# wooginawunan/multi-modal-uncertainty

Hardware: AMD Instinct MI355X
Metric: image+text samples/sec/node, MMBT Food-101 bs=256 seq=512; ECE/NLL parity (higher is better)
Workload: dtype bf16

## Files before the change

include/mmu.h:

```cpp
#ifndef MMU_H
#define MMU_H
#include <stdint.h>

#ifdef __cplusplus
extern "C" {
#endif

typedef void* mmu_stream_t;

enum { MMU_BF16 = 0, MMU_F32 = 1 };

#define MMU_ABI_VERSION 4
int mmu_version(void);
const char* mmu_last_error(void);

int mmu_set_seed_offset(const uint64_t* dev_counter);

enum {
  MMU_EPI_STORE = 0,
  MMU_EPI_BIAS_GELU = 1,
  MMU_EPI_BIAS_DROP_RES = 2,
  MMU_EPI_DGELU = 3,
  MMU_EPI_ADD_RES = 4,
  MMU_EPI_BIAS_DROP_QGELU = 5,
  MMU_EPI_STORE_STATS = 6,
  MMU_EPI_STORE_BNB = 7,
  MMU_EPI_ADD_RES_BNB = 8,
};
typedef struct mmu_epilogue {
  int32_t kind;
  int32_t accumulate;
  const float* bias;
  int64_t bias_bstride;
  const void* residual;
  int64_t ldr, res_bstride;
  void* aux;
  int64_t ldx, aux_bstride;
  float* colsum;
  int64_t colsum_bstride;
  float drop_p;
  uint64_t seed;
  float* workspace;
  int64_t workspace_floats;
  const float* res_ln_mean;
  const float* res_ln_rstd;
  const float* res_ln_w;
  const float* res_ln_b;
  int64_t res_ln_bstride;
  const void* bn_x;
  const uint8_t* bn_mask;
  const float* bn_mean;
  const uint8_t* res_mask;
} mmu_epilogue;

int mmu_gemm(const void* A, int64_t lda, int a_kmajor,
             const void* B, int64_t ldb, int b_kmajor,
             void* C, int64_t ldc, int c_dtype,
             int64_t M, int64_t N, int64_t K,
             int64_t batch, int64_t strideA, int64_t strideB, int64_t strideC,
             const mmu_epilogue* epi, mmu_stream_t stream);

int mmu_colsum_reduce(const float* partial, int64_t parts, int64_t N, float* out,
                      int accumulate, mmu_stream_t stream);
int mmu_colsum_reduce_multi(int n, const float* const* partial, const int64_t* parts, float* const* out, int64_t N,
                            int accumulate, mmu_stream_t stream);
int mmu_colsum_bf16(const void* X, int64_t M, int64_t N, int64_t ldx, float* partial,
                    float* out, int accumulate, mmu_stream_t stream);

int mmu_transpose_bf16_batched(const int64_t* jobs, int n_jobs, int64_t max_rows, int64_t max_cols,
                               mmu_stream_t stream);

int mmu_attention_fwd(const void* QKV, int64_t ld_qkv, const float* keymask,
                      void* O, int64_t ld_o, float* LSE,
                      int64_t batch, int64_t L, int64_t heads,
                      float drop_p, uint64_t seed, uint64_t* dropmask, mmu_stream_t stream);
int mmu_attention_bwd(const void* QKV, int64_t ld_qkv, const float* keymask,
                      const void* O, int64_t ld_o, const void* dO, int64_t ld_do,
                      const float* LSE, float* delta, void* dQKV, int64_t ld_dqkv,
                      int64_t batch, int64_t L, int64_t heads,
                      float drop_p, uint64_t seed, const uint64_t* dropmask, float* dbias_parts,
                      mmu_stream_t stream);

int mmu_layernorm_fwd(const void* X, const float* w, const float* b, void* Y,
                      float* mean, float* rstd, int64_t rows, int64_t H, float eps,
                      int64_t group_rows, int64_t param_stride, mmu_stream_t stream);
int mmu_layernorm_bwd(const void* dY, const void* X, const float* mean, const float* rstd,
                      const float* w, void* dX, void* dXdrop, float drop_p, uint64_t seed,
                      float* part_dw, float* part_db, float* part_dbias,
                      int64_t rows, int64_t H, int64_t rows_per_part, mmu_stream_t stream);

int mmu_layernorm_fwd_f32(const float* X, const float* w, const float* b, void* Y, float* Y32,
                          float* mean, float* rstd, int64_t rows, int64_t H, float eps,
                          int64_t group_rows, int64_t param_stride, mmu_stream_t stream);
int mmu_layernorm_bwd_f32(const void* dY, const float* X, const float* mean, const float* rstd,
                          const float* w, void* dX, void* dXdrop, float drop_p, uint64_t seed,
                          float* part_dw, float* part_db, float* part_dbias,
                          int64_t rows, int64_t H, int64_t rows_per_part, mmu_stream_t stream);

int mmu_layernorm_bwd_res(const void* dY, const void* X, const float* mean, const float* rstd,
                          const float* w, const void* dRes, void* dX,
                          float* part_dw, float* part_db, float* part_dbias,
                          int64_t rows, int64_t H, int64_t rows_per_part, mmu_stream_t stream);

int mmu_seqattn_fwd(const void* QKV, int64_t ld_qkv, void* O, int64_t ld_o, float* LSE2,
                    int64_t S, int64_t N, int64_t heads, int64_t head_dim, mmu_stream_t stream);
int mmu_seqattn_bwd(const void* QKV, int64_t ld_qkv, const void* O, int64_t ld_o,
                    const void* dO, int64_t ld_do, const float* LSE2, float* delta,
                    void* dQKV, int64_t ld_dqkv, int64_t S, int64_t N, int64_t heads,
                    int64_t head_dim, mmu_stream_t stream);

int mmu_embed_fwd(const int64_t* ids, const int64_t* seg, const int64_t* txt_mask,
                  const float* proj, const float* word, const float* pos, const float* type,
                  const float* ln_w, const float* ln_b, float eps,
                  int64_t cls_id, int64_t sep_id,
                  const int64_t* idx, int64_t V, int64_t B, int64_t T, int64_t n_img, int64_t Lout,
                  int64_t H, float drop_txt, float drop_img, uint64_t seed,
                  void* X, float* X32, float* keymask, float* mean, float* rstd, mmu_stream_t stream);
int64_t mmu_embed_bwd_ws_floats(int64_t B, int64_t T, int64_t n_img);
int mmu_embed_bwd(const void* dX, const int64_t* ids, const int64_t* seg,
                  const float* proj, const float* word, const float* pos, const float* type,
                  const float* ln_w, const float* mean, const float* rstd,
                  int64_t cls_id, int64_t sep_id, int64_t B, int64_t T, int64_t n_img, int64_t H,
                  float drop_txt, float drop_img, uint64_t seed, float* d_word, float* d_pos, float* d_type, float* d_ln_w, float* d_ln_b,
                  float* d_proj, float* ws, mmu_stream_t stream);

int mmu_image_normalize(const uint8_t* in, int64_t n, const float* mean, const float* stdv, void* out,
                        int out_dtype, mmu_stream_t stream);

int mmu_maxpool_fwd(const void* x, int64_t B, int64_t H, int64_t W, int64_t C, void* y, uint8_t* argmax,
                    mmu_stream_t stream);
int mmu_maxpool_bwd(const void* dy, const uint8_t* argmax, int64_t B, int64_t H, int64_t W, int64_t C, void* dx,
                    mmu_stream_t stream);

int mmu_row_pool_fwd(const void* fmap, int64_t B, int64_t Hh, int64_t Ww, int64_t C, int64_t n,
                     float* out, mmu_stream_t stream);
int mmu_row_pool_bwd(const float* dout, int64_t B, int64_t Hh, int64_t Ww, int64_t C, int64_t n,
                     void* dfmap, mmu_stream_t stream);

int mmu_conv3x3_wgrad(const void* dY, const void* X, float* dW, int64_t n_img, int64_t H, int64_t W,
                      int64_t Cin, int64_t Cout, int accumulate, float* ws, int64_t ws_floats,
                      mmu_stream_t stream);

int mmu_conv3x3_implicit(const void* X, const void* Wk, void* Y, int64_t n_img, int64_t H, int64_t W,
                         int64_t C, int64_t N, float* ws, int64_t ws_floats, mmu_stream_t stream);

int mmu_conv_implicit(const void* X, const void* Wk, void* Y, int64_t n_img, int64_t H, int64_t W, int64_t C,
                      int64_t N, int64_t ksize, int64_t stride, float* ws, int64_t ws_floats,
                      mmu_stream_t stream);
int mmu_conv_implicit_stats(const void* X, const void* Wk, void* Y, int64_t n_img, int64_t H, int64_t W, int64_t C,
                            int64_t N, int64_t ksize, int64_t stride, float* stats, float* ws, int64_t ws_floats,
                            mmu_stream_t stream);
int mmu_conv3x3_implicit_bnb(const void* X, const void* Wk, void* Y, int64_t n_img, int64_t H, int64_t W, int64_t C,
                             int64_t N, const void* bn_x, const uint8_t* bn_mask, const float* bn_mean,
                             float* stats, float* ws, int64_t ws_floats, mmu_stream_t stream);
int mmu_conv_wgrad(const void* dY, const void* X, float* dW, int64_t n_img, int64_t H, int64_t W, int64_t Cin,
                   int64_t Cout, int64_t ksize, int64_t stride, int accumulate, float* ws, int64_t ws_floats,
                   mmu_stream_t stream);

int mmu_stem_conv_fwd(const void* X, const void* Wk, void* Y, int64_t n_img, int64_t H, int64_t W,
                      mmu_stream_t stream);
int64_t mmu_stem_conv_wgrad_ws_floats(int64_t n_img, int64_t H, int64_t W);
int mmu_stem_conv_wgrad(const void* dY, const void* X, float* dW, int64_t n_img, int64_t H, int64_t W,
                        int accumulate, float* ws, int64_t ws_floats, mmu_stream_t stream);

int64_t mmu_batchnorm_ws_bytes(int64_t C);
int mmu_batchnorm_fwd(const void* X, const void* skip, void* Y, int64_t rows, int64_t C,
                      const float* weight, const float* bias, float* running_mean, float* running_var,
                      int64_t* num_batches_tracked, int training, float momentum, float eps, int relu,
                      float* save_mean, float* save_invstd, void* relu_mask, const void* skip_res, void* y_res,
                      void* ws, int64_t ws_bytes, mmu_stream_t stream);
int mmu_batchnorm_fwd_parts(const void* X, const void* skip, void* Y, int64_t rows, int64_t C, const float* parts,
                            int64_t nparts, const float* weight, const float* bias, float* running_mean,
                            float* running_var, int64_t* num_batches_tracked, float momentum, float eps, int relu,
                            float* save_mean, float* save_invstd, void* relu_mask, const void* skip_res, void* y_res,
                            void* ws, int64_t ws_bytes, mmu_stream_t stream);
int mmu_batchnorm_bwd(const void* dY, const void* Y, const void* relu_mask, const void* X, int64_t rows,
                      int64_t C, const float* weight, const float* save_mean, const float* save_invstd, int relu,
                      void* dX, void* dSkip, float* dweight, float* dbias, void* ws, int64_t ws_bytes,
                      mmu_stream_t stream);

int mmu_batchnorm_bwd_parts(const void* dY, const void* Y, const void* relu_mask, const void* X, int64_t rows,
                            int64_t C, const float* parts, int64_t nparts, const float* weight,
                            const float* save_mean, const float* save_invstd, int relu, void* dX, void* dSkip,
                            float* dweight, float* dbias, void* ws, int64_t ws_bytes, mmu_stream_t stream);

int mmu_batchnorm_stats(const void* X, int64_t rows, int64_t C, double* sums, void* ws, int64_t ws_bytes,
                        mmu_stream_t stream);
int mmu_batchnorm_fwd_sums(const void* X, const void* skip, void* Y, int64_t rows, int64_t C, const double* sums,
                           const float* weight, const float* bias, float* running_mean, float* running_var,
                           int64_t* num_batches_tracked, float momentum, float eps, int relu, float* save_mean,
                           float* save_invstd, void* relu_mask, const void* skip_res, void* y_res, void* ws,
                           int64_t ws_bytes, mmu_stream_t stream);
int mmu_batchnorm_bwd_reduce(const void* dY, const void* Y, const void* relu_mask, const void* X, int64_t rows,
                             int64_t C, const float* save_mean, const float* save_invstd, int relu, double* sums,
                             float* dweight, float* dbias, void* ws, int64_t ws_bytes, mmu_stream_t stream);
int mmu_batchnorm_bwd_sums(const void* dY, const void* Y, const void* relu_mask, const void* X, int64_t rows,
                           int64_t C, const double* sums, const float* weight, const float* save_mean,
                           const float* save_invstd, int relu, void* dX, void* dSkip, void* ws, int64_t ws_bytes,
                           mmu_stream_t stream);

int mmu_bertadam_step(float* params, const float* grads, float* m, float* v, void* bf16_copy,
                      const int64_t* table, int32_t* steps, int64_t n_tensors, int64_t n_chunks,
                      float lr_decay, float lr_nodecay, float wd, float warmup, float t_total,
                      float b1, float b2, float eps, float max_grad_norm, float grad_scale,
                      float* ws, int64_t ws_floats, mmu_stream_t stream);

int mmu_uncertainty(const float* logits, const int64_t* y, int64_t S, int64_t R, int64_t C,
                    float* p_bar, float* nll, float* conf, float* correct, mmu_stream_t stream);
int mmu_ece_bins(const float* conf, const float* correct, int64_t S, int64_t n_bins,
                 float* out, mmu_stream_t stream);

int mmu_timing_enable(int on);
int mmu_timing_pause(int paused);
int mmu_timing_read(double* total_ms, int64_t* launches, double* flops);

#ifdef __cplusplus
}
#endif
#endif
```

multi-modal-uncertainty_amd/csrc/attention.hip:

```cpp
#include "mmu_common.h"
#include "mmu_internal.h"
#include <cstdlib>
#include <type_traits>
#include <utility>

namespace mmu {

constexpr float LOG2E = 1.4426950408889634f;
constexpr float LN2 = 0.6931471805599453f;
constexpr float NEG_INF = -__builtin_huge_valf();

static __device__ __forceinline__ uint32_t lowbias32(uint32_t x) {
  x ^= x >> 16; x *= 0x7feb352du; x ^= x >> 15; x *= 0x846ca68bu; x ^= x >> 16;
  return x;
}
static __device__ __forceinline__ uint32_t seed_for(uint64_t seed, int bh) {
  return lowbias32((uint32_t)seed ^ lowbias32((uint32_t)(seed >> 32) + 0x9E3779B9u * (uint32_t)(bh + 1)));
}
static __device__ __forceinline__ uint32_t drop_pair(uint32_t sbh, uint32_t q, uint32_t key, uint32_t Lp) {
  return lowbias32(((q * Lp + key) >> 1) ^ sbh);
}

static __device__ __forceinline__ float max3f(float a, float b, float c) {
  return __builtin_fmaxf(__builtin_fmaxf(a, b), c);
// ... 558 lines not shown
#pragma unroll
  for (int ks = 0; ks < 4; ++ks) {
    uint4 u = qv ? *(const uint4*)(base + (int64_t)q * p.ld_qkv + 16 * ks + 8 * h) : make_uint4(0, 0, 0, 0);
    qf[ks] = scale_frag(u, 0.125f);
    uint4 v = qv ? *(const uint4*)(dob + 16 * ks + 8 * h) : make_uint4(0, 0, 0, 0);
    df[ks] = *(bf16x8*)&v;
  }
  float dsum = 0.f;
  {
    const bf16* ob = p.o + ((int64_t)b * L + q) * p.ld_o + hd * 64;
#pragma unroll
    for (int ks = 0; ks < 4; ++ks) {
      uint4 u = qv ? *(const uint4*)(ob + 16 * ks + 8 * h) : make_uint4(0, 0, 0, 0);
      const bf16x8 ov = *(bf16x8*)&u;
#pragma unroll
      for (int e = 0; e < 8; ++e) dsum = fmaf(bf2f(ov[e]), bf2f(df[ks][e]), dsum);
    }
    dsum += __shfl_xor(dsum, 32, 64);
    if (qv && h == 0) p.delta[(int64_t)bh * L + q] = -dsum / zs;
  }
  const float nlse2 = qv ? -p.lse[(int64_t)bh * L + q] * LOG2E : -__builtin_huge_valf();
  const float ndz = -dsum / zs;
  const uint32_t ndz_bits = __float_as_uint(ndz);
  f32x16 dq[2];
#pragma unroll
  for (int i = 0; i < 16; ++i) { dq[0][i] = 0.f; dq[1][i] = 0.f; }

  uint32_t kv_off[4];
#pragma unroll
  for (int pc = 0; pc < 4; ++pc) {
    const int piece = 4 * (w & 1) + pc;
    const int row = 8 * piece + (l >> 3), c = (l & 7) ^ fsw(row);
    kv_off[pc] = (uint32_t)((row * p.ld_qkv + (w < 2 ? HD : 2 * HD) + hd * 64 + 8 * c) * 2);
  }
  const uint32_t m_off = (uint32_t)(16 * l), kw_off = (uint32_t)(((q0w + (l >> 1)) * nkv * 8) + 4 * (l & 1));
  auto issue = [&](int j) {
    char* st = smem + (j % DQ_NS) * DQ_STAGE;
    const int k0 = j * 64;
    char* dst = st + (w < 2 ? 0 : DQ_TILE);
    const __amdgpu_buffer_rsrc_t rt = urs_at(kv_base, kv_bytes, k0 * p.ld_qkv * 2);
#pragma unroll
    for (int pc = 0; pc < 4; ++pc) dma16(rt, dst + (4 * (w & 1) + pc) * 1024, kv_off[pc]);
    if (w == 0 && l < 16) dma16(urs_at(m_base, L * 4, k0 * 4), st + 2 * DQ_TILE, m_off);
    dma4(urs_at(k_base, k_bytes, j * 8), st + 2 * DQ_TILE + 256 + w * 256, kw_off);
  };
  auto wait_for = [&](int ahead) {
    if (w == 0) {
      if (ahead >= 1) asm volatile("s_waitcnt vmcnt(6)" ::: "memory");
      else asm volatile("s_waitcnt vmcnt(0)" ::: "memory");
    } else {
      if (ahead >= 1) asm volatile("s_waitcnt vmcnt(5)" ::: "memory");
      else asm volatile("s_waitcnt vmcnt(0)" ::: "memory");
    }
  };
  asm volatile("s_waitcnt vmcnt(0)" ::: "memory");
  for (int j = 0; j < DQ_NS - 1 && j < nkv; ++j) issue(j);
  auto tile_step = [&](int j, auto sg_tag) {
    constexpr int SG = decltype(sg_tag)::value;
    const int ahead = nkv - 1 - j < DQ_NS - 2 ? nkv - 1 - j : DQ_NS - 2;
    wait_for(ahead);
    raw_barrier();
    if (j + DQ_NS - 1 < nkv) issue(j + DQ_NS - 1);
    const char* st = smem + SG * DQ_STAGE;
    const char* Ks = st;
    const char* Vs = st + DQ_TILE;
    const float* mk = (const float*)(st + 2 * DQ_TILE);
    const uint32_t* kwords = (const uint32_t*)(st + 2 * DQ_TILE + 256 + w * 256);
    if (wave_live) {
      const uint64_t kw = drop ? ((uint64_t)kwords[2 * (l & 31) + 1] << 32 | kwords[2 * (l & 31)]) : ~0ull;
      const uint64_t kwh = kw >> (4 * h);
#pragma unroll
      for (int st2 = 0; st2 < 2; ++st2) {
        if (st2 == 1 && 64 * j + 32 >= L) break;
        const uint32_t kw32 = (uint32_t)(kwh >> (32 * st2));
        f32x16 sc, dp;
#pragma unroll
        for (int g = 0; g < 4; ++g) {
          const f32x4 mv = *(const f32x4*)(mk + 32 * st2 + 8 * g + 4 * h);
#pragma unroll
          for (int e = 0; e < 4; ++e) {
            sc[4 * g + e] = mv[e];
            dp[4 * g + e] = ndz;
          }
        }
#pragma unroll
        for (int ks = 0; ks < 4; ++ks) {
          sc = __builtin_amdgcn_mfma_f32_32x32x16_bf16(row_frag(Ks, 32 * st2, ks, l), qf[ks], sc, 0, 0, 0);
          dp = __builtin_amdgcn_mfma_f32_32x32x16_bf16(row_frag(Vs, 32 * st2, ks, l), df[ks], dp, 0, 0, 0);
        }
        auto one = [&](auto r_tag) {
          constexpr int r = decltype(r_tag)::value;
          const float pr = __builtin_amdgcn_exp2f(fmaf(sc[r], LOG2E, nlse2));
          const uint32_t m = keepmask<(r & 3) + 8 * (r >> 2)>(kw32);
          sc[r] = pr * __uint_as_float(bfi(m, __float_as_uint(dp[r]), ndz_bits));
        };
        static_for(one, std::make_integer_sequence<int, 16>{});
#pragma unroll
        for (int s2 = 0; s2 < 2; ++s2) {
          bf16x8 sf = acc_frag(sc, s2);
#pragma unroll
          for (int dt = 0; dt < 2; ++dt)
            dq[dt] = __builtin_amdgcn_mfma_f32_32x32x16_bf16(tr_frag(Ks, 32 * st2 + 16 * s2, 32 * dt, l), sf, dq[dt],
                                                             0, 0, 0);
        }
      }
    }
    };
  for (int j0 = 0; j0 < nkv; j0 += DQ_NS) {
    tile_step(j0, std::integral_constant<int, 0>{});
    if (j0 + 1 < nkv) tile_step(j0 + 1, std::integral_constant<int, 1>{});
    if (j0 + 2 < nkv) tile_step(j0 + 2, std::integral_constant<int, 2>{});
  }
  if (p.colsum) {
    constexpr int RS = 68;
    static_assert(4 * 32 * RS * 4 <= DQ_NS * DQ_STAGE, "dQ column-sum rows exceed the ring's LDS");
    float* rows = (float*)smem;
    raw_barrier();
    float* mine = rows + w * 32 * RS + (l & 31) * RS;
    const float sc = qv ? 0.125f * zs : 0.f;
#pragma unroll
    for (int dt = 0; dt < 2; ++dt)
#pragma unroll
      for (int g = 0; g < 4; ++g)
        *(float4*)(mine + 32 * dt + 8 * g + 4 * h) =
            make_float4(dq[dt][4 * g] * sc, dq[dt][4 * g + 1] * sc, dq[dt][4 * g + 2] * sc, dq[dt][4 * g + 3] * sc);
    raw_barrier();
    if (t < 64) {
      float v = 0.f;
      for (int r = 0; r < 128; ++r) v += rows[r * RS + t];
      p.colsum[((int64_t)bx * p.batch + b) * HD + hd * 64 + t] = v;
    }
  }
  if (!qv) return;
  bf16* ob = p.out + ((int64_t)b * L + q) * p.ld_out + hd * 64;
#pragma unroll
  for (int dt = 0; dt < 2; ++dt)
#pragma unroll
    for (int g = 0; g < 4; ++g) {
      const float s = 0.125f * zs;
      bf16x4 v = {f2bf(dq[dt][4 * g] * s), f2bf(dq[dt][4 * g + 1] * s), f2bf(dq[dt][4 * g + 2] * s),
                  f2bf(dq[dt][4 * g + 3] * s)};
      *(bf16x4*)(ob + 32 * dt + 8 * g + 4 * h) = v;
    }
}

void attention_bwd_launch(const AttnParams& p, hipStream_t s) {
  hipLaunchKernelGGL(attn_dq_dma_kernel, dim3((p.L + 127) / 128, p.batch * p.heads), dim3(256), 0, s, p);
  if (drop_thr(p.drop_p))
    hipLaunchKernelGGL(attn_dkdv_dma_kernel<true>, dim3((p.L + 63) / 64, p.batch * p.heads), dim3(128), 0, s, p);
  else
    hipLaunchKernelGGL(attn_dkdv_dma_kernel<false>, dim3((p.L + 63) / 64, p.batch * p.heads), dim3(128), 0, s, p);
}

}
```

multi-modal-uncertainty_amd/csrc/capi.hip:

```cpp
#include <stdarg.h>
#include <stdio.h>
#include <map>
#include <tuple>
#include <mutex>
#include <string>
#include <vector>
#include "mmu_internal.h"
#include <cstdlib>
#include <cmath>

using namespace mmu;

static thread_local std::string g_err;

namespace mmu {
const uint64_t* g_seed_off = nullptr;
}

int mmu_set_seed_offset(const uint64_t* dev_counter) {
  g_seed_off = dev_counter;
  return 0;
}

static int fail(const char* fmt, ...) {
  char buf[512];
  va_list ap;
  va_start(ap, fmt);
  vsnprintf(buf, sizeof buf, fmt, ap);
  va_end(ap);
  g_err = buf;
  return 1;
}

static int check_launch(const char* what) {
  hipError_t e = hipGetLastError();
  if (e != hipSuccess) return fail("%s: launch failed: %s", what, hipGetErrorString(e));
  return 0;
}

namespace {
struct Timing {
  std::mutex mu;
  bool on = false;
  bool paused = false;
  std::vector<std::pair<hipEvent_t, hipEvent_t>> pool, used;
  std::vector<double> flops;
} g_t;

std::pair<hipEvent_t, hipEvent_t> take_events() {
  std::lock_guard<std::mutex> lk(g_t.mu);
  std::pair<hipEvent_t, hipEvent_t> ev;
  if (!g_t.pool.empty()) {
    ev = g_t.pool.back();
    g_t.pool.pop_back();
  } else {
    (void)hipEventCreate(&ev.first);
    (void)hipEventCreate(&ev.second);
  }
  return ev;
}
constexpr int64_t TAIL_WS_FLOATS = 8ll << 20;
float* tail_workspace(int64_t floats, hipStream_t s, int slot = 0) {
  static std::mutex mu;
  static std::map<std::tuple<int, hipStream_t, int>, float*> bufs;
  if (floats > TAIL_WS_FLOATS) return nullptr;
  int dev = 0;
  if (hipGetDevice(&dev) != hipSuccess) return nullptr;
  std::lock_guard<std::mutex> lk(mu);
  auto it = bufs.find({dev, s, slot});
  if (it != bufs.end()) return it->second;
  hipStreamCaptureStatus st = hipStreamCaptureStatusNone;
  if (hipStreamIsCapturing(s, &st) != hipSuccess || st != hipStreamCaptureStatusNone) return nullptr;
  void* b = nullptr;
  if (hipMalloc(&b, sizeof(float) * TAIL_WS_FLOATS) != hipSuccess) {
    (void)hipGetLastError();
    return nullptr;
  }
  bufs[{dev, s, slot}] = (float*)b;
  return (float*)b;
}
}

extern "C" {

int mmu_version(void) { return MMU_ABI_VERSION; }
const char* mmu_last_error(void) { return g_err.c_str(); }

int mmu_timing_enable(int on) {
  std::lock_guard<std::mutex> lk(g_t.mu);
  g_t.on = on != 0;
  for (auto& e : g_t.used) g_t.pool.push_back(e);
  g_t.used.clear();
  g_t.flops.clear();
  return 0;
}

int mmu_timing_pause(int paused) {
  std::lock_guard<std::mutex> lk(g_t.mu);
  g_t.paused = paused != 0;
  return 0;
}

int mmu_timing_read(double* total_ms, int64_t* launches, double* flops) {
  std::lock_guard<std::mutex> lk(g_t.mu);
  double tot = 0.0, fl = 0.0;
  for (size_t i = 0; i < g_t.used.size(); ++i) {
    (void)hipEventSynchronize(g_t.used[i].second);
    float ms = 0.f;
    if (hipEventElapsedTime(&ms, g_t.used[i].first, g_t.used[i].second) != hipSuccess) return fail("timing: elapsed");
    tot += ms;
    fl += g_t.flops[i];
  }
  *total_ms = tot;
  *launches = (int64_t)g_t.used.size();
  *flops = fl;
  return 0;
}

int mmu_gemm(const void* A, int64_t lda, int a_kmajor, const void* B, int64_t ldb, int b_kmajor, void* C,
             int64_t ldc, int c_dtype, int64_t M, int64_t N, int64_t K, int64_t batch, int64_t strideA,
             int64_t strideB, int64_t strideC, const mmu_epilogue* epi, mmu_stream_t stream) {
  if (!A || !B || !C) return fail("mmu_gemm: null operand");
  if (M <= 0 || N <= 0 || K <= 0 || batch <= 0) return fail("mmu_gemm: bad shape M=%ld N=%ld K=%ld", M, N, K);
  if (N % 128) return fail("mmu_gemm: N=%ld must be a multiple of 128", N);
  if ((a_kmajor || b_kmajor) && K % 64) return fail("mmu_gemm: K=%ld must be a multiple of 64 for a K-major operand", K);
  if (!a_kmajor && M % 128) return fail("mmu_gemm: M=%ld must be a multiple of 128 when A is M-major", M);
  if ((lda % 8) || (ldb % 8) || (ldc % 4)) return fail("mmu_gemm: leading dims must be 16-B aligned");
  if (c_dtype != MMU_BF16 && c_dtype != MMU_F32) return fail("mmu_gemm: bad c_dtype");
  GemmParams p{};
  p.A = (const bf16*)A; p.B = (const bf16*)B; p.C = C;
  p.lda = lda; p.ldb = ldb; p.ldc = ldc; p.M = M; p.N = N; p.K = K;
  p.sA = strideA; p.sB = strideB; p.sC = strideC;
  const int64_t a_span = 2 * (a_kmajor ? (M + 256) * lda : (K + 64) * lda);
  const int64_t b_span = 2 * (b_kmajor ? (N + 256) * ldb : (K + 64) * ldb);
  const bool big = M >= 256 && N >= 256 && a_span < (1ll << 32) - 4096 && b_span < (1ll << 32) - 4096;
  const int tile = big ? 256 : 128;
  p.tiles_m = (int)((M + tile - 1) / tile);
  p.tiles_n = (int)((N + tile - 1) / tile);
  int kind = MMU_EPI_STORE;
  if (epi) kind = epi->kind;
  p.group_m = p.tiles_n <= 3 ? 1 : ((b_kmajor && kind != MMU_EPI_DGELU) ? 8 : 2);
  if (epi) {
    kind = epi->kind;
    p.accumulate = epi->accumulate;
    p.bias = epi->bias; p.bias_bstride = epi->bias_bstride;
    p.residual = epi->residual; p.ldr = epi->ldr; p.res_bstride = epi->res_bstride;
    p.aux = epi->aux; p.ldx = epi->ldx; p.aux_bstride = epi->aux_bstride;
    p.colsum = epi->colsum; p.colsum_bstride = epi->colsum_bstride;
    p.drop_p = epi->drop_p; p.seed = epi->seed; p.seed_off = g_seed_off;
    p.res_ln_mean = epi->res_ln_mean; p.res_ln_rstd = epi->res_ln_rstd;
    p.res_ln_w = epi->res_ln_w; p.res_ln_b = epi->res_ln_b; p.res_ln_bstride = epi->res_ln_bstride;
    p.bn_x = (const bf16*)epi->bn_x; p.bn_mask = epi->bn_mask; p.bn_mean = epi->bn_mean;
    p.res_mask = epi->res_mask;
  }
  p.kind = kind;
  if (kind < 0 || kind > MMU_EPI_ADD_RES_BNB) return fail("mmu_gemm: bad epilogue kind %d", kind);
  if ((kind == MMU_EPI_STORE_BNB || kind == MMU_EPI_ADD_RES_BNB) &&
      (!p.colsum || !p.bn_x || !p.bn_mean || batch != 1 || !a_kmajor || b_kmajor || p.accumulate || p.bias ||
       ldc != N || c_dtype != MMU_BF16))
    return fail("mmu_gemm: *_BNB needs the table (colsum), bn_x, bn_mean, batch 1, K-major A, N-major B, "
                "bf16 C with ldc == N, no bias / accumulate");
  if (kind == MMU_EPI_STORE_STATS && (!p.colsum || batch != 1 || !a_kmajor || !b_kmajor || p.accumulate))
    return fail("mmu_gemm: STORE_STATS needs the stats table (colsum), batch 1, K-major A and B, no accumulate");
  if (kind != MMU_EPI_STORE && kind != MMU_EPI_BIAS_DROP_RES && c_dtype != MMU_BF16)
    return fail("mmu_gemm: fused epilogues other than BIAS_DROP_RES write bf16");
  if (kind == MMU_EPI_BIAS_DROP_RES && c_dtype == MMU_F32 && (ldc % 4 || (epi && epi->ldr % 4)))
    return fail("mmu_gemm: f32 hidden-stream epilogue needs 16-B aligned rows");
  {
    const int nln = !!p.res_ln_mean + !!p.res_ln_rstd + !!p.res_ln_w + !!p.res_ln_b;
    if (nln && (nln != 4 || kind != MMU_EPI_BIAS_DROP_RES || c_dtype != MMU_F32))
      return fail("mmu_gemm: res_ln_* (all four) only with BIAS_DROP_RES into an f32 C");
  }
  if (kind == MMU_EPI_DGELU && !p.aux) return fail("mmu_gemm: DGELU epilogue needs aux");
  if ((kind == MMU_EPI_BIAS_DROP_RES || kind == MMU_EPI_ADD_RES || kind == MMU_EPI_ADD_RES_BNB) && !p.residual)
    return fail("mmu_gemm: epilogue needs residual");
  if (p.res_mask && ((kind != MMU_EPI_ADD_RES && kind != MMU_EPI_ADD_RES_BNB) || epi->ldr != N || batch != 1))
    return fail("mmu_gemm: res_mask only with ADD_RES / ADD_RES_BNB, batch 1, ldr == N");
  if (p.accumulate && c_dtype != MMU_F32) return fail("mmu_gemm: accumulate needs f32 C");
  if (p.drop_p < 0.f || p.drop_p >= 1.f) return fail("mmu_gemm: drop_p out of range");
  p.splitk = 1;
  p.kchunk = K;
  if (kind == MMU_EPI_STORE && c_dtype == MMU_F32 && !p.bias && !p.colsum && epi && epi->workspace && K >= 1024) {
    const int64_t tiles = (int64_t)p.tiles_m * p.tiles_n * batch;
    const int64_t max_split = 64, min_k = K >= 32768 ? 1024 : 256;
    int64_t want = (640 + tiles - 1) / tiles;
    if (want > K / min_k) want = K / min_k;
    if (want > max_split) want = max_split;
    const int64_t cap = epi->workspace_floats / (batch * M * N);
    if (want > cap) want = cap;
    if (want >= 2) {
      int64_t chunk = (K + want - 1) / want;
      chunk = (chunk + 63) / 64 * 64;
      p.kchunk = chunk;
      p.splitk = (int)((K + chunk - 1) / chunk);
      p.ws = epi->workspace;
    }
  }
  const char* wide_env = getenv("MMU_GEMM_WIDE");
  const char* wide_min_env = getenv("MMU_GEMM_WIDE_MIN_TILES");
  const int wide_mode = wide_env ? atoi(wide_env) : 1;
  const int64_t wide_min = wide_min_env ? (int64_t)atoll(wide_min_env) : (int64_t)1024;
  const bool tail_kind = kind == MMU_EPI_STORE || kind == MMU_EPI_BIAS_GELU || kind == MMU_EPI_BIAS_DROP_RES ||
                         kind == MMU_EPI_DGELU || kind == MMU_EPI_ADD_RES;
  const bool wide_kind = tail_kind && kind != MMU_EPI_DGELU;
  const bool wide = (wide_mode == 2 ? tail_kind : wide_mode == 1 && wide_kind && N >= 2304) && big && a_kmajor &&
                    b_kmajor && N % 384 == 0 && p.splitk == 1 &&
                    2 * (M + 256) * lda < (1ll << 32) - 4096 && 2 * (N + 384) * ldb < (1ll << 32) - 4096 &&
                    (M + 255) / 256 * (N / 384) * batch >= wide_min;
  if (wide) {
    p.tiles_m = (int)((M + 255) / 256);
    p.tiles_n = (int)(N / 384);
    p.group_m = p.tiles_n <= 2 ? 1 : (kind != MMU_EPI_DGELU ? 8 : 2);
  }
  const char* tail_env = getenv("MMU_GEMM_TAIL");
  const int tail_mode = tail_env ? atoi(tail_env) : 1;
  int64_t tail_rows = 0, m_main = M, tail_chunk = K;
  int tail_split = 1;
  float* tail_ws = nullptr;
  if ((tail_mode == 2 || (tail_mode == 1 && wide)) && big && batch == 1 && p.splitk == 1 && tail_kind &&
      a_kmajor && K >= 512) {
    const int64_t tiles = (int64_t)p.tiles_m * p.tiles_n, left = tiles % 256;
    if (tiles > 256 && left > 0 && left % p.tiles_n == 0 && left * 8 <= 256) {
      m_main = (int64_t)(p.tiles_m - left / p.tiles_n) * 256;
      tail_rows = M - m_main;
      const int64_t st = (tail_rows + 127) / 128 * (N / 128);
      int64_t sk = 256 / st;
      if (sk > K / 256) sk = K / 256;
      if (sk < 1) sk = 1;
      tail_chunk = ((K + sk - 1) / sk + 63) / 64 * 64;
      tail_split = (int)((K + tail_chunk - 1) / tail_chunk);
      tail_ws = tail_split >= 2 ? tail_workspace((int64_t)tail_split * tail_rows * N, (hipStream_t)stream) : nullptr;
      if (!tail_ws) {
        tail_rows = 0;
        m_main = M;
      }
    }
  }
  hipStream_t s = (hipStream_t)stream;
  bool timed;
  std::pair<hipEvent_t, hipEvent_t> ev;
  {
    std::lock_guard<std::mutex> lk(g_t.mu);
    timed = g_t.on && !g_t.paused;
  }
  if (timed) {
    ev = take_events();
    (void)hipEventRecord(ev.first, s);
  }
  const char* csp_env = getenv("MMU_GEMM_CS_PART");
  const bool cs_rows_ok = p.colsum && batch == 1 && p.splitk == 1 && kind != MMU_EPI_STORE_STATS &&
                          kind != MMU_EPI_STORE_BNB && kind != MMU_EPI_ADD_RES_BNB && (!csp_env || atoi(csp_env) != 0);
  const int cs_rows_main = (big && !wide) ? 128 : 64;
  const int64_t cs_parts_main = (m_main + cs_rows_main - 1) / cs_rows_main;
  const int64_t cs_parts = cs_parts_main + (tail_rows + 63) / 64;
  float* cs_part = cs_rows_ok ? tail_workspace(cs_parts * N, s, 1) : nullptr;
  if (cs_part) {
    p.cs_part = cs_part;
    p.cs_m0 = 0;
    p.cs_rows = cs_rows_main;
  }
  {
    GemmParams pm = p;
    if (tail_rows) pm.tiles_m = (int)(m_main / 256);
    if (!(wide && gemm_wide_launch(pm, c_dtype == MMU_F32, (int)batch, s)))
      gemm_launch(pm, a_kmajor != 0, b_kmajor != 0, c_dtype == MMU_F32, big, (int)batch, s);
  }
  if (tail_rows) {
    GemmParams pt = p;
    pt.A = p.A + m_main * lda;
    pt.M = tail_rows;
    pt.kind = MMU_EPI_STORE;
    pt.accumulate = 0;
    pt.splitk = tail_split;
    pt.kchunk = tail_chunk;
    pt.ws = tail_ws;
    pt.tiles_m = (int)((tail_rows + 127) / 128);
    pt.tiles_n = (int)(N / 128);
    pt.group_m = 1;
    pt.cs_part = nullptr;
    gemm_launch(pt, true, b_kmajor != 0, true, false, 1, s);
    GemmParams pe = p;
    if (cs_part) {
      pe.cs_part = cs_part + cs_parts_main * N;
      pe.cs_m0 = m_main;
      pe.cs_rows = 64;
    }
    splitk_epilogue_launch(pe, c_dtype == MMU_F32, tail_ws, m_main, tail_rows, tail_split, s);
  }
  if (cs_part) colsum_reduce_launch(cs_part, cs_parts, N, p.colsum, 1, s);
  if (p.splitk > 1) splitk_reduce_launch(p, (int)batch, s);
  if (timed) {
    (void)hipEventRecord(ev.second, s);
    std::lock_guard<std::mutex> lk(g_t.mu);
    g_t.used.push_back(ev);
    g_t.flops.push_back(2.0 * (double)M * (double)N * (double)K * (double)batch);
  }
  return check_launch("mmu_gemm");
}

int mmu_transpose_bf16_batched(const int64_t* jobs, int n_jobs, int64_t max_rows, int64_t max_cols,
                               mmu_stream_t stream) {
  if (!jobs || n_jobs <= 0 || n_jobs > 65535 || max_rows <= 0 || max_cols <= 0)
    return fail("mmu_transpose_bf16_batched: bad args");
  transpose_bf16_batched_launch(jobs, n_jobs, max_rows, max_cols, (hipStream_t)stream);
  return check_launch("mmu_transpose_bf16_batched");
}

int mmu_colsum_reduce(const float* partial, int64_t parts, int64_t N, float* out, int accumulate,
                      mmu_stream_t stream) {
  if (!partial || !out || parts <= 0 || N <= 0) return fail("mmu_colsum_reduce: bad args");
  colsum_reduce_launch(partial, parts, N, out, accumulate, (hipStream_t)stream);
  return check_launch("mmu_colsum_reduce");
}

int mmu_colsum_reduce_multi(int n, const float* const* partial, const int64_t* parts, float* const* out, int64_t N,
                            int accumulate, mmu_stream_t stream) {
  if (n <= 0 || n > COLSUM_MULTI || !partial || !parts || !out || N <= 0)
    return fail("mmu_colsum_reduce_multi: bad args (1 <= n <= %d)", COLSUM_MULTI);
  ColsumJobs jobs{};
  for (int z = 0; z < n; ++z) {
    if (!partial[z] || !out[z] || parts[z] <= 0) return fail("mmu_colsum_reduce_multi: bad job %d", z);
    jobs.part[z] = partial[z];
    jobs.parts[z] = parts[z];
    jobs.out[z] = out[z];
  }
  colsum_reduce_multi_launch(jobs, n, N, accumulate, (hipStream_t)stream);
  return check_launch("mmu_colsum_reduce_multi");
}

int mmu_colsum_bf16(const void* X, int64_t M, int64_t N, int64_t ldx, float* partial, float* out, int accumulate,
                    mmu_stream_t stream) {
  if (!X || !out || M <= 0 || N <= 0 || N % 8 || ldx % 8) return fail("mmu_colsum_bf16: bad args");
  colsum_bf16_launch((const bf16*)X, M, N, ldx, partial, out, accumulate, (hipStream_t)stream);
  return check_launch("mmu_colsum_bf16");
}

static int attn_common(int64_t ld_qkv, int64_t batch, int64_t L, int64_t heads, float drop_p) {
  if (batch <= 0 || L <= 0 || heads <= 0) return fail("attention: bad shape");
  if (ld_qkv < 3 * heads * 64 || ld_qkv % 8) return fail("attention: ld_qkv too small / unaligned");
  if (drop_p < 0.f || drop_p >= 1.f) return fail("attention: drop_p out of range");
  if ((int64_t)batch * heads > 65535 * 64) return fail("attention: batch*heads too large");
  if (L > 576) return fail("attention: L=%ld > 576 (the kernels stage ceil(L/64) <= 9 key tiles)", L);
  return 0;
}

int mmu_attention_fwd(const void* QKV, int64_t ld_qkv, const float* keymask, void* O, int64_t ld_o, float* LSE,
                      int64_t batch, int64_t L, int64_t heads, float drop_p, uint64_t seed, uint64_t* dropmask,
                      mmu_stream_t stream) {
  if (!QKV || !keymask || !O || !LSE) return fail("mmu_attention_fwd: null pointer");
  if (attn_common(ld_qkv, batch, L, heads, drop_p)) return 1;
  if (ld_o < heads * 64 || ld_o % 8) return fail("mmu_attention_fwd: bad ld_o");
  if (batch * heads > 65535) return fail("mmu_attention_fwd: batch*heads > 65535");
  AttnParams p{};
  p.qkv = (const bf16*)QKV; p.ld_qkv = ld_qkv; p.keymask = keymask; p.out = (bf16*)O; p.ld_out = ld_o;
  p.lse = LSE; p.batch = (int)batch; p.L = (int)L; p.heads = (int)heads; p.drop_p = drop_p; p.seed = seed;
  p.seed_off = g_seed_off;
  p.dropmask = dropmask;
  attention_fwd_launch(p, (hipStream_t)stream);
  return check_launch("mmu_attention_fwd");
}

int mmu_attention_bwd(const void* QKV, int64_t ld_qkv, const float* keymask, const void* O, int64_t ld_o,
                      const void* dO, int64_t ld_do, const float* LSE, float* delta, void* dQKV, int64_t ld_dqkv,
                      int64_t batch, int64_t L, int64_t heads, float drop_p, uint64_t seed,
                      const uint64_t* dropmask, float* dbias_parts, mmu_stream_t stream) {
  if (!QKV || !keymask || !O || !dO || !LSE || !delta || !dQKV) return fail("mmu_attention_bwd: null pointer");
  if ((uint32_t)(drop_p * 65536.0f + 0.5f) != 0 && !dropmask)
    return fail("mmu_attention_bwd: dropout needs the forward's dropmask");
  if (attn_common(ld_qkv, batch, L, heads, drop_p)) return 1;
  if (ld_dqkv < 3 * heads * 64 || ld_do < heads * 64 || ld_o < heads * 64 || ld_do % 8 || ld_o % 8 || ld_dqkv % 4)
    return fail("mmu_attention_bwd: bad ld");
  if (batch * heads > 65535) return fail("mmu_attention_bwd: batch*heads > 65535");
  AttnParams p{};
  p.qkv = (const bf16*)QKV; p.ld_qkv = ld_qkv; p.keymask = keymask; p.o = (const bf16*)O; p.ld_o = ld_o;
  p.dout = (const bf16*)dO; p.ld_do = ld_do; p.lse = (float*)LSE; p.delta = delta; p.out = (bf16*)dQKV;
  p.ld_out = ld_dqkv; p.batch = (int)batch; p.L = (int)L; p.heads = (int)heads; p.drop_p = drop_p; p.seed = seed;
  p.seed_off = g_seed_off;
  p.dropmask = (uint64_t*)dropmask;
  p.colsum = dbias_parts;
  attention_bwd_launch(p, (hipStream_t)stream);
  return check_launch("mmu_attention_bwd");
}

int mmu_layernorm_fwd(const void* X, const float* w, const float* b, void* Y, float* mean, float* rstd, int64_t rows,
                      int64_t H, float eps, int64_t group_rows, int64_t param_stride, mmu_stream_t stream) {
  if (!X || !w || !b || !Y) return fail("mmu_layernorm_fwd: null pointer");
  if ((mean == nullptr) != (rstd == nullptr)) return fail("mmu_layernorm_fwd: mean/rstd must both be given or NULL");
  if (rows <= 0 || H <= 0 || H % 256 || H > 1024) return fail("mmu_layernorm_fwd: H=%ld must be 256/512/768/1024", H);
  if (group_rows <= 0) group_rows = rows;
  if (param_stride < 0) return fail("mmu_layernorm_fwd: bad param_stride");
  layernorm_fwd_launch((const bf16*)X, w, b, (bf16*)Y, mean, rstd, rows, H, eps, group_rows, param_stride,
                       (hipStream_t)stream);
  return check_launch("mmu_layernorm_fwd");
}

int mmu_layernorm_bwd(const void* dY, const void* X, const float* mean, const float* rstd, const float* w, void* dX,
                      void* dXdrop, float drop_p, uint64_t seed, float* part_dw, float* part_db, float* part_dbias,
                      int64_t rows, int64_t H, int64_t rows_per_part, mmu_stream_t stream) {
  if (!dY || !X || !mean || !rstd || !w || !dX) return fail("mmu_layernorm_bwd: null pointer");
  if (rows <= 0 || H <= 0 || H % 256 || H > 1024 || rows_per_part <= 0) return fail("mmu_layernorm_bwd: bad shape");
  if (drop_p < 0.f || drop_p >= 1.f) return fail("mmu_layernorm_bwd: drop_p out of range");
  layernorm_bwd_launch((const bf16*)dY, X, false, mean, rstd, w, (bf16*)dX, (bf16*)dXdrop, nullptr, drop_p, seed,
                       g_seed_off, part_dw, part_db, part_dbias, rows, H, rows_per_part, (hipStream_t)stream);
  return check_launch("mmu_layernorm_bwd");
}

int mmu_layernorm_fwd_f32(const float* X, const float* w, const float* b, void* Y, float* Y32, float* mean,
                          float* rstd, int64_t rows, int64_t H, float eps, int64_t group_rows, int64_t param_stride,
                          mmu_stream_t stream) {
  if (!X || !w || !b || !Y) return fail("mmu_layernorm_fwd_f32: null pointer");
  if ((mean == nullptr) != (rstd == nullptr)) return fail("mmu_layernorm_fwd_f32: mean/rstd must both be given or NULL");
  if (rows <= 0 || H <= 0 || H % 256 || H > 1024) return fail("mmu_layernorm_fwd_f32: H=%ld must be 256/512/768/1024", H);
  if (group_rows <= 0) group_rows = rows;
  if (param_stride < 0) return fail("mmu_layernorm_fwd_f32: bad param_stride");
  layernorm_fwd32_launch(X, w, b, (bf16*)Y, Y32, mean, rstd, rows, H, eps, group_rows, param_stride,
                         (hipStream_t)stream);
  return check_launch("mmu_layernorm_fwd_f32");
}

int mmu_layernorm_bwd_f32(const void* dY, const float* X, const float* mean, const float* rstd, const float* w,
                          void* dX, void* dXdrop, float drop_p, uint64_t seed, float* part_dw, float* part_db,
                          float* part_dbias, int64_t rows, int64_t H, int64_t rows_per_part, mmu_stream_t stream) {
  if (!dY || !X || !mean || !rstd || !w || !dX) return fail("mmu_layernorm_bwd_f32: null pointer");
  if (rows <= 0 || H <= 0 || H % 256 || H > 1024 || rows_per_part <= 0) return fail("mmu_layernorm_bwd_f32: bad shape");
  if (drop_p < 0.f || drop_p >= 1.f) return fail("mmu_layernorm_bwd_f32: drop_p out of range");
  layernorm_bwd_launch((const bf16*)dY, X, true, mean, rstd, w, (bf16*)dX, (bf16*)dXdrop, nullptr, drop_p, seed,
                       g_seed_off, part_dw, part_db, part_dbias, rows, H, rows_per_part, (hipStream_t)stream);
  return check_launch("mmu_layernorm_bwd_f32");
}

int mmu_layernorm_bwd_res(const void* dY, const void* X, const float* mean, const float* rstd, const float* w,
                          const void* dRes, void* dX, float* part_dw, float* part_db, float* part_dbias, int64_t rows,
                          int64_t H, int64_t rows_per_part, mmu_stream_t stream) {
  if (!dY || !X || !mean || !rstd || !w || !dX || !dRes) return fail("mmu_layernorm_bwd_res: null pointer");
  if (rows <= 0 || H <= 0 || H % 256 || H > 1024 || rows_per_part <= 0) return fail("mmu_layernorm_bwd_res: bad shape");
  layernorm_bwd_launch((const bf16*)dY, X, false, mean, rstd, w, (bf16*)dX, nullptr, (const bf16*)dRes, 0.f, 0,
                       nullptr, part_dw, part_db, part_dbias, rows, H, rows_per_part, (hipStream_t)stream);
  return check_launch("mmu_layernorm_bwd_res");
}

static int seqattn_check(const char* what, int64_t ld_qkv, int64_t S, int64_t N, int64_t heads, int64_t D) {
  if (S <= 0 || N <= 0 || heads <= 0) return fail("%s: bad shape", what);
  if (D != 64 && D != 128 && D != 256) return fail("%s: head_dim %ld not in {64, 128, 256}", what, D);
  if (ld_qkv < 3 * heads * D || ld_qkv % 8) return fail("%s: ld_qkv too small / unaligned", what);
  if (N * heads > 65535) return fail("%s: N*heads > 65535", what);
  return 0;
}

int mmu_seqattn_fwd(const void* QKV, int64_t ld_qkv, void* O, int64_t ld_o, float* LSE2, int64_t S, int64_t N,
                    int64_t heads, int64_t head_dim, mmu_stream_t stream) {
  if (!QKV || !O || !LSE2) return fail("mmu_seqattn_fwd: null pointer");
  if (seqattn_check("mmu_seqattn_fwd", ld_qkv, S, N, heads, head_dim)) return 1;
  if (ld_o < heads * head_dim || ld_o % 4) return fail("mmu_seqattn_fwd: bad ld_o");
  SeqAttnParams p{};
  p.qkv = (const bf16*)QKV; p.ld_qkv = ld_qkv;
  p.out = (bf16*)O; p.ld_out = ld_o;
  p.lse2 = LSE2;
  p.S = (int)S; p.N = (int)N; p.heads = (int)heads; p.D = (int)head_dim; p.E = (int)(heads * head_dim);
  p.scale = 1.0f / sqrtf((float)head_dim);
  seqattn_fwd_launch(p, (hipStream_t)stream);
  return check_launch("mmu_seqattn_fwd");
}

int mmu_seqattn_bwd(const void* QKV, int64_t ld_qkv, const void* O, int64_t ld_o, const void* dO, int64_t ld_do,
                    const float* LSE2, float* delta, void* dQKV, int64_t ld_dqkv, int64_t S, int64_t N, int64_t heads,
                    int64_t head_dim, mmu_stream_t stream) {
  if (!QKV || !O || !dO || !LSE2 || !delta || !dQKV) return fail("mmu_seqattn_bwd: null pointer");
  if (seqattn_check("mmu_seqattn_bwd", ld_qkv, S, N, heads, head_dim)) return 1;
  if (ld_dqkv < 3 * heads * head_dim || ld_dqkv % 4 || ld_o % 4 || ld_do % 8) return fail("mmu_seqattn_bwd: bad ld");
  SeqAttnParams p{};
  p.qkv = (const bf16*)QKV; p.ld_qkv = ld_qkv;
  p.o = (const bf16*)O; p.ld_o = ld_o;
  p.dout = (const bf16*)dO; p.ld_do = ld_do;
  p.out = (bf16*)dQKV; p.ld_out = ld_dqkv;
  p.lse2 = (float*)LSE2; p.delta = delta;
  p.S = (int)S; p.N = (int)N; p.heads = (int)heads; p.D = (int)head_dim; p.E = (int)(heads * head_dim);
  p.scale = 1.0f / sqrtf((float)head_dim);
  seqattn_bwd_launch(p, (hipStream_t)stream);
  return check_launch("mmu_seqattn_bwd");
}


int mmu_embed_fwd(const int64_t* ids, const int64_t* seg, const int64_t* txt_mask, const float* proj, const float* word,
                  const float* pos, const float* type, const float* ln_w, const float* ln_b, float eps, int64_t cls_id,
                  int64_t sep_id, const int64_t* idx, int64_t V, int64_t B, int64_t T, int64_t n_img, int64_t Lout,
                  int64_t H, float drop_txt, float drop_img, uint64_t seed, void* X, float* X32, float* keymask,
                  float* mean, float* rstd, mmu_stream_t stream) {
  if (H != 768) return fail("mmu_embed_fwd: H must be 768");
  if (!word || !pos || !type || !ln_w || !ln_b || !X || !keymask || !proj) return fail("mmu_embed_fwd: null pointer");
  if (T > 0 && (!ids || !seg)) return fail("mmu_embed_fwd: text ids/segments missing");
  if (V <= 0 || B <= 0 || Lout <= 0 || n_img <= 0) return fail("mmu_embed_fwd: bad shape");
  if (!idx && Lout != n_img + 2 + T) return fail("mmu_embed_fwd: identity variant needs Lout == n_img+2+T");
  EmbedParams p{};
  p.ids = ids; p.seg = seg; p.txt_mask = txt_mask; p.idx = idx; p.proj = proj; p.word = word; p.pos = pos;
  p.type = type; p.ln_w = ln_w; p.ln_b = ln_b; p.eps = eps; p.cls_id = cls_id; p.sep_id = sep_id; p.V = V; p.B = B;
  p.T = T; p.n_img = n_img; p.Lout = Lout; p.H = H; p.X = (bf16*)X; p.X32 = X32;
  if (drop_txt < 0.f || drop_txt >= 1.f || drop_img < 0.f || drop_img >= 1.f) return fail("mmu_embed_fwd: bad dropout");
  p.drop_txt = drop_txt; p.drop_img = drop_img; p.seed = seed; p.seed_off = g_seed_off; p.keymask = keymask; p.mean = mean; p.rstd = rstd;
  embed_fwd_launch(p, (hipStream_t)stream);
  return check_launch("mmu_embed_fwd");
}

int64_t mmu_embed_bwd_ws_floats(int64_t B, int64_t T, int64_t n_img) {
  return 4 * embed_bwd_blocks(B, n_img + 2 + T) * 768;
}

int mmu_embed_bwd(const void* dX, const int64_t* ids, const int64_t* seg, const float* proj, const float* word,
                  const float* pos, const float* type, const float* ln_w, const float* mean, const float* rstd,
                  int64_t cls_id, int64_t sep_id, int64_t B, int64_t T, int64_t n_img, int64_t H, float drop_txt,
                  float drop_img, uint64_t seed, float* d_word,
                  float* d_pos, float* d_type, float* d_ln_w, float* d_ln_b, float* d_proj, float* ws,
                  mmu_stream_t stream) {
  if (H != 768) return fail("mmu_embed_bwd: H must be 768");
  if (!dX || !ids || !seg || !proj || !word || !pos || !type || !ln_w || !mean || !rstd || !d_word || !d_pos ||
      !d_type || !d_ln_w || !d_ln_b || !d_proj || !ws)
    return fail("mmu_embed_bwd: null pointer");
  EmbedBwdParams q{};
  q.dX = (const bf16*)dX; q.ids = ids; q.seg = seg; q.proj = proj; q.word = word; q.pos = pos; q.type = type;
  q.ln_w = ln_w; q.mean = mean; q.rstd = rstd; q.cls_id = cls_id; q.sep_id = sep_id; q.B = B; q.T = T;
  q.n_img = n_img; q.H = H; q.drop_txt = drop_txt; q.drop_img = drop_img; q.seed = seed; q.seed_off = g_seed_off; q.d_word = d_word; q.d_pos = d_pos; q.d_type = d_type; q.d_ln_w = d_ln_w;
  q.d_ln_b = d_ln_b; q.d_proj = d_proj; q.ws = ws;
  embed_bwd_launch(q, (hipStream_t)stream);
  return check_launch("mmu_embed_bwd");
}

int mmu_image_normalize(const uint8_t* in, int64_t n, const float* mean, const float* stdv, void* out,
                        int out_dtype, mmu_stream_t stream) {
  if (!in || !out || !mean || !stdv || n < 0) return fail("mmu_image_normalize: bad args");
  if (out_dtype != MMU_BF16 && out_dtype != MMU_F32) return fail("mmu_image_normalize: bad out_dtype");
  for (int c = 0; c < 3; ++c)
    if (!(stdv[c] > 0.f)) return fail("mmu_image_normalize: std must be > 0");
  if (n == 0) return 0;
  image_normalize_launch(in, n, mean, stdv, out, out_dtype == MMU_BF16, (hipStream_t)stream);
  return check_launch("mmu_image_normalize");
}

int mmu_maxpool_fwd(const void* x, int64_t B, int64_t H, int64_t W, int64_t C, void* y, uint8_t* argmax,
                    mmu_stream_t stream) {
  if (!x || !y || !argmax || B <= 0 || H <= 0 || W <= 0 || C <= 0 || C % 8 || H > 65536 || W > 65536)
    return fail("mmu_maxpool_fwd: bad args");
  maxpool3s2_fwd_launch((const bf16*)x, B, (int)H, (int)W, (int)C, (int)((H - 1) / 2 + 1), (int)((W - 1) / 2 + 1),
                        (bf16*)y, argmax, (hipStream_t)stream);
  return check_launch("mmu_maxpool_fwd");
}

int mmu_maxpool_bwd(const void* dy, const uint8_t* argmax, int64_t B, int64_t H, int64_t W, int64_t C, void* dx,
                    mmu_stream_t stream) {
  if (!dy || !dx || !argmax || B <= 0 || H <= 0 || W <= 0 || C <= 0 || C % 8 || H > 65536 || W > 65536)
    return fail("mmu_maxpool_bwd: bad args");
  maxpool3s2_bwd_launch((const bf16*)dy, argmax, B, (int)H, (int)W, (int)C, (int)((H - 1) / 2 + 1),
                        (int)((W - 1) / 2 + 1), (bf16*)dx, (hipStream_t)stream);
  return check_launch("mmu_maxpool_bwd");
}

int mmu_row_pool_fwd(const void* fmap, int64_t B, int64_t Hh, int64_t Ww, int64_t C, int64_t n, float* out,
                     mmu_stream_t stream) {
  if (!fmap || !out || C % 8 || n <= 0 || n > Hh) return fail("mmu_row_pool_fwd: bad args");
  row_pool_fwd_launch((const bf16*)fmap, B, Hh, Ww, C, n, out, (hipStream_t)stream);
  return check_launch("mmu_row_pool_fwd");
}

int mmu_row_pool_bwd(const float* dout, int64_t B, int64_t Hh, int64_t Ww, int64_t C, int64_t n, void* dfmap,
                     mmu_stream_t stream) {
  if (!dout || !dfmap || C % 8 || n <= 0 || n > Hh) return fail("mmu_row_pool_bwd: bad args");
  row_pool_bwd_launch(dout, B, Hh, Ww, C, n, (bf16*)dfmap, (hipStream_t)stream);
  return check_launch("mmu_row_pool_bwd");
}

static int conv_geometry(GemmParams& p, int64_t n_img, int64_t H, int64_t W, int64_t C, int64_t ks, int64_t st,
                         int64_t& Mo, const char* who) {
  if (n_img <= 0 || H <= 0 || W <= 0 || C <= 0 || (ks != 1 && ks != 3) || st < 1 || st > 4)
    return fail("%s: bad geometry (n=%ld H=%ld W=%ld C=%ld ksize=%ld stride=%ld)", who, n_img, H, W, C, ks, st);
  const int64_t pad = ks / 2, Ho = (H + 2 * pad - ks) / st + 1, Wo = (W + 2 * pad - ks) / st + 1;
  const int64_t in_bytes = 2 * n_img * H * W * C;
  if (in_bytes >= 0x7FFF0000ll) return fail("%s: input map too large for 32-bit buffer offsets", who);
  p.conv_h = (int)H; p.conv_w = (int)W; p.conv_c = (int)C;
  p.conv_ho = (int)Ho; p.conv_wo = (int)Wo; p.conv_ks = (int)ks; p.conv_s = (int)st; p.conv_pad = (int)pad;
  p.conv_in_bytes = in_bytes;
  Mo = n_img * Ho * Wo;
  return 0;
}
// ... 350 lines not shown
```

multi-modal-uncertainty_amd/csrc/gemm.hip:

```cpp
#include "mmu_common.h"
#include "mmu_internal.h"
#include <cstdlib>

namespace mmu {

constexpr int BKT = 64;

#ifdef MMU_GEMM_STAMPS
__device__ uint64_t g_gemm_stamps[1 << 16][4];
#define GEMM_STAMP(i)                                                                       \
  do {                                                                                      \
    if (threadIdx.x == 0) {                                                                 \
      const int lin_ = (int)(blockIdx.x + gridDim.x * (blockIdx.y + gridDim.y * blockIdx.z)); \
      if (lin_ < (1 << 16)) g_gemm_stamps[lin_][i] = __builtin_amdgcn_s_memtime();          \
    }                                                                                       \
  } while (0)
#else
#define GEMM_STAMP(i) \
  do {                \
  } while (0)
#endif

static __device__ __forceinline__ int sw_mn(int r) { return (r & 7) ^ (((r >> 3) & 1) << 2); }

static __device__ __forceinline__ void tile_of(int pid, int tiles_m, int tiles_n, int group_m, int& tm, int& tn) {
  const int per_group = group_m * tiles_n;
  const int g = pid / per_group, first = g * group_m;
  const int gm = tiles_m - first < group_m ? tiles_m - first : group_m;
  const int r = pid - g * per_group;
  tm = first + r % gm;
  tn = r / gm;
}
static __device__ __forceinline__ void block_tile(const GemmParams& p, int64_t& z, int& slice, int& tm, int& tn) {
  const int ntiles = p.tiles_m * p.tiles_n;
  const int per_z = ntiles * (int)gridDim.y;
  const int lin = (int)(blockIdx.x + gridDim.x * (blockIdx.y + gridDim.y * blockIdx.z));
  const int pid = xcd_remap(lin, per_z * (int)gridDim.z);
  z = pid / per_z;
  const int r = pid - (int)z * per_z;
  slice = r / ntiles;
  tile_of(r - slice * ntiles, p.tiles_m, p.tiles_n, p.group_m, tm, tn);
}

template <bool KMAJ, int ROWB>
static __device__ __forceinline__ bf16x8 s_frag(const char* s, int row0, int ks, int l) {
  if (KMAJ) {
    const int row = row0 + (l & 15), c = 4 * ks + (l >> 4);
    return *(const bf16x8*)(s + row * 128 + ((c ^ (row & 7)) << 4));
  } else {
    const int g = l >> 4, i = l & 15, q = i >> 2, p = i & 3;
    const int b = row0 >> 4;
    const int k0 = 32 * ks + 8 * g + q, k1 = k0 + 4;
    const char* a0 = s + k0 * ROWB + ((b ^ sw_mn(k0)) << 5) + 8 * p;
    const char* a1 = s + k1 * ROWB + ((b ^ sw_mn(k1)) << 5) + 8 * p;
    bf16x4 lo = __builtin_amdgcn_ds_read_tr16_b64_v4bf16((MMU_LDS(bf16x4)*)a0);
    bf16x4 hi = __builtin_amdgcn_ds_read_tr16_b64_v4bf16((MMU_LDS(bf16x4)*)a1);
    return __builtin_shufflevector(lo, hi, 0, 1, 2, 3, 4, 5, 6, 7);
  }
}


template <int EPI, bool OUT_F32>
static __device__ __forceinline__ void epi_oct(const GemmParams& p, void* cdst, bf16* xdst, uint64_t qd,
                                               float (&v)[8], const float (&in)[8], float scale, uint32_t thr,
                                               uint64_t seed) {
  if (EPI == MMU_EPI_BIAS_GELU) {
    float d[8];
#pragma unroll
    for (int r = 0; r < 8; ++r) gelu_pair(v[r], v[r], d[r]);
    if (xdst) {
      bf16x8 o;
#pragma unroll
      for (int r = 0; r < 8; ++r) o[r] = f2bf(d[r]);
      *(bf16x8*)xdst = o;
    }
  } else if (EPI == MMU_EPI_BIAS_DROP_RES) {
    if (thr) {
      const uint32_t keep = mmu_keep4(seed, qd, thr) | (mmu_keep4(seed, qd + 1, thr) << 4);
#pragma unroll
      for (int r = 0; r < 8; ++r) v[r] = ((keep >> r) & 1) ? v[r] * scale : 0.f;
    }
#pragma unroll
    for (int r = 0; r < 8; ++r) v[r] += in[r];
  } else if (EPI == MMU_EPI_BIAS_DROP_QGELU) {
    uint32_t keep = 0xFFu;
    if (thr) keep = mmu_keep4(seed, qd, thr) | (mmu_keep4(seed, qd + 1, thr) << 4);
    float d[8];
#pragma unroll
    for (int r = 0; r < 8; ++r) {
      const float kz = ((keep >> r) & 1) ? scale : 0.f;
      const float u = v[r] * kz;
      const float sg = __builtin_amdgcn_rcpf(1.0f + __builtin_amdgcn_exp2f(u * -2.4554669595930157f));
      v[r] = u * sg;
      d[r] = kz * fmaf(1.702f * u * sg, 1.0f - sg, sg);
    }
    if (xdst) {
      bf16x8 o;
#pragma unroll
      for (int r = 0; r < 8; ++r) o[r] = f2bf(d[r]);
      *(bf16x8*)xdst = o;
    }
  } else if (EPI == MMU_EPI_DGELU) {
#pragma unroll
    for (int r = 0; r < 8; ++r) v[r] *= in[r];
  } else if (EPI == MMU_EPI_ADD_RES) {
#pragma unroll
    for (int r = 0; r < 8; ++r) v[r] += in[r];
  }
  if (OUT_F32) {
    float4* C = (float4*)cdst;
    float4 lo = make_float4(v[0], v[1], v[2], v[3]), hi = make_float4(v[4], v[5], v[6], v[7]);
    if (p.accumulate) {
      const float4 c0 = C[0], c1 = C[1];
      lo.x += c0.x; lo.y += c0.y; lo.z += c0.z; lo.w += c0.w;
      hi.x += c1.x; hi.y += c1.y; hi.z += c1.z; hi.w += c1.w;
    }
    C[0] = lo;
    C[1] = hi;
  } else {
    bf16x8 o;
#pragma unroll
    for (int r = 0; r < 8; ++r) o[r] = f2bf(v[r]);
    *(bf16x8*)cdst = o;
  }
}

template <int EPI_, bool OUT_F32, int NJ, int PJ = 4>
static __device__ __forceinline__ void epilogue_block(const GemmParams& p, int64_t z, int slice, int64_t mw,
                                                      int64_t nw, f32x4 (&acc)[4][NJ], int l, char* ws) {
  constexpr bool BNB = EPI_ == MMU_EPI_STORE_BNB || EPI_ == MMU_EPI_ADD_RES_BNB;
  constexpr int EPI = EPI_ == MMU_EPI_STORE_BNB ? MMU_EPI_STORE : EPI_ == MMU_EPI_ADD_RES_BNB ? MMU_EPI_ADD_RES : EPI_;
  if (nw >= p.N) return;
  const int q = l & 7, rr = l >> 3;
  const int64_t n = nw + 8 * q;
  const bool slab = EPI == MMU_EPI_STORE && p.splitk > 1;
  float* slab_base = slab ? p.ws + (z * p.splitk + slice) * p.M * p.N : nullptr;
  const float* bias = (!slab && p.bias && EPI != MMU_EPI_DGELU && EPI != MMU_EPI_ADD_RES)
                          ? p.bias + z * p.bias_bstride : nullptr;
  const bf16* res = p.residual ? (const bf16*)p.residual + z * p.res_bstride : nullptr;
  bf16* aux = p.aux ? (bf16*)p.aux + z * p.aux_bstride : nullptr;
  const float scale = p.drop_p > 0.f ? 1.0f / (1.0f - p.drop_p) : 1.0f;
  const uint32_t thr = (uint32_t)(p.drop_p * 65536.0f + 0.5f);
  float bv[8];
  {
    float4 b0 = make_float4(0.f, 0.f, 0.f, 0.f), b1 = b0;
    if (bias) { b0 = *(const float4*)(bias + n); b1 = *(const float4*)(bias + n + 4); }
    bv[0] = b0.x; bv[1] = b0.y; bv[2] = b0.z; bv[3] = b0.w; bv[4] = b1.x; bv[5] = b1.y; bv[6] = b1.z; bv[7] = b1.w;
  }
  constexpr bool STATS = EPI == MMU_EPI_STORE_STATS;
  const bool want_cs = !STATS && !BNB && p.colsum != nullptr && !slab;
  constexpr bool TAB = STATS || BNB;
  float mu[8];
  const int64_t b_l = BNB ? (mw + rr) * p.N + n : 0;
  if (BNB) {
    const float4 m0 = *(const float4*)(p.bn_mean + n), m1 = *(const float4*)(p.bn_mean + n + 4);
    mu[0] = m0.x; mu[1] = m0.y; mu[2] = m0.z; mu[3] = m0.w; mu[4] = m1.x; mu[5] = m1.y; mu[6] = m1.z; mu[7] = m1.w;
  }
  float cs[8];
#pragma unroll
  for (int r = 0; r < 8; ++r) cs[r] = 0.f;
  constexpr bool LOADS = EPI == MMU_EPI_BIAS_DROP_RES || EPI == MMU_EPI_DGELU || EPI == MMU_EPI_ADD_RES;
  constexpr bool RES32 = OUT_F32 && EPI == MMU_EPI_BIAS_DROP_RES;
  const bf16* src = EPI == MMU_EPI_DGELU ? (const bf16*)aux : res;
  const float* src32 = RES32 && p.residual ? (const float*)p.residual + z * p.res_bstride : nullptr;
  const int64_t lds_ = EPI == MMU_EPI_DGELU ? p.ldx : p.ldr;
  const int64_t m_l = mw + rr;
  const int64_t in_l = m_l * lds_ + n;
  const int64_t c_l = z * p.sC + m_l * p.ldc + n;
  constexpr bool XST = EPI == MMU_EPI_BIAS_GELU || EPI == MMU_EPI_BIAS_DROP_QGELU;
  constexpr bool DRP = EPI == MMU_EPI_BIAS_DROP_RES || EPI == MMU_EPI_BIAS_DROP_QGELU;
  const int64_t x_l = XST ? m_l * p.ldx + n : 0;
  const int64_t s_l = EPI == MMU_EPI_STORE ? m_l * p.N + n : 0;
  const int64_t q_l = DRP ? (z * p.M + m_l) * p.N + n : 0;
  const uint64_t seed = DRP && thr ? mmu_eff_seed(p.seed, p.seed_off) : 0;
  const bool res_ln = RES32 && p.res_ln_w != nullptr && !slab;
  float lw[8], lb[8];
  if (RES32) {
    float4 w0 = make_float4(1.f, 1.f, 1.f, 1.f), w1 = w0, b0 = make_float4(0.f, 0.f, 0.f, 0.f), b1 = b0;
    if (res_ln) {
      const float* lw_ = p.res_ln_w + z * p.res_ln_bstride;
      const float* lb_ = p.res_ln_b + z * p.res_ln_bstride;
      w0 = *(const float4*)(lw_ + n); w1 = *(const float4*)(lw_ + n + 4);
      b0 = *(const float4*)(lb_ + n); b1 = *(const float4*)(lb_ + n + 4);
    }
    lw[0] = w0.x; lw[1] = w0.y; lw[2] = w0.z; lw[3] = w0.w; lw[4] = w1.x; lw[5] = w1.y; lw[6] = w1.z; lw[7] = w1.w;
    lb[0] = b0.x; lb[1] = b0.y; lb[2] = b0.z; lb[3] = b0.w; lb[4] = b1.x; lb[5] = b1.y; lb[6] = b1.z; lb[7] = b1.w;
  }
  static_assert(!TAB || PJ == 4, "STORE_STATS / *_BNB: one epilogue pass = one 64-row table block");
#pragma unroll
  for (int pass = 0; pass < NJ / PJ; ++pass) {
    float st1[8], st2[8];
    if (TAB) {
#pragma unroll
      for (int e = 0; e < 8; ++e) st1[e] = st2[e] = 0.f;
    }
    bf16x8 in[RES32 ? 1 : 2 * PJ];
    uint32_t rmk[EPI == MMU_EPI_ADD_RES ? 2 * PJ : 1];
    float4 in32[RES32 ? 2 * PJ : 1][2];
    float rmu[RES32 ? 2 * PJ : 1], rrs[RES32 ? 2 * PJ : 1];
#pragma unroll
    for (int it = 0; it < 2 * PJ; ++it) {
      const int d = 16 * PJ * pass + 8 * it;
      const int64_t m = m_l + d;
      if (RES32) {
        rmu[it] = 0.f;
        rrs[it] = 1.f;
        if (!slab && m < p.M) {
          const float* s32 = src32 + in_l + d * lds_;
          in32[it][0] = *(const float4*)s32;
          in32[it][1] = *(const float4*)(s32 + 4);
          if (res_ln) {
            rmu[it] = p.res_ln_mean[z * p.M + m];
            rrs[it] = p.res_ln_rstd[z * p.M + m];
          }
        } else {
          in32[it][0] = in32[it][1] = make_float4(0.f, 0.f, 0.f, 0.f);
        }
      } else if (LOADS && !slab && m < p.M) {
        in[it] = *(const bf16x8*)(src + in_l + d * lds_);
        if (EPI == MMU_EPI_ADD_RES) rmk[it] = p.res_mask ? (uint32_t)p.res_mask[(in_l + d * lds_) >> 3] : 0xFFu;
      } else {
        in[it] = bf16x8{};
        if (EPI == MMU_EPI_ADD_RES) rmk[it] = 0;
      }
    }
#pragma unroll
    for (int jj = 0; jj < PJ; ++jj) {
      const int r = 16 * jj + (l & 15);
#pragma unroll
      for (int i = 0; i < 4; ++i) {
        const int ch = 4 * i + (l >> 4);
        *(f32x4*)(ws + r * 256 + ((ch ^ (r & 15)) << 4)) = acc[i][PJ * pass + jj];
      }
    }
    bf16x8 bx[BNB ? 2 * PJ : 1];
    uint32_t bm[BNB ? 2 * PJ : 1];
    if (BNB) {
#pragma unroll
      for (int it = 0; it < 2 * PJ; ++it) {
        const int d = 16 * PJ * pass + 8 * it;
        if (!slab && m_l + d < p.M) {
          const int64_t o = b_l + (int64_t)d * p.N;
          bx[it] = *(const bf16x8*)(p.bn_x + o);
          bm[it] = p.bn_mask ? (uint32_t)p.bn_mask[o >> 3] : 0xFFu;
        } else {
          bx[it] = bf16x8{};
          bm[it] = 0;
        }
      }
    }
#pragma unroll
    for (int it = 0; it < 2 * PJ; ++it) {
      const int r = rr + 8 * it;
      const int d = 16 * PJ * pass + 8 * it;
      const int64_t m = m_l + d;
      const float4 lo = *(const float4*)(ws + r * 256 + (((2 * q) ^ (r & 15)) << 4));
      const float4 hi = *(const float4*)(ws + r * 256 + (((2 * q + 1) ^ (r & 15)) << 4));
      if (m >= p.M) continue;
      if (slab) {
        float4* sd = (float4*)(slab_base + s_l + d * p.N);
        sd[0] = lo;
        sd[1] = hi;
        continue;
      }
      float v[8] = {lo.x + bv[0], lo.y + bv[1], lo.z + bv[2], lo.w + bv[3],
                    hi.x + bv[4], hi.y + bv[5], hi.z + bv[6], hi.w + bv[7]};
      float inf[8];
      if (RES32) {
        inf[0] = in32[it][0].x; inf[1] = in32[it][0].y; inf[2] = in32[it][0].z; inf[3] = in32[it][0].w;
        inf[4] = in32[it][1].x; inf[5] = in32[it][1].y; inf[6] = in32[it][1].z; inf[7] = in32[it][1].w;
        if (res_ln) {
#pragma unroll
          for (int e = 0; e < 8; ++e) inf[e] = fmaf((inf[e] - rmu[it]) * rrs[it], lw[e], lb[e]);
        }
      } else {
#pragma unroll
        for (int r = 0; r < 8; ++r) inf[r] = LOADS ? bf2f(in[RES32 ? 0 : it][r]) : 0.f;
        if (EPI == MMU_EPI_ADD_RES) {
#pragma unroll
          for (int r = 0; r < 8; ++r) inf[r] = ((rmk[EPI == MMU_EPI_ADD_RES ? it : 0] >> r) & 1) ? inf[r] : 0.f;
        }
      }
      void* cdst = OUT_F32 ? (void*)((float*)p.C + c_l + d * p.ldc) : (void*)((bf16*)p.C + c_l + d * p.ldc);
      epi_oct<EPI, OUT_F32>(p, cdst, (XST && aux) ? aux + x_l + d * p.ldx : nullptr,
                            DRP ? (uint64_t)(q_l + d * p.N) >> 2 : 0, v, inf, scale, thr, seed);
      if (want_cs) {
#pragma unroll
        for (int e = 0; e < 8; ++e) cs[e] += v[e];
      }
      if (STATS) {
#pragma unroll
        for (int e = 0; e < 8; ++e) {
          const float y = bf2f(f2bf(v[e]));
          st1[e] += y;
          st2[e] = fmaf(y, y, st2[e]);
        }
      }
      if (BNB) {
#pragma unroll
        for (int e = 0; e < 8; ++e) {
          const float g = ((bm[BNB ? it : 0] >> e) & 1) ? bf2f(f2bf(v[e])) : 0.f;
          st1[e] += g;
          st2[e] = fmaf(g, bf2f(bx[BNB ? it : 0][e]) - mu[e], st2[e]);
        }
      }
    }
    if (TAB) {
#pragma unroll
      for (int e = 0; e < 8; ++e) {
#pragma unroll
        for (int o = 8; o < 64; o <<= 1) {
          st1[e] += __shfl_xor(st1[e], o, 64);
          st2[e] += __shfl_xor(st2[e], o, 64);
        }
      }
      const int64_t prow = (mw + 64 * pass) >> 6;
      if (rr == 0 && mw + 64 * pass < p.M) {
        float4* d = (float4*)(p.colsum + 2 * (prow * p.N + n));
#pragma unroll
        for (int e = 0; e < 4; ++e) d[e] = make_float4(st1[2 * e], st2[2 * e], st1[2 * e + 1], st2[2 * e + 1]);
      }
    }
  }
  if (want_cs) {
#pragma unroll
    for (int e = 0; e < 8; ++e) {
      float s = cs[e];
      s += __shfl_xor(s, 8, 64);
      s += __shfl_xor(s, 16, 64);
      s += __shfl_xor(s, 32, 64);
      cs[e] = s;
    }
    if (rr == 0) {
      if (p.cs_part) {
        if (mw >= p.M) return;
        float4* d = (float4*)(p.cs_part + ((mw - p.cs_m0) / p.cs_rows) * p.N + n);
        d[0] = make_float4(cs[0], cs[1], cs[2], cs[3]);
        d[1] = make_float4(cs[4], cs[5], cs[6], cs[7]);
      } else {
        float* out = p.colsum + z * p.colsum_bstride + n;
#pragma unroll
        for (int e = 0; e < 8; ++e) atomicAdd(out + e, cs[e]);
      }
    }
  }
}

constexpr int SBM = 128, SBN = 128;
constexpr int S_STAGE = (SBM * BKT + SBN * BKT) * 2;

template <bool KMAJ>
static __device__ __forceinline__ void g_load(uint4 (&r)[4], const bf16* __restrict__ P, int64_t ld, int64_t r0,
                                              int64_t rlim, int64_t k0, int64_t klim, int t) {
#pragma unroll
  for (int i = 0; i < 4; ++i) {
    if (KMAJ) {
      const int row = (t >> 3) + 32 * i, c = t & 7;
      const int64_t gr = r0 + row;
      r[i] = gr < rlim ? *(const uint4*)(P + gr * ld + k0 + 8 * c) : make_uint4(0, 0, 0, 0);
    } else {
      const int kr = (t >> 4) + 16 * i, c = t & 15;
      const int64_t gk = k0 + kr;
      r[i] = (gk < klim && r0 + 8 * c < rlim) ? *(const uint4*)(P + gk * ld + r0 + 8 * c) : make_uint4(0, 0, 0, 0);
    }
  }
}

template <bool KMAJ>
static __device__ __forceinline__ void s_store(char* s, const uint4 (&r)[4], int t) {
#pragma unroll
  for (int i = 0; i < 4; ++i) {
    int off;
    if (KMAJ) {
      const int row = (t >> 3) + 32 * i, c = t & 7;
      off = row * 128 + ((c ^ (row & 7)) << 4);
    } else {
      const int kr = (t >> 4) + 16 * i, c = t & 15;
      off = kr * 256 + (((c >> 1) ^ sw_mn(kr)) << 5) + ((c & 1) << 4);
    }
    *(uint4*)(s + off) = r[i];
  }
}

template <bool AK, bool BKM, int EPI, bool OUT_F32>
__global__ __launch_bounds__(256) void gemm_small_kernel(GemmParams p) {
  __shared__ __attribute__((aligned(16))) char smem[2 * S_STAGE];
  const int t = threadIdx.x, l = t & 63, w = t >> 6, wm = w >> 1, wn = w & 1;
  int tm, tn, slice;
  int64_t z;
  block_tile(p, z, slice, tm, tn);
  const bf16* __restrict__ A = p.A + z * p.sA;
  const bf16* __restrict__ B = p.B + z * p.sB;
  const int64_t m0 = (int64_t)tm * SBM, n0 = (int64_t)tn * SBN;
  f32x4 acc[4][4];
#pragma unroll
  for (int i = 0; i < 4; ++i)
#pragma unroll
    for (int j = 0; j < 4; ++j) acc[i][j] = f32x4{0.f, 0.f, 0.f, 0.f};
  uint4 ra[4], rb[4];
  const int64_t kb = (int64_t)slice * p.kchunk;
  const int64_t ke = kb + p.kchunk < p.K ? kb + p.kchunk : p.K;
  const int nk = (int)((ke - kb + BKT - 1) / BKT);
  g_load<AK>(ra, A, p.lda, m0, p.M, kb, ke, t);
  g_load<BKM>(rb, B, p.ldb, n0, p.N, kb, ke, t);
  s_store<AK>(smem, ra, t);
  s_store<BKM>(smem + SBM * BKT * 2, rb, t);
  __syncthreads();
  for (int kt = 0; kt < nk; ++kt) {
    const char* sa = smem + (kt & 1) * S_STAGE;
    const char* sb = sa + SBM * BKT * 2;
    const bool more = kt + 1 < nk;
    if (more) {
      g_load<AK>(ra, A, p.lda, m0, p.M, kb + (int64_t)(kt + 1) * BKT, ke, t);
      g_load<BKM>(rb, B, p.ldb, n0, p.N, kb + (int64_t)(kt + 1) * BKT, ke, t);
    }
#pragma unroll
    for (int ks = 0; ks < 2; ++ks) {
      bf16x8 fb[4], fa[4];
#pragma unroll
      for (int i = 0; i < 4; ++i) fb[i] = s_frag<BKM, 256>(sb, 64 * wn + 16 * i, ks, l);
#pragma unroll
      for (int j = 0; j < 4; ++j) fa[j] = s_frag<AK, 256>(sa, 64 * wm + 16 * j, ks, l);
#pragma unroll
      for (int i = 0; i < 4; ++i)
#pragma unroll
        for (int j = 0; j < 4; ++j)
          acc[i][j] = __builtin_amdgcn_mfma_f32_16x16x32_bf16(fb[i], fa[j], acc[i][j], 0, 0, 0);
    }
    if (more) {
      char* dst = smem + ((kt + 1) & 1) * S_STAGE;
      s_store<AK>(dst, ra, t);
      s_store<BKM>(dst + SBM * BKT * 2, rb, t);
    }
    __syncthreads();
  }
  epilogue_block<EPI, OUT_F32, 4>(p, z, slice, m0 + 64 * wm, n0 + 64 * wn, acc, l, smem + w * 16384);
}

// ... 773 lines not shown
```

multi-modal-uncertainty_amd/csrc/layernorm.hip:

```cpp
#include <cstdlib>
#include "mmu_common.h"
#include "mmu_internal.h"

namespace mmu {

constexpr int LN_FWD_ROWS = 16;

template <int NV>
__global__ __launch_bounds__(256) void ln_fwd_kernel(const bf16* __restrict__ X, const float* __restrict__ w,
                                                     const float* __restrict__ b, bf16* __restrict__ Y,
                                                     float* __restrict__ mean, float* __restrict__ rstd,
                                                     int64_t rows, float eps, int64_t group_rows, int64_t pstride) {
  constexpr int H = 256 * NV;
  const int l = threadIdx.x & 63, wv = threadIdx.x >> 6;
  auto load = [&](int64_t row, bf16x4 (&x)[NV]) {
#pragma unroll
    for (int i = 0; i < NV; ++i) x[i] = *(const bf16x4*)(X + row * H + 256 * i + 4 * l);
  };
  auto process = [&](int64_t row, const bf16x4 (&x)[NV]) {
    float v[NV][4];
    float s = 0.f;
#pragma unroll
    for (int i = 0; i < NV; ++i)
#pragma unroll
// ... 24 lines not shown
    const bool two = row + 4 < rend;
    load(row, xa);
    if (two) load(row + 4, xb);
    process(row, xa);
    if (two) process(row + 4, xb);
  }
}

constexpr int LN2_PAIRS = 8;
template <int NV>
__global__ __launch_bounds__(256) void ln_fwd2_kernel(const bf16* __restrict__ X, const float* __restrict__ w,
                                                      const float* __restrict__ b, bf16* __restrict__ Y,
                                                      float* __restrict__ mean, float* __restrict__ rstd,
                                                      int64_t rows, float eps, int64_t group_rows, int64_t pstride) {
  constexpr int H = 256 * NV, CPR = 32 * NV;
  const int l = threadIdx.x & 63, wv = threadIdx.x >> 6;
  int cc[NV];
  bool hb[NV];
#pragma unroll
  for (int i = 0; i < NV; ++i) {
    const int q = 64 * i + l;
    hb[i] = q >= CPR;
    cc[i] = 8 * (hb[i] ? q - CPR : q);
  }
  const int64_t p0 = (int64_t)blockIdx.x * LN2_PAIRS;
  const int64_t np = (rows + 1) / 2;
  const int64_t pend = p0 + LN2_PAIRS < np ? p0 + LN2_PAIRS : np;
  for (int64_t pr = p0 + wv; pr < pend; pr += 8) {
    bf16x8 xa[NV], xb[NV];
    const bool two = pr + 4 < pend;
    auto load = [&](int64_t pp, bf16x8 (&x)[NV]) {
#pragma unroll
      for (int i = 0; i < NV; ++i) {
        const int64_t row = 2 * pp + (hb[i] ? 1 : 0);
        x[i] = row < rows ? *(const bf16x8*)(X + row * H + cc[i]) : bf16x8{};
      }
    };
    auto process = [&](int64_t pp, const bf16x8 (&x)[NV]) {
      float v[NV][8];
      float sa = 0.f, sb = 0.f;
#pragma unroll
      for (int i = 0; i < NV; ++i) {
        float s = 0.f;
#pragma unroll
        for (int e = 0; e < 8; ++e) { v[i][e] = bf2f(x[i][e]); s += v[i][e]; }
        if (hb[i]) sb += s; else sa += s;
      }
      const float mua = wave_sum(sa) / H, mub = wave_sum(sb) / H;
      float qa = 0.f, qb = 0.f;
#pragma unroll
      for (int i = 0; i < NV; ++i) {
        const float mu = hb[i] ? mub : mua;
        float q = 0.f;
#pragma unroll
        for (int e = 0; e < 8; ++e) { const float d = v[i][e] - mu; q += d * d; }
        if (hb[i]) qb += q; else qa += q;
      }
      const float rsa = rsqrtf(wave_sum(qa) / H + eps), rsb = rsqrtf(wave_sum(qb) / H + eps);
      const int64_t ra = 2 * pp;
      const float* wr = w + (ra / group_rows) * pstride;
      const float* br = b + (ra / group_rows) * pstride;
#pragma unroll
      for (int i = 0; i < NV; ++i) {
        const int64_t row = ra + (hb[i] ? 1 : 0);
        if (row >= rows) continue;
        const float mu = hb[i] ? mub : mua, rs = hb[i] ? rsb : rsa;
        const float4 w0 = *(const float4*)(wr + cc[i]), w1 = *(const float4*)(wr + cc[i] + 4);
        const float4 b0 = *(const float4*)(br + cc[i]), b1 = *(const float4*)(br + cc[i] + 4);
        const float ww[8] = {w0.x, w0.y, w0.z, w0.w, w1.x, w1.y, w1.z, w1.w};
        const float bb[8] = {b0.x, b0.y, b0.z, b0.w, b1.x, b1.y, b1.z, b1.w};
        bf16x8 y;
#pragma unroll
        for (int e = 0; e < 8; ++e) y[e] = f2bf((v[i][e] - mu) * rs * ww[e] + bb[e]);
        *(bf16x8*)(Y + row * H + cc[i]) = y;
      }
      if (mean && l == 0) {
        mean[ra] = mua;
        rstd[ra] = rsa;
        if (ra + 1 < rows) { mean[ra + 1] = mub; rstd[ra + 1] = rsb; }
      }
    };
    load(pr, xa);
    if (two) load(pr + 4, xb);
    process(pr, xa);
    if (two) process(pr + 4, xb);
  }
}

template <int NV>
__global__ __launch_bounds__(256) void ln_fwd32_kernel(const float* __restrict__ X, const float* __restrict__ w,
                                                       const float* __restrict__ b, bf16* __restrict__ Y,
                                                       float* __restrict__ Y32, float* __restrict__ mean,
                                                       float* __restrict__ rstd, int64_t rows, float eps,
                                                       int64_t group_rows, int64_t pstride) {
  constexpr int H = 256 * NV;
  const int l = threadIdx.x & 63, wv = threadIdx.x >> 6;
  auto load = [&](int64_t row, float4 (&x)[NV]) {
#pragma unroll
    for (int i = 0; i < NV; ++i) x[i] = *(const float4*)(X + row * H + 256 * i + 4 * l);
  };
  auto process = [&](int64_t row, const float4 (&x)[NV]) {
    float s = 0.f;
#pragma unroll
    for (int i = 0; i < NV; ++i) s += (x[i].x + x[i].y) + (x[i].z + x[i].w);
    const float mu = wave_sum(s) / H;
    float q = 0.f;
#pragma unroll
    for (int i = 0; i < NV; ++i) {
      const float d0 = x[i].x - mu, d1 = x[i].y - mu, d2 = x[i].z - mu, d3 = x[i].w - mu;
      q += (d0 * d0 + d1 * d1) + (d2 * d2 + d3 * d3);
    }
    const float rs = rsqrtf(wave_sum(q) / H + eps);
    const float* wr = w + (row / group_rows) * pstride;
    const float* br = b + (row / group_rows) * pstride;
#pragma unroll
    for (int i = 0; i < NV; ++i) {
      const int c = 256 * i + 4 * l;
      const float4 ww = *(const float4*)(wr + c), bb = *(const float4*)(br + c);
      const float4 y = make_float4((x[i].x - mu) * rs * ww.x + bb.x, (x[i].y - mu) * rs * ww.y + bb.y,
                                   (x[i].z - mu) * rs * ww.z + bb.z, (x[i].w - mu) * rs * ww.w + bb.w);
      *(bf16x4*)(Y + row * H + c) = bf16x4{f2bf(y.x), f2bf(y.y), f2bf(y.z), f2bf(y.w)};
      if (Y32) *(float4*)(Y32 + row * H + c) = y;
    }
    if (l == 0 && mean) { mean[row] = mu; rstd[row] = rs; }
  };
  const int64_t r0 = (int64_t)blockIdx.x * LN_FWD_ROWS;
  const int64_t rend = r0 + LN_FWD_ROWS < rows ? r0 + LN_FWD_ROWS : rows;
  for (int64_t row = r0 + wv; row < rend; row += 8) {
    float4 xa[NV], xb[NV];
    const bool two = row + 4 < rend;
    load(row, xa);
    if (two) load(row + 4, xb);
    process(row, xa);
    if (two) process(row + 4, xb);
  }
}

static __device__ __forceinline__ void ld4f(const bf16* p, float (&o)[4]) {
  const bf16x4 v = *(const bf16x4*)p;
  o[0] = bf2f(v[0]); o[1] = bf2f(v[1]); o[2] = bf2f(v[2]); o[3] = bf2f(v[3]);
}
static __device__ __forceinline__ void ld4f(const float* p, float (&o)[4]) {
  const float4 v = *(const float4*)p;
  o[0] = v.x; o[1] = v.y; o[2] = v.z; o[3] = v.w;
}

template <int NV, typename XT>
__global__ __launch_bounds__(256) void ln_bwd_kernel(const bf16* __restrict__ dY, const XT* __restrict__ X,
                                                     const float* __restrict__ mean, const float* __restrict__ rstd,
                                                     const float* __restrict__ w, bf16* __restrict__ dX,
                                                     bf16* __restrict__ dXd, const bf16* __restrict__ dR,
                                                     float drop_p, uint64_t seed, const uint64_t* seed_off,
                                                     float* __restrict__ pdw, float* __restrict__ pdb,
                                                     float* __restrict__ pdbias, int64_t rows, int rpp) {
  constexpr int H = 256 * NV, nv = NV;
  __shared__ float red[4][H];
  const int l = threadIdx.x & 63, wv = threadIdx.x >> 6;
  const float scale = drop_p > 0.f ? 1.0f / (1.0f - drop_p) : 1.0f;
  const uint32_t thr = (uint32_t)(drop_p * 65536.0f + 0.5f);
  float aw[NV][4], ab[NV][4], ac[NV][4], ww[NV][4];
#pragma unroll
  for (int i = 0; i < NV; ++i)
#pragma unroll
    for (int e = 0; e < 4; ++e) {
      aw[i][e] = ab[i][e] = ac[i][e] = 0.f;
      ww[i][e] = w[256 * i + 4 * l + e];
    }
  struct Row {
    bf16x4 a[NV];
    float x[NV][4];
    float mu, rs;
  };
  auto load = [&](int64_t row, Row& R) {
    R.mu = mean[row];
    R.rs = rstd[row];
#pragma unroll
    for (int i = 0; i < NV; ++i)
      if (i < nv) {
        R.a[i] = *(const bf16x4*)(dY + row * H + 256 * i + 4 * l);
        ld4f(X + row * H + 256 * i + 4 * l, R.x[i]);
      }
  };
  auto process = [&](int64_t row, const Row& R) {
    float g[NV][4], xh[NV][4], dy[NV][4];
    float s1 = 0.f, s2 = 0.f;
#pragma unroll
    for (int i = 0; i < NV; ++i)
      if (i < nv) {
#pragma unroll
        for (int e = 0; e < 4; ++e) {
          dy[i][e] = bf2f(R.a[i][e]);
          xh[i][e] = (R.x[i][e] - R.mu) * R.rs;
          g[i][e] = dy[i][e] * ww[i][e];
          s1 += g[i][e];
          s2 += g[i][e] * xh[i][e];
        }
      }
    s1 = wave_sum(s1) / H;
    s2 = wave_sum(s2) / H;
#pragma unroll
    for (int i = 0; i < NV; ++i)
      if (i < nv) {
        const int c = 256 * i + 4 * l;
        float dx[4];
        bf16x4 rr{};
        if (dR) rr = *(const bf16x4*)(dR + row * H + c);
#pragma unroll
        for (int e = 0; e < 4; ++e) {
          dx[e] = R.rs * (g[i][e] - s1 - xh[i][e] * s2);
          if (dR) dx[e] += bf2f(rr[e]);
          aw[i][e] += dy[i][e] * xh[i][e];
          ab[i][e] += dy[i][e];
        }
        *(bf16x4*)(dX + row * H + c) = bf16x4{f2bf(dx[0]), f2bf(dx[1]), f2bf(dx[2]), f2bf(dx[3])};
        if (dXd) {
          uint32_t keep = thr ? mmu_keep4(mmu_eff_seed(seed, seed_off), (uint64_t)(row * H + c) >> 2, thr) : 0xFu;
#pragma unroll
          for (int e = 0; e < 4; ++e) dx[e] = ((keep >> e) & 1) ? dx[e] * scale : 0.f;
          *(bf16x4*)(dXd + row * H + c) = bf16x4{f2bf(dx[0]), f2bf(dx[1]), f2bf(dx[2]), f2bf(dx[3])};
        }
#pragma unroll
        for (int e = 0; e < 4; ++e) ac[i][e] += dx[e];
      }
  };
  const int64_t r0 = (int64_t)blockIdx.x * rpp;
  const int64_t rend = r0 + rpp < rows ? r0 + rpp : rows;
  for (int64_t row = r0 + wv; row < rend; row += 8) {
    Row A, Bq;
    const bool two = row + 4 < rend;
    load(row, A);
    if (two) load(row + 4, Bq);
    process(row, A);
    if (two) process(row + 4, Bq);
  }
  float* outs[3] = {pdw, pdb, pdbias};
#pragma unroll
  for (int k = 0; k < 3; ++k) {
#pragma unroll
    for (int i = 0; i < NV; ++i)
      if (i < nv)
#pragma unroll
        for (int e = 0; e < 4; ++e) red[wv][256 * i + 4 * l + e] = k == 0 ? aw[i][e] : (k == 1 ? ab[i][e] : ac[i][e]);
    __syncthreads();
    if (outs[k])
      for (int c = threadIdx.x; c < H; c += 256)
        outs[k][(int64_t)blockIdx.x * H + c] = red[0][c] + red[1][c] + red[2][c] + red[3][c];
    __syncthreads();
  }
}

void layernorm_fwd_launch(const bf16* X, const float* w, const float* b, bf16* Y, float* mean, float* rstd,
                          int64_t rows, int64_t H, float eps, int64_t group_rows, int64_t pstride, hipStream_t s) {
  if ((group_rows % 2 == 0 || group_rows >= rows || pstride == 0) && H % 256 == 0 && H <= 1024) {
    const dim3 g2((unsigned)(((rows + 1) / 2 + LN2_PAIRS - 1) / LN2_PAIRS));
#define LNF2(NV) hipLaunchKernelGGL(ln_fwd2_kernel<NV>, g2, dim3(256), 0, s, X, w, b, Y, mean, rstd, rows, eps, \
                                    group_rows, pstride)
    switch (H / 256) {
      case 1: LNF2(1); break;
      case 2: LNF2(2); break;
      case 3: LNF2(3); break;
      default: LNF2(4); break;
    }
#undef LNF2
    return;
  }
  const dim3 g((unsigned)((rows + LN_FWD_ROWS - 1) / LN_FWD_ROWS));
#define LNF(NV) hipLaunchKernelGGL(ln_fwd_kernel<NV>, g, dim3(256), 0, s, X, w, b, Y, mean, rstd, rows, eps, \
                                   group_rows, pstride)
  switch (H / 256) {
    case 1: LNF(1); break;
    case 2: LNF(2); break;
    case 3: LNF(3); break;
    default: LNF(4); break;
  }
#undef LNF
}

void layernorm_fwd32_launch(const float* X, const float* w, const float* b, bf16* Y, float* Y32, float* mean,
                            float* rstd, int64_t rows, int64_t H, float eps, int64_t group_rows, int64_t pstride,
                            hipStream_t s) {
  const dim3 g((unsigned)((rows + LN_FWD_ROWS - 1) / LN_FWD_ROWS));
#define LNF32(NV) hipLaunchKernelGGL(ln_fwd32_kernel<NV>, g, dim3(256), 0, s, X, w, b, Y, Y32, mean, rstd, rows, eps, \
                                     group_rows, pstride)
  switch (H / 256) {
    case 1: LNF32(1); break;
    case 2: LNF32(2); break;
    case 3: LNF32(3); break;
    default: LNF32(4); break;
  }
#undef LNF32
}

template <typename XT>
static void ln_bwd_launch_t(const bf16* dY, const XT* X, const float* mean, const float* rstd, const float* w,
                            bf16* dX, bf16* dXdrop, const bf16* dR, float drop_p, uint64_t seed,
                            const uint64_t* seed_off, float* pdw, float* pdb, float* pdbias, int64_t rows, int64_t H,
                            int64_t rpp, hipStream_t s) {
  const dim3 g((unsigned)((rows + rpp - 1) / rpp));
#define LNB(NV) hipLaunchKernelGGL((ln_bwd_kernel<NV, XT>), g, dim3(256), 0, s, dY, X, mean, rstd, w, dX, dXdrop, dR, \
                                   drop_p, seed, seed_off, pdw, pdb, pdbias, rows, (int)rpp)
  switch (H / 256) {
    case 1: LNB(1); break;
    case 2: LNB(2); break;
    case 3: LNB(3); break;
    default: LNB(4); break;
  }
#undef LNB
}

void layernorm_bwd_launch(const bf16* dY, const void* X, bool x_f32, const float* mean, const float* rstd,
                          const float* w, bf16* dX, bf16* dXdrop, const bf16* dR, float drop_p, uint64_t seed,
                          const uint64_t* seed_off, float* pdw, float* pdb, float* pdbias, int64_t rows, int64_t H,
                          int64_t rpp, hipStream_t s) {
  if (x_f32)
    ln_bwd_launch_t(dY, (const float*)X, mean, rstd, w, dX, dXdrop, dR, drop_p, seed, seed_off, pdw, pdb, pdbias, rows,
                    H, rpp, s);
  else
    ln_bwd_launch_t(dY, (const bf16*)X, mean, rstd, w, dX, dXdrop, dR, drop_p, seed, seed_off, pdw, pdb, pdbias, rows,
                    H, rpp, s);
}

}
```

multi-modal-uncertainty_amd/csrc/mmu_internal.h:

```cpp
#pragma once
#include <hip/hip_runtime.h>
#include <stdint.h>
#include "../../include/mmu.h"

typedef __bf16 bf16;

namespace mmu {

extern const uint64_t* g_seed_off;

struct GemmParams {
  const bf16* A;
  const bf16* B;
  void* C;
  int64_t lda, ldb, ldc, M, N, K, sA, sB, sC;
  int tiles_m, tiles_n;
  int group_m;
  int kind, accumulate;
  const float* bias;
  int64_t bias_bstride;
  const void* residual;
  int64_t ldr, res_bstride;
  void* aux;
  int64_t ldx, aux_bstride;
  float* colsum;
  int64_t colsum_bstride;
  float drop_p;
  uint64_t seed;
  const uint64_t* seed_off;
  const float *res_ln_mean, *res_ln_rstd, *res_ln_w, *res_ln_b;
  int64_t res_ln_bstride;
  int splitk;
  int64_t kchunk;
  float* ws;
  int conv_h, conv_w, conv_c, conv_ho, conv_wo, conv_ks, conv_s, conv_pad;
  int64_t conv_in_bytes;
  const bf16* bn_x;
  const uint8_t* bn_mask;
  const float* bn_mean;
  const uint8_t* res_mask;
  float* cs_part;
  int64_t cs_m0;
  int cs_rows;
};
void conv3x3_wgrad_launch(const GemmParams& p, hipStream_t s);
void conv3x3_implicit_launch(const GemmParams& p, bool small, hipStream_t s);
struct StemParams {
  const bf16* X;
  const bf16* Wt;
  const bf16* dY;
  bf16* Y;
  int n, H, W, Ho, Wo, tiles_r, tiles_c;
  int64_t n_tiles;
};
void stem_fill_geometry(StemParams& p);
int64_t stem_wgrad_ws_floats(int64_t n_tiles);
void stem_fwd_launch(const StemParams& p, hipStream_t s);
void stem_wgrad_launch(const StemParams& p, float* dW, int accumulate, float* ws, hipStream_t s);

void splitk_reduce_launch(const GemmParams& p, int batch, hipStream_t s);
void gemm_launch(const GemmParams& p, bool a_kmajor, bool b_kmajor, bool f32out, bool big, int batch, hipStream_t s);
bool gemm_wide_launch(const GemmParams& p, bool f32out, int batch, hipStream_t s);
bool splitk_epilogue_launch(const GemmParams& p, bool f32out, const float* slabs, int64_t m_base, int64_t rows,
                            int splitk, hipStream_t s);
void transpose_bf16_batched_launch(const int64_t* jobs, int n_jobs, int64_t max_rows, int64_t max_cols,
                                   hipStream_t s);
void colsum_reduce_launch(const float* part, int64_t parts, int64_t N, float* out, int acc, hipStream_t s);
constexpr int COLSUM_MULTI = 4;
struct ColsumJobs {
  const float* part[COLSUM_MULTI];
  int64_t parts[COLSUM_MULTI];
  float* out[COLSUM_MULTI];
};
void colsum_reduce_multi_launch(const ColsumJobs& jobs, int n, int64_t N, int acc, hipStream_t s);
void colsum_bf16_launch(const bf16* X, int64_t M, int64_t N, int64_t ld, float* part, float* out, int acc,
                        hipStream_t s);

struct AttnParams {
  const bf16* qkv;
  int64_t ld_qkv;
  const float* keymask;
  const bf16* o;
  int64_t ld_o;
  const bf16* dout;
  int64_t ld_do;
  float* lse;
  float* delta;
  bf16* out;
  int64_t ld_out;
  uint64_t* dropmask;
  float* colsum;
  int batch, L, heads;
  float drop_p;
  uint64_t seed;
  const uint64_t* seed_off;
};
void attention_fwd_launch(const AttnParams& p, hipStream_t s);
void attention_bwd_launch(const AttnParams& p, hipStream_t s);

void layernorm_fwd_launch(const bf16* X, const float* w, const float* b, bf16* Y, float* mean, float* rstd,
                          int64_t rows, int64_t H, float eps, int64_t group_rows, int64_t pstride, hipStream_t s);
void layernorm_fwd32_launch(const float* X, const float* w, const float* b, bf16* Y, float* Y32, float* mean,
                            float* rstd, int64_t rows, int64_t H, float eps, int64_t group_rows, int64_t pstride,
                            hipStream_t s);
void layernorm_bwd_launch(const bf16* dY, const void* X, bool x_f32, const float* mean, const float* rstd,
                          const float* w, bf16* dX, bf16* dXdrop, const bf16* dR, float drop_p, uint64_t seed,
                          const uint64_t* seed_off, float* pdw, float* pdb, float* pdbias, int64_t rows, int64_t H,
                          int64_t rows_per_part, hipStream_t s);

struct SeqAttnParams {
  const bf16* qkv;
  int64_t ld_qkv;
  const bf16* o;
  int64_t ld_o;
  const bf16* dout;
  int64_t ld_do;
  bf16* out;
  int64_t ld_out;
  float* lse2;
  float* delta;
  int S, N, heads, E, D;
  float scale;
};
void seqattn_fwd_launch(const SeqAttnParams& p, hipStream_t s);
void seqattn_bwd_launch(const SeqAttnParams& p, hipStream_t s);

struct EmbedParams {
  const int64_t *ids, *seg, *txt_mask, *idx;
  const float *proj, *word, *pos, *type, *ln_w, *ln_b;
  float eps, drop_txt, drop_img;
  uint64_t seed;
  const uint64_t* seed_off;
  int64_t cls_id, sep_id, V, B, T, n_img, Lout, H;
  bf16* X;
  float* X32;
  float *keymask, *mean, *rstd;
};
void embed_fwd_launch(const EmbedParams& p, hipStream_t s);
struct EmbedBwdParams {
  const bf16* dX;
  const int64_t *ids, *seg;
  const float *proj, *word, *pos, *type, *ln_w, *mean, *rstd;
  int64_t cls_id, sep_id, B, T, n_img, H;
  float drop_txt, drop_img;
  uint64_t seed;
  const uint64_t* seed_off;
  float *d_word, *d_pos, *d_type, *d_ln_w, *d_ln_b, *d_proj, *ws;
};
void embed_bwd_launch(const EmbedBwdParams& p, hipStream_t s);
int64_t embed_bwd_blocks(int64_t B, int64_t S);
void image_normalize_launch(const uint8_t* in, int64_t n, const float* mean, const float* stdv, void* out,
                            bool out_bf16, hipStream_t s);
void maxpool3s2_fwd_launch(const bf16* x, int64_t B, int H, int W, int C, int OH, int OW, bf16* y, uint8_t* am,
                           hipStream_t s);
void maxpool3s2_bwd_launch(const bf16* dy, const uint8_t* am, int64_t B, int H, int W, int C, int OH, int OW,
                           bf16* dx, hipStream_t s);
void row_pool_fwd_launch(const bf16* fmap, int64_t B, int64_t Hh, int64_t Ww, int64_t C, int64_t n, float* out,
                         hipStream_t s);
void row_pool_bwd_launch(const float* dout, int64_t B, int64_t Hh, int64_t Ww, int64_t C, int64_t n, bf16* dfmap,
                         hipStream_t s);

struct AdamParams {
  float *params, *m, *v;
  const float* grads;
  bf16* bf16_copy;
  const int64_t* table;
  int32_t* steps;
  int64_t n_tensors, total;
  float lr_decay, lr_nodecay, wd, warmup, t_total, b1, b2, eps, max_grad_norm, grad_scale;
  float* ws;
  int64_t ws_floats;
};
int bertadam_launch(const AdamParams& p, hipStream_t s, const char** err);

struct BnFwdParams {
  const bf16 *X, *skip;
  bf16* Y;
  int64_t rows;
  int C;
  const float *w, *b;
  float *rmean, *rvar;
  int training, relu;
  float momentum, eps;
  float *smean, *sinvstd;
  int64_t* nbt;
  void* ws;
  uint8_t* mask;
  const int8_t* skip_res;
  int8_t* y_res;
  double* lsum;
  const double* gsum;
  const float* parts;
  int64_t nparts;
};
void batchnorm_fwd_launch(const BnFwdParams& q, hipStream_t s);
struct BnBwdParams {
  const bf16 *dY, *Y, *X;
  int64_t rows;
  int C;
  const float *w, *smean, *sinvstd;
  int relu;
  bf16 *dX, *dS;
  float *dw, *db;
  void* ws;
  const uint8_t* mask;
  double* lsum;
  const double* gsum;
  const float* parts;
  int64_t nparts;
};
void batchnorm_bwd_launch(const BnBwdParams& q, hipStream_t s);
int64_t batchnorm_ws_bytes(int64_t C);

void uncertainty_launch(const float* logits, const int64_t* y, int64_t S, int64_t R, int64_t C, float* p_bar,
                        float* nll, float* conf, float* correct, hipStream_t s);
void ece_bins_launch(const float* conf, const float* correct, int64_t S, int64_t n_bins, float* out, hipStream_t s);

}
```

multi-modal-uncertainty_amd/src/_native.py:

```python
import ctypes
import os

_HERE = os.path.dirname(os.path.abspath(__file__))
LIB_PATH = os.environ.get("MMU_LIB_PATH") or os.path.join(_HERE, "libmmu_hip.so")

c_i64, c_i32, c_f32, c_u64, c_vp = ctypes.c_int64, ctypes.c_int32, ctypes.c_float, ctypes.c_uint64, ctypes.c_void_p
c_f32p, c_i64p, c_dp = ctypes.POINTER(ctypes.c_float), ctypes.POINTER(ctypes.c_int64), ctypes.POINTER(ctypes.c_double)

MMU_BF16, MMU_F32 = 0, 1
(EPI_STORE, EPI_BIAS_GELU, EPI_BIAS_DROP_RES, EPI_DGELU, EPI_ADD_RES, EPI_BIAS_DROP_QGELU, EPI_STORE_STATS,
 EPI_STORE_BNB, EPI_ADD_RES_BNB) = range(9)


class Epilogue(ctypes.Structure):
    _fields_ = [("kind", c_i32), ("accumulate", c_i32), ("bias", c_vp), ("bias_bstride", c_i64),
                ("residual", c_vp), ("ldr", c_i64), ("res_bstride", c_i64), ("aux", c_vp), ("ldx", c_i64),
                ("aux_bstride", c_i64), ("colsum", c_vp), ("colsum_bstride", c_i64), ("drop_p", c_f32),
                ("seed", c_u64), ("workspace", c_vp), ("workspace_floats", c_i64), ("res_ln_mean", c_vp),
                ("res_ln_rstd", c_vp), ("res_ln_w", c_vp), ("res_ln_b", c_vp), ("res_ln_bstride", c_i64),
                ("bn_x", c_vp), ("bn_mask", c_vp), ("bn_mean", c_vp), ("res_mask", c_vp)]


SIGNATURES = {
    "mmu_version": (c_i32, []),
    "mmu_embed_bwd_ws_floats": (c_i64, [c_i64, c_i64, c_i64]),
    "mmu_last_error": (ctypes.c_char_p, []),
    "mmu_set_seed_offset": (c_i32, [c_vp]),
    "mmu_gemm": (c_i32, [c_vp, c_i64, c_i32, c_vp, c_i64, c_i32, c_vp, c_i64, c_i32, c_i64, c_i64, c_i64,
                         c_i64, c_i64, c_i64, c_i64, ctypes.POINTER(Epilogue), c_vp]),
    "mmu_colsum_reduce": (c_i32, [c_vp, c_i64, c_i64, c_vp, c_i32, c_vp]),
    "mmu_colsum_reduce_multi": (c_i32, [c_i32, c_vp, c_vp, c_vp, c_i64, c_i32, c_vp]),
    "mmu_colsum_bf16": (c_i32, [c_vp, c_i64, c_i64, c_i64, c_vp, c_vp, c_i32, c_vp]),
    "mmu_transpose_bf16_batched": (c_i32, [c_vp, c_i32, c_i64, c_i64, c_vp]),
    "mmu_attention_fwd": (c_i32, [c_vp, c_i64, c_vp, c_vp, c_i64, c_vp, c_i64, c_i64, c_i64, c_f32, c_u64, c_vp,
                                  c_vp]),
    "mmu_attention_bwd": (c_i32, [c_vp, c_i64, c_vp, c_vp, c_i64, c_vp, c_i64, c_vp, c_vp, c_vp, c_i64,
                                  c_i64, c_i64, c_i64, c_f32, c_u64, c_vp, c_vp, c_vp]),
    "mmu_layernorm_fwd": (c_i32, [c_vp, c_vp, c_vp, c_vp, c_vp, c_vp, c_i64, c_i64, c_f32, c_i64, c_i64, c_vp]),
    "mmu_layernorm_bwd": (c_i32, [c_vp, c_vp, c_vp, c_vp, c_vp, c_vp, c_vp, c_f32, c_u64, c_vp, c_vp, c_vp,
                                  c_i64, c_i64, c_i64, c_vp]),
    "mmu_layernorm_fwd_f32": (c_i32, [c_vp, c_vp, c_vp, c_vp, c_vp, c_vp, c_vp, c_i64, c_i64, c_f32, c_i64, c_i64,
                                      c_vp]),
    "mmu_layernorm_bwd_f32": (c_i32, [c_vp, c_vp, c_vp, c_vp, c_vp, c_vp, c_vp, c_f32, c_u64, c_vp, c_vp, c_vp,
                                      c_i64, c_i64, c_i64, c_vp]),
    "mmu_layernorm_bwd_res": (c_i32, [c_vp, c_vp, c_vp, c_vp, c_vp, c_vp, c_vp, c_vp, c_vp, c_vp, c_i64, c_i64,
                                      c_i64, c_vp]),
    "mmu_seqattn_fwd": (c_i32, [c_vp, c_i64, c_vp, c_i64, c_vp, c_i64, c_i64, c_i64, c_i64, c_vp]),
    "mmu_seqattn_bwd": (c_i32, [c_vp, c_i64, c_vp, c_i64, c_vp, c_i64, c_vp, c_vp, c_vp, c_i64, c_i64, c_i64, c_i64,
                                c_i64, c_vp]),
    "mmu_embed_fwd": (c_i32, [c_vp, c_vp, c_vp, c_vp, c_vp, c_vp, c_vp, c_vp, c_vp, c_f32, c_i64, c_i64, c_vp,
                              c_i64, c_i64, c_i64, c_i64, c_i64, c_i64, c_f32, c_f32, c_u64, c_vp, c_vp, c_vp, c_vp,
                              c_vp, c_vp]),
    "mmu_embed_bwd": (c_i32, [c_vp, c_vp, c_vp, c_vp, c_vp, c_vp, c_vp, c_vp, c_vp, c_vp, c_i64, c_i64, c_i64,
                              c_i64, c_i64, c_i64, c_f32, c_f32, c_u64, c_vp, c_vp, c_vp, c_vp, c_vp, c_vp, c_vp,
                              c_vp]),
    "mmu_image_normalize": (c_i32, [c_vp, c_i64, c_f32p, c_f32p, c_vp, c_i32, c_vp]),
    "mmu_maxpool_fwd": (c_i32, [c_vp, c_i64, c_i64, c_i64, c_i64, c_vp, c_vp, c_vp]),
    "mmu_maxpool_bwd": (c_i32, [c_vp, c_vp, c_i64, c_i64, c_i64, c_i64, c_vp, c_vp]),
    "mmu_row_pool_fwd": (c_i32, [c_vp, c_i64, c_i64, c_i64, c_i64, c_i64, c_vp, c_vp]),
    "mmu_row_pool_bwd": (c_i32, [c_vp, c_i64, c_i64, c_i64, c_i64, c_i64, c_vp, c_vp]),
    "mmu_conv3x3_implicit": (c_i32, [c_vp, c_vp, c_vp, c_i64, c_i64, c_i64, c_i64, c_i64, c_vp, c_i64, c_vp]),
    "mmu_conv3x3_implicit_bnb": (c_i32, [c_vp, c_vp, c_vp, c_i64, c_i64, c_i64, c_i64, c_i64, c_vp, c_vp, c_vp,
                                         c_vp, c_vp, c_i64, c_vp]),
    "mmu_conv3x3_wgrad": (c_i32, [c_vp, c_vp, c_vp, c_i64, c_i64, c_i64, c_i64, c_i64, c_i32, c_vp, c_i64, c_vp]),
    "mmu_conv_implicit": (c_i32, [c_vp, c_vp, c_vp, c_i64, c_i64, c_i64, c_i64, c_i64, c_i64, c_i64, c_vp, c_i64,
                                  c_vp]),
    "mmu_conv_implicit_stats": (c_i32, [c_vp, c_vp, c_vp, c_i64, c_i64, c_i64, c_i64, c_i64, c_i64, c_i64, c_vp, c_vp,
                                        c_i64, c_vp]),
    "mmu_conv_wgrad": (c_i32, [c_vp, c_vp, c_vp, c_i64, c_i64, c_i64, c_i64, c_i64, c_i64, c_i64, c_i32, c_vp, c_i64,
                               c_vp]),
    "mmu_stem_conv_fwd": (c_i32, [c_vp, c_vp, c_vp, c_i64, c_i64, c_i64, c_vp]),
    "mmu_stem_conv_wgrad_ws_floats": (c_i64, [c_i64, c_i64, c_i64]),
    "mmu_stem_conv_wgrad": (c_i32, [c_vp, c_vp, c_vp, c_i64, c_i64, c_i64, c_i32, c_vp, c_i64, c_vp]),
    "mmu_batchnorm_ws_bytes": (c_i64, [c_i64]),
    "mmu_batchnorm_fwd": (c_i32, [c_vp, c_vp, c_vp, c_i64, c_i64, c_vp, c_vp, c_vp, c_vp, c_vp, c_i32, c_f32,
                                  c_f32, c_i32, c_vp, c_vp, c_vp, c_vp, c_vp, c_vp, c_i64, c_vp]),
    "mmu_batchnorm_bwd": (c_i32, [c_vp, c_vp, c_vp, c_vp, c_i64, c_i64, c_vp, c_vp, c_vp, c_i32, c_vp, c_vp,
                                  c_vp, c_vp, c_vp, c_i64, c_vp]),
    "mmu_batchnorm_bwd_parts": (c_i32, [c_vp, c_vp, c_vp, c_vp, c_i64, c_i64, c_vp, c_i64, c_vp, c_vp, c_vp, c_i32,
                                        c_vp, c_vp, c_vp, c_vp, c_vp, c_i64, c_vp]),
    "mmu_batchnorm_stats": (c_i32, [c_vp, c_i64, c_i64, c_vp, c_vp, c_i64, c_vp]),
    "mmu_batchnorm_fwd_sums": (c_i32, [c_vp, c_vp, c_vp, c_i64, c_i64, c_vp, c_vp, c_vp, c_vp, c_vp, c_vp, c_f32,
                                       c_f32, c_i32, c_vp, c_vp, c_vp, c_vp, c_vp, c_vp, c_i64, c_vp]),
    "mmu_batchnorm_fwd_parts": (c_i32, [c_vp, c_vp, c_vp, c_i64, c_i64, c_vp, c_i64, c_vp, c_vp, c_vp, c_vp, c_vp,
                                        c_f32, c_f32, c_i32, c_vp, c_vp, c_vp, c_vp, c_vp, c_vp, c_i64, c_vp]),
    "mmu_batchnorm_bwd_reduce": (c_i32, [c_vp, c_vp, c_vp, c_vp, c_i64, c_i64, c_vp, c_vp, c_i32, c_vp, c_vp, c_vp,
                                         c_vp, c_i64, c_vp]),
    "mmu_batchnorm_bwd_sums": (c_i32, [c_vp, c_vp, c_vp, c_vp, c_i64, c_i64, c_vp, c_vp, c_vp, c_vp, c_i32, c_vp,
                                       c_vp, c_vp, c_i64, c_vp]),
    "mmu_bertadam_step": (c_i32, [c_vp, c_vp, c_vp, c_vp, c_vp, c_vp, c_vp, c_i64, c_i64, c_f32, c_f32, c_f32,
                                  c_f32, c_f32, c_f32, c_f32, c_f32, c_f32, c_f32, c_vp, c_i64, c_vp]),
    "mmu_uncertainty": (c_i32, [c_vp, c_vp, c_i64, c_i64, c_i64, c_vp, c_vp, c_vp, c_vp, c_vp]),
    "mmu_ece_bins": (c_i32, [c_vp, c_vp, c_i64, c_i64, c_vp, c_vp]),
    "mmu_timing_enable": (c_i32, [c_i32]),
    "mmu_timing_pause": (c_i32, [c_i32]),
    "mmu_timing_read": (c_i32, [c_dp, c_i64p, c_dp]),
}

_lib = None


class NativeError(RuntimeError):
    pass


ABI_VERSION = 4


def load():
    global _lib
    if _lib is None:
        if not os.path.exists(LIB_PATH):
            raise NativeError(f"libmmu_hip.so not built at {LIB_PATH}: run `python -c 'import __graft_entry__ as g; "
                              f"g.build()'` (hipcc --offload-arch=gfx950)")
        import torch
        if torch.cuda.is_available():
            torch.cuda.init()
        lib = ctypes.CDLL(LIB_PATH)
        for name, (res, args) in SIGNATURES.items():
            fn = getattr(lib, name)
            fn.restype, fn.argtypes = res, args
        if lib.mmu_version() != ABI_VERSION:
            raise NativeError(f"libmmu_hip.so ABI {lib.mmu_version()} != {ABI_VERSION} (include/mmu.h "
                              "MMU_ABI_VERSION): rebuild the library")
        _lib = lib
    return _lib


def call(name, *args):
    rc = getattr(load(), name)(*args)
    if rc != 0:
        raise NativeError(f"{name}: {load().mmu_last_error().decode()}")
    return rc


def last_error():
    return load().mmu_last_error().decode()
```

multi-modal-uncertainty_amd/src/encoder.py:

```python

import os

import torch

from . import kernels as K

HID, FFN, HEADS = 768, 3072, 12
bf16 = torch.bfloat16


class LayerWeights:

    def __init__(self, store, prefix, layer_module):
        self.store, self.prefix, self.module = store, prefix, layer_module
        q = [f"{prefix}attention.self.{n}.weight" for n in ("query", "key", "value")]
        qb = [f"{prefix}attention.self.{n}.bias" for n in ("query", "key", "value")]
        self._names = dict(
            wqkv=q, bqkv=qb,
            wo=[f"{prefix}attention.output.dense.weight"], bo=[f"{prefix}attention.output.dense.bias"],
            ln1w=[f"{prefix}attention.output.LayerNorm.weight"], ln1b=[f"{prefix}attention.output.LayerNorm.bias"],
            w1=[f"{prefix}intermediate.dense.weight"], b1=[f"{prefix}intermediate.dense.bias"],
            w2=[f"{prefix}output.dense.weight"], b2=[f"{prefix}output.dense.bias"],
            ln2w=[f"{prefix}output.LayerNorm.weight"], ln2b=[f"{prefix}output.LayerNorm.bias"])
        self._shapes = dict(wqkv=(3 * HID, HID), bqkv=(3 * HID,), wo=(HID, HID), bo=(HID,), ln1w=(HID,), ln1b=(HID,),
                            w1=(FFN, HID), b1=(FFN,), w2=(HID, FFN), b2=(HID,), ln2w=(HID,), ln2b=(HID,))
        self.refresh()

    def refresh(self):
        s = self.store
        for k, names in self._names.items():
            setattr(self, k, s.fused(names, self._shapes[k]))
            setattr(self, "g_" + k, s.fused_grad(names, self._shapes[k]))
        for k in ("wqkv", "wo", "w1", "w2"):
            setattr(self, k + "16", s.fused_compute(self._names[k], self._shapes[k]))
        for k in ("wqkv", "wo", "w1", "w2"):
            setattr(self, k + "t16", s.transposed_compute(self._names[k], self._shapes[k]))
        self.anchor = s.params[self._names["wqkv"][0]]

    def trainable(self):
        return self.anchor.requires_grad


def layer_forward(lw, X, R, keymask, B, L, p_attn, p_hid, seeds, save, res_ln=None, out32=False):
    M = B * L
    dev = X.device
    f32 = torch.float32
    qkv = torch.empty(M, 3 * HID, dtype=bf16, device=dev)
    K.gemm(X, HID, True, lw.wqkv16, HID, True, qkv, 3 * HID, M, 3 * HID, HID, epi=K.epilogue(K.EPI_STORE, bias=lw.bqkv))
    O = torch.empty(M, HID, dtype=bf16, device=dev)
    lse = torch.empty(B * HEADS, L, dtype=torch.float32, device=dev)
    dmask = K.dropmask_empty(B, L, HEADS, dev) if (save and p_attn > 0) else None
    K.attention_fwd(qkv, keymask, O, lse, B, L, HEADS, p_attn, seeds[0], dmask)
    S1 = torch.empty(M, HID, dtype=f32, device=dev)
    K.gemm(O, HID, True, lw.wo16, HID, True, S1, HID, M, HID, HID,
           epi=K.epilogue(K.EPI_BIAS_DROP_RES, bias=lw.bo, residual=R, drop_p=p_hid, seed=seeds[1], res_ln=res_ln))
    A = torch.empty(M, HID, dtype=bf16, device=dev)
    mean1 = torch.empty(M, dtype=f32, device=dev)
    rstd1 = torch.empty(M, dtype=f32, device=dev)
    K.layernorm_fwd_f32(S1, lw.ln1w, lw.ln1b, A, None, mean1, rstd1)
    Z = torch.empty(M, FFN, dtype=bf16, device=dev) if save else None
    Hh = torch.empty(M, FFN, dtype=bf16, device=dev)
    K.gemm(A, HID, True, lw.w116, HID, True, Hh, FFN, M, FFN, HID, epi=K.epilogue(K.EPI_BIAS_GELU, bias=lw.b1, aux=Z))
    S2 = torch.empty(M, HID, dtype=f32, device=dev)
    K.gemm(Hh, FFN, True, lw.w216, FFN, True, S2, HID, M, HID, FFN,
           epi=K.epilogue(K.EPI_BIAS_DROP_RES, bias=lw.b2, residual=S1, drop_p=p_hid, seed=seeds[2],
                          res_ln=(mean1, rstd1, lw.ln1w, lw.ln1b)))
    Y = torch.empty(M, HID, dtype=bf16, device=dev)
    Y32 = torch.empty(M, HID, dtype=f32, device=dev) if out32 is True else None
    mean2 = torch.empty(M, dtype=f32, device=dev)
    rstd2 = torch.empty(M, dtype=f32, device=dev)
    K.layernorm_fwd_f32(S2, lw.ln2w, lw.ln2b, Y, Y32, mean2, rstd2)
    if out32 == "cls":
        S2c = S2.view(B, L, HID)[:, 0].contiguous()
        Y32 = torch.empty(B, HID, dtype=f32, device=dev)
        K.layernorm_fwd_f32(S2c, lw.ln2w, lw.ln2b, torch.empty(B, HID, dtype=bf16, device=dev), Y32)
    saved = (X, qkv, O, lse, dmask, S1, mean1, rstd1, A, Z, Hh, S2, mean2, rstd2) if save else None
    return Y, S2, mean2, rstd2, saved, Y32


def encoder_stack(lws, X, X32, keymask, B, L, p_attn, p_hid, seeds_of, need_grad, hook=None, all_layers=False,
                  cls_only=False):
    R, rln, outs = X32, None, []
    n = len(lws)
    for i, lw in enumerate(lws):
        out32 = all_layers or i == n - 1
        if out32 and cls_only and not all_layers:
            out32 = "cls"
        if need_grad:
            X, R, mu, rs, Y32 = BertLayerFunction.apply(X, R, lw.anchor, lw, keymask, B, L, p_attn, p_hid,
                                                        seeds_of(i), hook, rln, out32, i == 0)
        else:
            X, R, mu, rs, _, Y32 = layer_forward(lw, X, R, keymask, B, L, p_attn, p_hid, seeds_of(i), False, rln,
                                                 out32)
        rln = (mu, rs, lw.ln2w, lw.ln2b)
        if out32:
            outs.append(Y32)
    return outs if all_layers else outs[-1]


DEFER_WGRAD = True
DEFER_MAX_BYTES = None

_deferred = {}
_deferred_bytes = {}


def _defer_budget(dev):
    if DEFER_MAX_BYTES is not None:
        return DEFER_MAX_BYTES
    return torch.cuda.get_device_properties(dev).total_memory // 4


INTERLEAVE = os.environ.get("MMU_WGRAD_INTERLEAVE", "2") != "0"
INTERLEAVE_ALL = os.environ.get("MMU_WGRAD_INTERLEAVE", "2") == "2"
_pending = {}


def _issue(dev, items):
    side = K.side_stream(dev)
    with torch.cuda.stream(side):
        e0 = _mark()
        for fn, tensors in items:
            for t in tensors:
                t.record_stream(side)
            fn()
        if e0 is not None:
            _block_extra.append((e0, _mark()))


def _flush_deferred(dev, interleave=False):
    items = _deferred.pop(dev, None)
    _deferred_bytes.pop(dev, None)
    if not items:
        return
    main = torch.cuda.current_stream(dev)
    side = K.side_stream(dev)
    side.wait_stream(main)
    if interleave:
        _pending.setdefault(dev, []).extend(items)
    else:
        _issue(dev, items)
    K.join_at_backward_end(main, side)


def pump_deferred(dev, n=1):
    items = _pending.get(dev)
    if items:
        if INTERLEAVE_ALL:
            K.side_stream(dev).wait_stream(torch.cuda.current_stream(dev))
            n = len(items)
        _pending[dev] = items[n:]
        _issue(dev, items[:n])


K.set_side_pump(pump_deferred)


def _defer(dev, fn, tensors):
    items = _deferred.get(dev)
    if items is None:
        items = _deferred[dev] = []

        def at_end():
            if dev in _deferred:
                _flush_deferred(dev)
            if _pending.get(dev):
                _issue(dev, _pending.pop(dev))
            torch.cuda.current_stream(dev).wait_stream(K.side_stream(dev))

        torch.autograd.Variable._execution_engine.queue_callback(at_end)
    items.append((fn, tensors))
    held = _deferred_bytes.get(dev, 0) + sum(t.numel() * t.element_size() for t in tensors)
    _deferred_bytes[dev] = held
    if held > _defer_budget(dev):
        _flush_deferred(dev)


class _Side:

    def __init__(self, dev, on):
        self.dev = dev
        self.defer = on and DEFER_WGRAD and dev.type == "cuda"

    def run(self, fn, *tensors):
        if self.defer:
            return _defer(self.dev, fn, tensors)
        return fn()


def layer_backward(lw, saved, dY, keymask, B, L, p_attn, p_hid, seeds, wgrad):
    X, qkv, O, lse, dmask, S1, mean1, rstd1, A, Z, Hh, S2, mean2, rstd2 = saved
    M = B * L
    dev = dY.device
    P = K.ln_parts(M)
    side = _Side(dev, wgrad)
    pw = pb = pbias = pw1 = pb1 = pbias1 = None
    if wgrad:
        pw, pb, pbias, pw1, pb1, pbias1 = (torch.empty(P, HID, dtype=torch.float32, device=dev) for _ in range(6))
    acc = K.epilogue(K.EPI_STORE, accumulate=True)
    dS2 = torch.empty(M, HID, dtype=bf16, device=dev)
    dY2 = torch.empty(M, HID, dtype=bf16, device=dev)
    K.layernorm_bwd(dY, S2, mean2, rstd2, lw.ln2w, dS2, dY2, p_hid, seeds[2], pw, pb, pbias)
    if wgrad:
        def w2():
            K.colsum_reduce_multi([(pw, lw.g_ln2w), (pb, lw.g_ln2b), (pbias, lw.g_b2)], accumulate=True)
            K.gemm(dY2, HID, False, Hh, FFN, False, lw.g_w2, FFN, HID, FFN, M, epi=acc)
        side.run(w2, pw, pb, pbias, dY2, Hh)
    dZ = torch.empty(M, FFN, dtype=bf16, device=dev)
    K.gemm(dY2, HID, True, lw.w2t16, HID, True, dZ, FFN, M, FFN, HID,
           epi=K.epilogue(K.EPI_DGELU, aux=Z, colsum=lw.g_b1 if wgrad else None))
    if wgrad:
        side.run(lambda: K.gemm(dZ, FFN, False, A, HID, False, lw.g_w1, HID, FFN, HID, M, epi=acc), dZ, A)
    dA = torch.empty(M, HID, dtype=bf16, device=dev)
    K.gemm(dZ, FFN, True, lw.w1t16, FFN, True, dA, HID, M, HID, FFN, epi=K.epilogue(K.EPI_ADD_RES, residual=dS2))
    dS1 = torch.empty(M, HID, dtype=bf16, device=dev)
    dAo = torch.empty(M, HID, dtype=bf16, device=dev)
    K.layernorm_bwd(dA, S1, mean1, rstd1, lw.ln1w, dS1, dAo, p_hid, seeds[1], pw1, pb1, pbias1)
    if wgrad:
        def wo():
            K.colsum_reduce_multi([(pw1, lw.g_ln1w), (pb1, lw.g_ln1b), (pbias1, lw.g_bo)], accumulate=True)
            K.gemm(dAo, HID, False, O, HID, False, lw.g_wo, HID, HID, HID, M, epi=acc)
        side.run(wo, pw1, pb1, pbias1, dAo, O)
    dO = torch.empty(M, HID, dtype=bf16, device=dev)
    K.gemm(dAo, HID, True, lw.wot16, HID, True, dO, HID, M, HID, HID)
    dqkv = torch.empty(M, 3 * HID, dtype=bf16, device=dev)
    delta = torch.empty(B * HEADS, L, dtype=torch.float32, device=dev)
    dbp = K.attention_dbias_parts(B, L, HEADS, dev) if wgrad else None
    K.attention_bwd(qkv, keymask, O, dO, lse, delta, dqkv, B, L, HEADS, p_attn, seeds[0], dmask, dbp)
    if wgrad:
        def wqkv():
            K.attention_dbias_reduce(dbp, B, L, lw.g_bqkv, HEADS)
            K.gemm(dqkv, 3 * HID, False, X, HID, False, lw.g_wqkv, HID, 3 * HID, HID, M, epi=acc)
        side.run(wqkv, dqkv, X, dbp)
    dX = torch.empty(M, HID, dtype=bf16, device=dev)
    K.gemm(dqkv, 3 * HID, True, lw.wqkvt16, 3 * HID, True, dX, HID, M, HID, 3 * HID,
           epi=K.epilogue(K.EPI_ADD_RES, residual=dS1))
    return dX, side


_block_events = None
_block_extra = []


def block_timing(on):
    global _block_events, _block_extra
    _block_events = [] if on else None
    _block_extra = []


def block_timing_read():
    if not _block_events:
        return 0.0, 0
    torch.cuda.synchronize()
    ms = sum(a.elapsed_time(b) for a, b in _block_events) + sum(a.elapsed_time(b) for a, b in _block_extra)
    return ms, len(_block_events)


def _mark():
    if _block_events is None:
        return None
    e = torch.cuda.Event(enable_timing=True)
    e.record()
    return e


class BertLayerFunction(torch.autograd.Function):

    @staticmethod
    def forward(ctx, X, R, anchor, lw, keymask, B, L, p_attn, p_hid, seeds, on_grads_ready, res_ln=None,
                out32=True, flush=False):
        ctx.set_materialize_grads(False)
        e0 = _mark()
        Y, S2, mean2, rstd2, saved, Y32 = layer_forward(lw, X, R, keymask, B, L, p_attn, p_hid, seeds, True,
                                                        res_ln, out32)
        if e0 is not None:
            _block_events.append((e0, _mark()))
        ctx.saved_bufs = saved
        ctx.meta = (lw, keymask, B, L, p_attn, p_hid, seeds, on_grads_ready, flush)
        ctx.mark_non_differentiable(S2, mean2, rstd2)
        if Y32 is None:
            Y32 = Y.new_empty(0, dtype=torch.float32)
            ctx.mark_non_differentiable(Y32)
        return Y, S2, mean2, rstd2, Y32

    @staticmethod
    def backward(ctx, dY, _dS2, _dmean2, _drstd2, dY32):
        lw, keymask, B, L, p_attn, p_hid, seeds, hook, flush = ctx.meta
        wgrad = lw.trainable()
        if dY32 is not None and dY32.numel():
            if dY32.shape[0] == B and B * L != B:
                g = torch.zeros(B * L, HID, dtype=bf16, device=dY32.device) if dY is None else dY.clone()
                g.view(B, L, HID)[:, 0] += dY32.to(bf16)
                dY = g
            else:
                dY = dY32.to(bf16) if dY is None else dY + dY32.to(bf16)
        if dY is None:
            return (None,) * 14
        e0 = _mark()
        dX, side = layer_backward(lw, ctx.saved_bufs, dY.contiguous(), keymask, B, L, p_attn, p_hid, seeds, wgrad)
        if e0 is not None:
            _block_events.append((e0, _mark()))
        ctx.saved_bufs = None
        if wgrad and side.defer:
            if hook is not None:
                _defer(side.dev, lambda: hook(lw), ())
            if flush:
                _flush_deferred(side.dev, INTERLEAVE)
        elif wgrad and hook is not None:
            hook(lw)
        return (dX,) + (None,) * 13
```

multi-modal-uncertainty_amd/src/kernels.py:

```python
import ctypes

import torch

from . import _native as N
from ._native import (Epilogue, EPI_STORE, EPI_BIAS_GELU, EPI_BIAS_DROP_RES, EPI_DGELU, EPI_ADD_RES,
                      EPI_BIAS_DROP_QGELU, EPI_STORE_STATS, EPI_STORE_BNB, EPI_ADD_RES_BNB)


def bn_stats_table(rows, C, device):
    nparts = (rows + 63) // 64
    return torch.empty(nparts * C * 2, dtype=torch.float32, device=device), nparts


def _dev_check(*ts):
    for t in ts:
        if t is not None and not t.is_cuda:
            raise N.NativeError("mmu kernels need tensors on a HIP (cuda) device; got CPU tensor "
                                f"{tuple(t.shape)} {t.dtype}")


_raw_stream = torch._C._cuda_getCurrentRawStream


def _stream(t):
    return _raw_stream(t.get_device())


def _ptr(t):
    return None if t is None else t.data_ptr()


def _want(t, dtype, name):
    if t.dtype != dtype:
        raise N.NativeError(f"{name}: expected {dtype}, got {t.dtype}")


def epilogue(kind=EPI_STORE, bias=None, residual=None, aux=None, colsum=None, drop_p=0.0, seed=0, accumulate=False,
             ldr=0, ldx=0, bias_bstride=0, res_bstride=0, aux_bstride=0, colsum_bstride=0, res_ln=None,
             res_ln_bstride=0, bn=None, res_mask=None):
    e = Epilogue()
    e.kind, e.accumulate = kind, int(accumulate)
    e.bias, e.bias_bstride = _ptr(bias), bias_bstride
    e.residual, e.ldr, e.res_bstride = _ptr(residual), ldr or (residual.shape[-1] if residual is not None else 0), \
        res_bstride
    e.aux, e.ldx, e.aux_bstride = _ptr(aux), ldx or (aux.shape[-1] if aux is not None else 0), aux_bstride
    e.colsum, e.colsum_bstride = _ptr(colsum), colsum_bstride
    e.drop_p, e.seed = float(drop_p), int(seed) & 0xFFFFFFFFFFFFFFFF
    e.workspace, e.workspace_floats = None, 0
    if res_ln is not None:
        for t in res_ln:
            _want(t, torch.float32, "epilogue res_ln")
            if not t.is_contiguous():
                raise N.NativeError("epilogue res_ln tensors must be contiguous")
        e.res_ln_mean, e.res_ln_rstd, e.res_ln_w, e.res_ln_b = (_ptr(t) for t in res_ln)
        e.res_ln_bstride = res_ln_bstride
    if bn is not None:
        _bnb_check(*bn, "epilogue bn")
        e.bn_x, e.bn_mask, e.bn_mean = (_ptr(t) for t in bn)
    if res_mask is not None:
        if res_mask.dtype != torch.uint8 or not res_mask.is_contiguous() or residual is None \
                or res_mask.numel() * 8 != residual.numel():
            raise N.NativeError("epilogue res_mask: contiguous uint8 with numel = residual.numel() / 8")
        e.res_mask = _ptr(res_mask)
    return e


def _bnb_check(x, mask, mean, what):
    if (x.dtype != torch.bfloat16 or mean.dtype != torch.float32 or not mean.is_contiguous()
            or mean.numel() != x.shape[1] or not x.is_contiguous(memory_format=torch.channels_last)):
        raise N.NativeError(f"{what}: (x channels-last bf16, relu_mask, mean f32 [C]) of a training BatchNorm")
    _bn_mask_check(mask, x, what)


SPLITK_WS_FLOATS = 16 << 20
_ws = {}
_side = {}


def _splitk_workspace(dev):
    key = (dev, _raw_stream(dev.index if dev.index is not None else torch.cuda.current_device()))
    t = _ws.get(key)
    if t is None:
        t = _ws[key] = torch.empty(SPLITK_WS_FLOATS, dtype=torch.float32, device=dev)
    return t


SIDE_CU_FRAC = None


def _cu_masked_stream(dev, frac):
    import ctypes
    n_cu = torch.cuda.get_device_properties(dev).multi_processor_count
    groups = n_cu // 8
    keep = max(1, min(groups, round(frac * groups)))
    bits = [0] * ((n_cu + 31) // 32)
    for g in range(groups):
        if (g + 1) * keep // groups != g * keep // groups:
            for c in range(8 * g, 8 * g + 8):
                bits[c // 32] |= 1 << (c % 32)
    hip = ctypes.CDLL("libamdhip64.so.7")
    h = ctypes.c_void_p()
    arr = (ctypes.c_uint32 * len(bits))(*bits)
    with torch.cuda.device(dev):
        err = hip.hipExtStreamCreateWithCUMask(ctypes.byref(h), ctypes.c_uint32(len(bits)), arr)
    if err != 0:
        raise N.NativeError(f"hipExtStreamCreateWithCUMask failed ({err})")
    return torch.cuda.ExternalStream(h.value, device=dev)


def side_stream(dev):
    dev = torch.device(dev)
    s = _side.get(dev)
    if s is None:
        s = _side[dev] = (_cu_masked_stream(dev, SIDE_CU_FRAC) if SIDE_CU_FRAC
                          else torch.cuda.Stream(device=dev))
    return s


_side_pump = None


def set_side_pump(fn):
    global _side_pump
    _side_pump = fn


def side_pump(dev, n=1):
    if _side_pump is not None:
        _side_pump(dev, n)


def side_stream_if_any(dev):
    return _side.get(torch.device(dev))


_pending_join = set()


def join_at_backward_end(main, side):
    key = (main.cuda_stream, side.cuda_stream)
    if key in _pending_join:
        return
    _pending_join.add(key)

    def join():
        _pending_join.discard(key)
        main.wait_stream(side)

    torch.autograd.Variable._execution_engine.queue_callback(join)


def gemm(A, lda, a_kmajor, B, ldb, b_kmajor, C, ldc, M, N_, K, epi=None, batch=1, sA=0, sB=0, sC=0):
    _dev_check(A, B, C)
    _want(A, torch.bfloat16, "gemm A")
    _want(B, torch.bfloat16, "gemm B")
    cdt = N.MMU_F32 if C.dtype == torch.float32 else N.MMU_BF16
    if C.dtype not in (torch.float32, torch.bfloat16):
        raise N.NativeError("gemm C must be f32 or bf16")
    if epi is None:
        epi = epilogue(EPI_STORE)
    if not epi.workspace:
        epi = type(epi).from_buffer_copy(epi)
        ws = _splitk_workspace(C.device)
        epi.workspace, epi.workspace_floats = ws.data_ptr(), ws.numel()
    N.call("mmu_gemm", _ptr(A), lda, int(a_kmajor), _ptr(B), ldb, int(b_kmajor), _ptr(C), ldc, cdt, M, N_, K,
           batch, sA, sB, sC, ctypes.byref(epi) if epi is not None else None, _stream(C))
    if _alg["on"]:
        _count_alg(M, N_, K, batch, 4 if cdt == N.MMU_F32 else 2, epi)
    return C


def colsum_reduce_multi(jobs, accumulate=False):
    n = len(jobs)
    N_ = jobs[0][0].shape[1]
    for part, out in jobs:
        _dev_check(part, out)
        if part.dtype != torch.float32 or out.dtype != torch.float32 or part.shape[1] != N_ or out.numel() != N_ \
                or not part.is_contiguous() or not out.is_contiguous():
            raise N.NativeError("colsum_reduce_multi: f32 contiguous [parts, N] partials / [N] outputs of one N")
    parts_p = (ctypes.c_void_p * n)(*[p.data_ptr() for p, _ in jobs])
    rows = (ctypes.c_int64 * n)(*[p.shape[0] for p, _ in jobs])
    outs = (ctypes.c_void_p * n)(*[o.data_ptr() for _, o in jobs])
    N.call("mmu_colsum_reduce_multi", n, ctypes.cast(parts_p, ctypes.c_void_p), ctypes.cast(rows, ctypes.c_void_p),
           ctypes.cast(outs, ctypes.c_void_p), N_, int(accumulate), _stream(jobs[0][1]))


def colsum_reduce(partial, out, accumulate=False):
    _dev_check(partial, out)
    N.call("mmu_colsum_reduce", _ptr(partial), partial.shape[0], partial.shape[1], _ptr(out), int(accumulate),
           _stream(out))


def transpose_bf16_batched(jobs, n_jobs, max_rows, max_cols, stream_of):
    _dev_check(jobs, stream_of)
    if jobs.dtype != torch.int64 or not jobs.is_contiguous() or jobs.numel() < 6 * n_jobs:
        raise N.NativeError("transpose_bf16_batched: jobs must be a contiguous int64 [n_jobs, 6] device table")
    N.call("mmu_transpose_bf16_batched", _ptr(jobs), int(n_jobs), int(max_rows), int(max_cols), _stream(stream_of))


def colsum_bf16(X, out, accumulate=False):
    _dev_check(X, out)
    M, N_ = X.shape
    part = torch.empty(((M + 63) // 64) * N_, dtype=torch.float32, device=X.device)
    N.call("mmu_colsum_bf16", _ptr(X), M, N_, X.stride(0), _ptr(part), _ptr(out), int(accumulate), _stream(X))


def dropmask_empty(batch, L, heads=12, device=None):
    return torch.empty(batch * heads, L, (L + 63) // 64, dtype=torch.int64, device=device)


def dropmask_dense(mask, L):
    bits = torch.arange(64, device=mask.device, dtype=torch.int64)
    d = (mask.unsqueeze(-1) >> bits) & 1
    return d.flatten(-2)[..., :L].float()


def attention_fwd(qkv, keymask, O, lse, batch, L, heads=12, drop_p=0.0, seed=0, dropmask=None):
    _dev_check(qkv, keymask, O, lse)
    _want(qkv, torch.bfloat16, "attention qkv")
    if dropmask is not None:
        _dev_check(dropmask)
        if dropmask.numel() < batch * heads * L * ((L + 63) // 64) or not dropmask.is_contiguous():
            raise ValueError("attention_fwd: dropmask too small / not contiguous")
    N.call("mmu_attention_fwd", _ptr(qkv), qkv.stride(0), _ptr(keymask), _ptr(O), O.stride(0), _ptr(lse), batch, L,
           heads, float(drop_p), int(seed), _ptr(dropmask) if dropmask is not None else None, _stream(qkv))


def attention_dbias_parts(batch, L, heads=12, device=None):
    nqb, nkb = (L + 127) // 128, (L + 63) // 64
    return torch.empty((nqb + 2 * nkb) * batch, heads * 64, dtype=torch.float32, device=device)


def attention_dbias_reduce(parts, batch, L, g_bqkv, heads=12):
    nqb, nkb = (L + 127) // 128, (L + 63) // 64
    H = heads * 64
    r0, r1 = nqb * batch, (nqb + nkb) * batch
    colsum_reduce_multi([(parts[:r0], g_bqkv[:H]), (parts[r0:r1], g_bqkv[H:2 * H]), (parts[r1:], g_bqkv[2 * H:])],
                        accumulate=True)


def attention_bwd(qkv, keymask, O, dO, lse, delta, dqkv, batch, L, heads=12, drop_p=0.0, seed=0, dropmask=None,
                  dbias_parts=None):
    _dev_check(qkv, keymask, O, dO, lse, delta, dqkv)
    if dropmask is not None:
        _dev_check(dropmask)
        if dropmask.numel() < batch * heads * L * ((L + 63) // 64) or not dropmask.is_contiguous():
            raise ValueError("attention_bwd: dropmask too small / not contiguous")
    N.call("mmu_attention_bwd", _ptr(qkv), qkv.stride(0), _ptr(keymask), _ptr(O), O.stride(0), _ptr(dO), dO.stride(0),
           _ptr(lse), _ptr(delta), _ptr(dqkv), dqkv.stride(0), batch, L, heads, float(drop_p), int(seed),
           _ptr(dropmask) if dropmask is not None else None, _ptr(dbias_parts), _stream(qkv))


LN_ROWS_PER_PART = 64


def ln_parts(rows):
    return (rows + LN_ROWS_PER_PART - 1) // LN_ROWS_PER_PART


def _ln_rows(who, X, x_dtype, same=(), vecs=(), parts=()):
    if X.dim() != 2 or not X.is_contiguous():
        raise N.NativeError(f"{who}: X must be a contiguous 2-D [rows, H] tensor, got {tuple(X.shape)}")
    _want(X, x_dtype, f"{who} X")
    rows, H = X.shape
    for name, t in same:
        if t is None:
            continue
        _want(t, torch.bfloat16, f"{who} {name}")
        if t.shape != X.shape or not t.is_contiguous():
            raise N.NativeError(f"{who}: {name} must be contiguous [{rows}, {H}] like X, got {tuple(t.shape)}")
    for name, t in vecs:
        if t is None:
            continue
        _want(t, torch.float32, f"{who} {name}")
        if t.numel() < rows or not t.is_contiguous():
            raise N.NativeError(f"{who}: {name} must hold >= {rows} contiguous elements, got {t.numel()}")
    need = ln_parts(rows) * H
    for name, t in parts:
        if t is None:
            continue
        _want(t, torch.float32, f"{who} {name}")
        if t.numel() < need or not t.is_contiguous():
            raise N.NativeError(f"{who}: {name} must hold >= ln_parts(rows) x H = {need} contiguous elements, "
                                f"got {t.numel()}")
    return rows, H


def _ln_params(who, rows, H, group_rows, param_stride, **params):
    group_rows, param_stride = int(group_rows), int(param_stride)
    groups = 1
    if group_rows > 0:
        if rows % group_rows:
            raise N.NativeError(f"{who}: rows = {rows} is no multiple of group_rows = {group_rows}")
        groups = rows // group_rows
    if param_stride < 0:
        raise N.NativeError(f"{who}: bad param_stride {param_stride}")
    need = (groups - 1) * param_stride + H
    for name, t in params.items():
        _want(t, torch.float32, f"{who} {name}")
        if t.numel() < need or not t.is_contiguous():
            raise N.NativeError(f"{who}: {name} must hold (groups - 1) * param_stride + H = {need} contiguous "
                                f"elements, got {t.numel()}")


def layernorm_fwd(X, w, b, Y, mean, rstd, eps=1e-12, group_rows=0, param_stride=0):
    rows, H = _ln_rows("layernorm_fwd", X, torch.bfloat16, same=(("Y", Y),), vecs=(("mean", mean), ("rstd", rstd)))
    _ln_params("layernorm_fwd", rows, H, group_rows, param_stride, w=w, b=b)
    _dev_check(X, w, b, Y, mean, rstd)
    N.call("mmu_layernorm_fwd", _ptr(X), _ptr(w), _ptr(b), _ptr(Y), _ptr(mean), _ptr(rstd), rows, H, float(eps),
           int(group_rows), int(param_stride), _stream(X))


def layernorm_fwd_f32(X, w, b, Y, Y32=None, mean=None, rstd=None, eps=1e-12, group_rows=0, param_stride=0):
    rows, H = _ln_rows("layernorm_fwd_f32", X, torch.float32, same=(("Y", Y),),
                       vecs=(("mean", mean), ("rstd", rstd)))
    if Y32 is not None:
        _want(Y32, torch.float32, "layernorm_fwd_f32 Y32")
        if Y32.shape != X.shape or not Y32.is_contiguous():
            raise N.NativeError(f"layernorm_fwd_f32: Y32 must be contiguous [{rows}, {H}] like X, got "
                                f"{tuple(Y32.shape)}")
    _ln_params("layernorm_fwd_f32", rows, H, group_rows, param_stride, w=w, b=b)
    _dev_check(X, w, b, Y, Y32, mean, rstd)
    N.call("mmu_layernorm_fwd_f32", _ptr(X), _ptr(w), _ptr(b), _ptr(Y), _ptr(Y32), _ptr(mean), _ptr(rstd), rows, H,
           float(eps), int(group_rows), int(param_stride), _stream(X))


def layernorm_bwd(dY, X, mean, rstd, w, dX, dXdrop=None, drop_p=0.0, seed=0, part_dw=None, part_db=None,
                  part_dbias=None):
    x32 = X.dtype == torch.float32
    rows, H = _ln_rows("layernorm_bwd", X, torch.float32 if x32 else torch.bfloat16,
                       same=(("dY", dY), ("dX", dX), ("dXdrop", dXdrop)), vecs=(("mean", mean), ("rstd", rstd)),
                       parts=(("part_dw", part_dw), ("part_db", part_db), ("part_dbias", part_dbias)))
    _ln_params("layernorm_bwd", rows, H, 0, 0, w=w)
    _dev_check(dY, X, mean, rstd, w, dX, dXdrop, part_dw, part_db, part_dbias)
    N.call("mmu_layernorm_bwd_f32" if x32 else "mmu_layernorm_bwd", _ptr(dY), _ptr(X), _ptr(mean), _ptr(rstd),
           _ptr(w), _ptr(dX), _ptr(dXdrop), float(drop_p), int(seed), _ptr(part_dw), _ptr(part_db), _ptr(part_dbias),
           rows, H, LN_ROWS_PER_PART, _stream(X))


def layernorm_bwd_res(dY, X, mean, rstd, w, dRes, dX, part_dw=None, part_db=None, part_dbias=None):
    rows, H = _ln_rows("layernorm_bwd_res", X, torch.bfloat16, same=(("dY", dY), ("dRes", dRes), ("dX", dX)),
                       vecs=(("mean", mean), ("rstd", rstd)),
                       parts=(("part_dw", part_dw), ("part_db", part_db), ("part_dbias", part_dbias)))
    _ln_params("layernorm_bwd_res", rows, H, 0, 0, w=w)
    _dev_check(dY, X, mean, rstd, w, dRes, dX, part_dw, part_db, part_dbias)
    N.call("mmu_layernorm_bwd_res", _ptr(dY), _ptr(X), _ptr(mean), _ptr(rstd), _ptr(w), _ptr(dRes), _ptr(dX),
           _ptr(part_dw), _ptr(part_db), _ptr(part_dbias), rows, H, LN_ROWS_PER_PART, _stream(X))


def seqattn_fwd(qkv, O, lse2, S, N_, heads):
    _dev_check(qkv, O, lse2)
    _want(qkv, torch.bfloat16, "seqattn qkv")
    D = qkv.shape[1] // (3 * heads)
    if lse2.numel() < S * N_ * heads:
        raise ValueError("seqattn_fwd: lse2 too small")
    N.call("mmu_seqattn_fwd", _ptr(qkv), qkv.stride(0), _ptr(O), O.stride(0), _ptr(lse2), S, N_, heads, D,
           _stream(qkv))


def seqattn_bwd(qkv, O, dO, lse2, delta, dqkv, S, N_, heads):
    _dev_check(qkv, O, dO, lse2, delta, dqkv)
    D = qkv.shape[1] // (3 * heads)
    if delta.numel() < S * N_ * heads:
        raise ValueError("seqattn_bwd: delta too small")
    N.call("mmu_seqattn_bwd", _ptr(qkv), qkv.stride(0), _ptr(O), O.stride(0), _ptr(dO), dO.stride(0), _ptr(lse2),
           _ptr(delta), _ptr(dqkv), dqkv.stride(0), S, N_, heads, D, _stream(qkv))


def _embed_common(who, ids, seg, proj, word, pos, typ, ln_w, cls_id, sep_id, B, T, n_img):
    B, T, n_img = int(B), int(T), int(n_img)
    for name, t in (("ids", ids), ("seg", seg)):
        _want(t, torch.int64, f"{who} {name}")
        if tuple(t.shape) != (B, T) or not t.is_contiguous():
            raise N.NativeError(f"{who}: {name} must be contiguous int64 [B, T] = [{B}, {T}], got {tuple(t.shape)}")
    _want(proj, torch.float32, f"{who} proj")
    if tuple(proj.shape) != (B, n_img, 768) or not proj.is_contiguous():
        raise N.NativeError(f"{who}: proj must be contiguous f32 [B, n_img, 768] = [{B}, {n_img}, 768], got "
                            f"{tuple(proj.shape)}")
    for name, t in (("word", word), ("pos", pos), ("typ", typ)):
        _want(t, torch.float32, f"{who} {name}")
        if t.dim() != 2 or t.shape[1] != 768 or not t.is_contiguous():
            raise N.NativeError(f"{who}: {name} must be a contiguous f32 [n, 768] table, got {tuple(t.shape)}")
    _want(ln_w, torch.float32, f"{who} ln_w")
    if ln_w.numel() != 768 or not ln_w.is_contiguous():
        raise N.NativeError(f"{who}: ln_w must hold 768 contiguous elements, got {ln_w.numel()}")
    if max(n_img + 2, T) > pos.shape[0]:
        raise N.NativeError(f"{who}: max(n_img + 2, T) = {max(n_img + 2, T)} exceeds the {pos.shape[0]} position rows")
    if not (0 <= int(cls_id) < word.shape[0] and 0 <= int(sep_id) < word.shape[0]):
        raise N.NativeError(f"{who}: cls_id / sep_id = {cls_id} / {sep_id} outside the {word.shape[0]} word rows")
    if typ.shape[0] < 2:
        raise N.NativeError(f"{who}: typ must hold >= 2 token-type rows, got {typ.shape[0]}")


def embed_fwd(ids, seg, txt_mask, proj, word, pos, typ, ln_w, ln_b, eps, cls_id, sep_id, idx, V, B, T, n_img, Lout,
              X, keymask, mean=None, rstd=None, drop_txt=0.0, drop_img=0.0, seed=0, X32=None):
    who = "embed_fwd"
    _embed_common(who, ids, seg, proj, word, pos, typ, ln_w, cls_id, sep_id, B, T, n_img)
    rows = int(V) * int(B) * int(Lout)
    if txt_mask is not None:
        _want(txt_mask, torch.int64, f"{who} txt_mask")
        if tuple(txt_mask.shape) != (B, T) or not txt_mask.is_contiguous():
            raise N.NativeError(f"{who}: txt_mask must be contiguous int64 [B, T] = [{B}, {T}], got "
                                f"{tuple(txt_mask.shape)}")
    _want(ln_b, torch.float32, f"{who} ln_b")
    if ln_b.numel() != 768 or not ln_b.is_contiguous():
        raise N.NativeError(f"{who}: ln_b must hold 768 contiguous elements, got {ln_b.numel()}")
    if idx is not None:
        _want(idx, torch.int64, f"{who} idx")
        if tuple(idx.shape) != (V, Lout) or not idx.is_contiguous():
            raise N.NativeError(f"{who}: idx must be contiguous int64 [V, Lout] = [{V}, {Lout}], got "
                                f"{tuple(idx.shape)}")
    for name, t, dt in (("X", X, torch.bfloat16), ("X32", X32, torch.float32)):
        if t is None:
            continue
        _want(t, dt, f"{who} {name}")
        if tuple(t.shape) != (rows, 768) or not t.is_contiguous():
            raise N.NativeError(f"{who}: {name} must be contiguous [V * B * Lout, 768] = [{rows}, 768], got "
                                f"{tuple(t.shape)}")
    for name, t in (("keymask", keymask), ("mean", mean), ("rstd", rstd)):
        if t is None:
            continue
        _want(t, torch.float32, f"{who} {name}")
        if t.numel() < rows or not t.is_contiguous():
            raise N.NativeError(f"{who}: {name} must hold >= V * B * Lout = {rows} contiguous elements, got "
                                f"{t.numel()}")
    _dev_check(ids, seg, txt_mask, idx, proj, word, pos, typ, ln_w, ln_b, X, X32, keymask, mean, rstd)
    N.call("mmu_embed_fwd", _ptr(ids), _ptr(seg), _ptr(txt_mask), _ptr(proj), _ptr(word), _ptr(pos), _ptr(typ),
           _ptr(ln_w), _ptr(ln_b), float(eps), int(cls_id), int(sep_id), _ptr(idx), V, B, T, n_img, Lout, 768,
           float(drop_txt), float(drop_img), int(seed), _ptr(X), _ptr(X32), _ptr(keymask), _ptr(mean), _ptr(rstd),
           _stream(X))


def embed_bwd(dX, ids, seg, proj, word, pos, typ, ln_w, mean, rstd, cls_id, sep_id, B, T, n_img, d_word, d_pos,
              d_type, d_ln_w, d_ln_b, d_proj, drop_txt=0.0, drop_img=0.0, seed=0):
    who = "embed_bwd"
    _embed_common(who, ids, seg, proj, word, pos, typ, ln_w, cls_id, sep_id, B, T, n_img)
    rows = int(B) * (int(n_img) + 2 + int(T))
    _want(dX, torch.bfloat16, f"{who} dX")
    if tuple(dX.shape) != (rows, 768) or not dX.is_contiguous():
        raise N.NativeError(f"{who}: dX must be contiguous bf16 [B * (n_img + 2 + T), 768] = [{rows}, 768], got "
                            f"{tuple(dX.shape)}")
    for name, t in (("mean", mean), ("rstd", rstd)):
        _want(t, torch.float32, f"{who} {name}")
        if t.numel() < rows or not t.is_contiguous():
            raise N.NativeError(f"{who}: {name} must hold >= {rows} contiguous elements, got {t.numel()}")
    for name, t, like in (("d_word", d_word, word), ("d_pos", d_pos, pos), ("d_type", d_type, typ),
                          ("d_ln_w", d_ln_w, ln_w), ("d_ln_b", d_ln_b, ln_w), ("d_proj", d_proj, proj)):
        _want(t, torch.float32, f"{who} {name}")
        if t.shape != like.shape or not t.is_contiguous():
            raise N.NativeError(f"{who}: {name} must be contiguous f32 {tuple(like.shape)} like its parameter, got "
                                f"{tuple(t.shape)}")
    _dev_check(dX, ids, seg, proj, word, pos, typ, ln_w, mean, rstd, d_word, d_pos, d_type, d_ln_w, d_ln_b, d_proj)
    ws = torch.empty(N.load().mmu_embed_bwd_ws_floats(B, T, n_img), dtype=torch.float32, device=dX.device)
    N.call("mmu_embed_bwd", _ptr(dX), _ptr(ids), _ptr(seg), _ptr(proj), _ptr(word), _ptr(pos), _ptr(typ),
           _ptr(ln_w), _ptr(mean), _ptr(rstd), int(cls_id), int(sep_id), B, T, n_img, 768, float(drop_txt),
           float(drop_img), int(seed), _ptr(d_word),
           _ptr(d_pos), _ptr(d_type), _ptr(d_ln_w), _ptr(d_ln_b), _ptr(d_proj), _ptr(ws), _stream(dX))


def image_normalize(img_u8, mean, std, out):
    _dev_check(img_u8, out)
    _want(img_u8, torch.uint8, "image_normalize input")
    if not img_u8.is_contiguous() or img_u8.shape[-1] != 3:
        raise N.NativeError("image_normalize: input must be contiguous [B, H, W, 3] uint8")
    if out.dtype not in (torch.float32, torch.bfloat16) or out.numel() != img_u8.numel() or \
            not out.is_contiguous(memory_format=torch.channels_last):
        raise N.NativeError("image_normalize: out must be a channels-last f32/bf16 [B, 3, H, W] of the same size")
    m = (ctypes.c_float * 3)(*[float(v) for v in mean])
    s = (ctypes.c_float * 3)(*[float(v) for v in std])
    N.call("mmu_image_normalize", _ptr(img_u8), img_u8.numel(), m, s, _ptr(out),
           N.MMU_F32 if out.dtype == torch.float32 else N.MMU_BF16, _stream(out))
    return out


def maxpool_fwd(x, y, argmax):
    _dev_check(x, y, argmax)
    B, C, H, W = x.shape
    _maxpool_check(x, y, argmax, B, C, H, W, "x", "y")
    N.call("mmu_maxpool_fwd", _ptr(x), B, H, W, C, _ptr(y), _ptr(argmax), _stream(x))


def maxpool_bwd(dy, argmax, dx):
    _dev_check(dy, argmax, dx)
    B, C, H, W = dx.shape
    _maxpool_check(dx, dy, argmax, B, C, H, W, "dx", "dy")
    N.call("mmu_maxpool_bwd", _ptr(dy), _ptr(argmax), B, H, W, C, _ptr(dx), _stream(dx))

# ... 378 lines not shown
```

Baseline: 1616.

## Compute only the CLS row through the final encoder layer

Adds a last-layer path for when only the CLS output is needed. The final layer's attention computes a single query row per batch and head, using new row-0 forward and backward kernels, and the output projection, FFN and LayerNorm run on the CLS rows only. New row-stepped GEMM and LayerNorm-backward entry points keep the dropout RNG indexing identical to the full-sequence layout so results stay consistent. This removes roughly L-1 of L rows of work from the last layer's post-attention compute, at the cost of extra code paths and a dependence on matching the dropout masks exactly.

```diff
diff --git a/include/mmu.h b/include/mmu.h
--- a/include/mmu.h
+++ b/include/mmu.h
@@ -60,6 +60,14 @@
              int64_t batch, int64_t strideA, int64_t strideB, int64_t strideC,
              const mmu_epilogue* epi, mmu_stream_t stream);
 
+int mmu_gemm_rows(const void* A, int64_t lda, int a_kmajor,
+                  const void* B, int64_t ldb, int b_kmajor,
+                  void* C, int64_t ldc, int c_dtype,
+                  int64_t M, int64_t N, int64_t K,
+                  int64_t batch, int64_t strideA, int64_t strideB, int64_t strideC,
+                  const mmu_epilogue* epi, int64_t drop_row_step, int64_t drop_row_offset,
+                  mmu_stream_t stream);
+
 int mmu_colsum_reduce(const float* partial, int64_t parts, int64_t N, float* out,
                       int accumulate, mmu_stream_t stream);
 int mmu_colsum_reduce_multi(int n, const float* const* partial, const int64_t* parts, float* const* out, int64_t N,
@@ -81,6 +89,17 @@
                       float drop_p, uint64_t seed, const uint64_t* dropmask, float* dbias_parts,
                       mmu_stream_t stream);
 
+int mmu_attention_row0_fwd(const void* QKV, int64_t ld_qkv, const float* keymask,
+                           void* O, int64_t ld_o, float* LSE,
+                           int64_t batch, int64_t L, int64_t heads,
+                           float drop_p, uint64_t seed, uint64_t* dropmask, mmu_stream_t stream);
+int mmu_attention_row0_bwd(const void* QKV, int64_t ld_qkv, const float* keymask,
+                           const void* O, int64_t ld_o, const void* dO, int64_t ld_do,
+                           const float* LSE, void* dQKV, int64_t ld_dqkv,
+                           int64_t batch, int64_t L, int64_t heads,
+                           float drop_p, const uint64_t* dropmask, float* dbias_sums,
+                           mmu_stream_t stream);
+
 int mmu_layernorm_fwd(const void* X, const float* w, const float* b, void* Y,
                       float* mean, float* rstd, int64_t rows, int64_t H, float eps,
                       int64_t group_rows, int64_t param_stride, mmu_stream_t stream);
@@ -96,6 +115,12 @@
                           const float* w, void* dX, void* dXdrop, float drop_p, uint64_t seed,
                           float* part_dw, float* part_db, float* part_dbias,
                           int64_t rows, int64_t H, int64_t rows_per_part, mmu_stream_t stream);
+
+int mmu_layernorm_bwd_f32_rows(const void* dY, const float* X, const float* mean, const float* rstd,
+                               const float* w, void* dX, void* dXdrop, float drop_p, uint64_t seed,
+                               float* part_dw, float* part_db, float* part_dbias,
+                               int64_t rows, int64_t H, int64_t rows_per_part,
+                               int64_t drop_row_step, int64_t drop_row_offset, mmu_stream_t stream);
 
 int mmu_layernorm_bwd_res(const void* dY, const void* X, const float* mean, const float* rstd,
                           const float* w, const void* dRes, void* dX,
diff --git a/multi-modal-uncertainty_amd/csrc/attention.hip b/multi-modal-uncertainty_amd/csrc/attention.hip
--- a/multi-modal-uncertainty_amd/csrc/attention.hip
+++ b/multi-modal-uncertainty_amd/csrc/attention.hip
@@ -734,4 +734,207 @@
     hipLaunchKernelGGL(attn_dkdv_dma_kernel<false>, dim3((p.L + 63) / 64, p.batch * p.heads), dim3(128), 0, s, p);
 }
 
-}
+constexpr int R0_GROUPS = 32;
+
+static __device__ __forceinline__ void ld8f(const bf16* p, float (&o)[8]) {
+  const uint4 u = *(const uint4*)p;
+  const bf16x8 v = *(const bf16x8*)&u;
+#pragma unroll
+  for (int j = 0; j < 8; ++j) o[j] = bf2f(v[j]);
+}
+static __device__ __forceinline__ float dot8(const float (&a)[8], const float (&b)[8]) {
+  float s = 0.f;
+#pragma unroll
+  for (int j = 0; j < 8; ++j) s = fmaf(a[j], b[j], s);
+  return s;
+}
+static __device__ __forceinline__ float sum8(float v) {
+  v += __shfl_xor(v, 1, 64);
+  v += __shfl_xor(v, 2, 64);
+  v += __shfl_xor(v, 4, 64);
+  return v;
+}
+template <bool MAX>
+static __device__ __forceinline__ float block_red(float v, float* red, int t) {
+  v = MAX ? wave_max(v) : wave_sum(v);
+  __syncthreads();
+  if ((t & 63) == 0) red[t >> 6] = v;
+  __syncthreads();
+  return MAX ? fmaxf(fmaxf(red[0], red[1]), fmaxf(red[2], red[3])) : (red[0] + red[1]) + (red[2] + red[3]);
+}
+static __device__ __forceinline__ uint32_t pair_draw_rt(uint32_t hb, int i) {
+  uint32_t mul = kDropMul24[0];
+#pragma unroll
+  for (int e = 1; e < 8; ++e) mul = i == e ? kDropMul24[e] : mul;
+  const uint32_t x = __umul24(__builtin_amdgcn_alignbit(hb, hb, 4 * i), mul);
+  return x ^ (x >> 16);
+}
+
+template <bool DROP>
+__global__ __launch_bounds__(256) void attn_row0_fwd_kernel(AttnParams p) {
+  __shared__ float sp[FWD_MAX_NKV * 64];
+  __shared__ float part[R0_GROUPS][64];
+  __shared__ float red[4];
+  const int t = threadIdx.x, c = t & 7, g = t >> 3;
+  const int bh = blockIdx.x, b = bh / p.heads, hd = bh - b * p.heads;
+  const int L = p.L, HD = p.heads * 64, nkv = (L + 63) / 64;
+  const bf16* rows = p.qkv + (int64_t)b * L * p.ld_qkv + hd * 64 + 8 * c;
+  const float* mask = p.keymask + (int64_t)b * L;
+  float q[8];
+  ld8f(rows, q);
+#pragma unroll
+  for (int j = 0; j < 8; ++j) q[j] *= 0.125f;
+  for (int k0 = g; k0 < L; k0 += 4 * R0_GROUPS) {
+    float kk[4][8];
+#pragma unroll
+    for (int u = 0; u < 4; ++u) {
+      const int k = k0 + R0_GROUPS * u;
+      ld8f(rows + (int64_t)(k < L ? k : 0) * p.ld_qkv + HD, kk[u]);
+    }
+#pragma unroll
+    for (int u = 0; u < 4; ++u) {
+      const int k = k0 + R0_GROUPS * u;
+      const float s = sum8(dot8(q, kk[u]));
+      if (c == 0 && k < L) sp[k] = s + mask[k];
+    }
+  }
+  __syncthreads();
+  float mx = NEG_INF;
+  for (int k = t; k < L; k += 256) mx = fmaxf(mx, sp[k]);
+  mx = block_red<true>(mx, red, t);
+  const uint32_t thr = drop_thr(p.drop_p);
+  const uint32_t ctr = DROP ? seed_for(mmu_eff_seed(p.seed, p.seed_off), bh) : 0u;
+  float ls = 0.f;
+  for (int k = t; (k >> 6) < nkv; k += 256) {
+    const int j = k >> 6, ko = k & 63;
+    float e = 0.f;
+    if (k < L) {
+      e = __builtin_amdgcn_exp2f((sp[k] - mx) * LOG2E);
+      ls += e;
+    }
+    if (DROP) {
+      const int s2 = ko >> 5, h = (ko >> 4) & 1;
+      const uint32_t hsh = pair_draw_rt(lowbias32(ctr + 4u * (uint32_t)j + 2u * (uint32_t)h + (uint32_t)s2), (ko & 15) >> 1);
+      bool keep = (ko & 1) ? hsh >= (thr << 16) : (hsh & 0xFFFFu) >= thr;
+      if (s2 == 1 && L - 64 * j <= 32) keep = false;
+      const uint64_t word = __ballot(keep);
+      if (p.dropmask && ko == 0) p.dropmask[(int64_t)bh * L * nkv + j] = word;
+      if (!keep) e = 0.f;
+    }
+    if (k < L) sp[k] = e;
+  }
+  ls = block_red<false>(ls, red, t);
+  float acc[8];
+#pragma unroll
+  for (int j = 0; j < 8; ++j) acc[j] = 0.f;
+#pragma unroll 4
+  for (int k = g; k < L; k += R0_GROUPS) {
+    float v[8];
+    ld8f(rows + (int64_t)k * p.ld_qkv + 2 * HD, v);
+    const float pk = sp[k];
+#pragma unroll
+    for (int j = 0; j < 8; ++j) acc[j] = fmaf(pk, v[j], acc[j]);
+  }
+#pragma unroll
+  for (int j = 0; j < 8; ++j) part[g][8 * c + j] = acc[j];
+  __syncthreads();
+  if (t < 64) {
+    float o = 0.f;
+    for (int gg = 0; gg < R0_GROUPS; ++gg) o += part[gg][t];
+    const float inv = (DROP ? 1.0f / (1.0f - p.drop_p) : 1.0f) / ls;
+    p.out[(int64_t)b * L * p.ld_out + hd * 64 + t] = f2bf(o * inv);
+  }
+  if (t == 0) p.lse[(int64_t)bh * L] = mx + logf(ls);
+}
+
+template <bool DROP>
+__global__ __launch_bounds__(256) void attn_row0_bwd_kernel(AttnParams p) {
+  __shared__ float part[R0_GROUPS][64];
+  __shared__ float red[4];
+  __shared__ uint64_t kw[FWD_MAX_NKV];
+  const int t = threadIdx.x, c = t & 7, g = t >> 3;
+  const int bh = blockIdx.x, b = bh / p.heads, hd = bh - b * p.heads;
+  const int L = p.L, HD = p.heads * 64, nkv = (L + 63) / 64;
+  const bf16* rows = p.qkv + (int64_t)b * L * p.ld_qkv + hd * 64 + 8 * c;
+  bf16* drows = p.out + (int64_t)b * L * p.ld_out + hd * 64 + 8 * c;
+  const bf16* do0 = p.dout + (int64_t)b * L * p.ld_do + hd * 64;
+  const float* mask = p.keymask + (int64_t)b * L;
+  float q[8], dO[8], o[8];
+  ld8f(rows, q);
+  ld8f(do0 + 8 * c, dO);
+  ld8f(p.o + (int64_t)b * L * p.ld_o + hd * 64 + 8 * c, o);
+#pragma unroll
+  for (int j = 0; j < 8; ++j) q[j] *= 0.125f;
+  const float delta = sum8(dot8(dO, o));
+  const float nlse2 = -p.lse[(int64_t)bh * L] * LOG2E;
+  const float zs = DROP ? 1.0f / (1.0f - p.drop_p) : 1.0f;
+  if (DROP && t < nkv) kw[t] = p.dropmask[(int64_t)bh * L * nkv + t];
+  __syncthreads();
+  float dq[8];
+#pragma unroll
+  for (int j = 0; j < 8; ++j) dq[j] = 0.f;
+  float sds = 0.f, spd = 0.f;
+  for (int k0 = g; k0 < L; k0 += 2 * R0_GROUPS) {
+    float kk2[2][8], v2[2][8];
+#pragma unroll
+    for (int u = 0; u < 2; ++u) {
+      const int k = k0 + R0_GROUPS * u;
+      ld8f(rows + (int64_t)(k < L ? k : 0) * p.ld_qkv + HD, kk2[u]);
+      ld8f(rows + (int64_t)(k < L ? k : 0) * p.ld_qkv + 2 * HD, v2[u]);
+    }
+#pragma unroll
+    for (int u = 0; u < 2; ++u) {
+      const int k = k0 + R0_GROUPS * u;
+      const float(&kk)[8] = kk2[u];
+      const float s = sum8(dot8(q, kk)), dp = sum8(dot8(dO, v2[u]));
+      if (k < L) {
+        const float pr = __builtin_amdgcn_exp2f(fmaf(s + mask[k], LOG2E, nlse2));
+        const bool keep = !DROP || ((kw[k >> 6] >> (k & 63)) & 1ull);
+        const float pd = keep ? pr * zs : 0.f;
+        const float ds = fmaf(pd, dp, -pr * delta);
+        bf16x8 ok, ov;
+#pragma unroll
+        for (int j = 0; j < 8; ++j) {
+          ok[j] = f2bf(ds * q[j]);
+          ov[j] = f2bf(pd * dO[j]);
+          dq[j] = fmaf(ds, kk[j], dq[j]);
+        }
+        *(bf16x8*)(drows + (int64_t)k * p.ld_out + HD) = ok;
+        *(bf16x8*)(drows + (int64_t)k * p.ld_out + 2 * HD) = ov;
+        sds += ds;
+        spd += pd;
+      }
+    }
+  }
+#pragma unroll
+  for (int j = 0; j < 8; ++j) part[g][8 * c + j] = dq[j];
+  sds = block_red<false>(c == 0 ? sds : 0.f, red, t);
+  spd = block_red<false>(c == 0 ? spd : 0.f, red, t);
+  if (t < 64) {
+    float v = 0.f;
+    for (int gg = 0; gg < R0_GROUPS; ++gg) v += part[gg][t];
+    v *= 0.125f;
+    p.out[(int64_t)b * L * p.ld_out + hd * 64 + t] = f2bf(v);
+    if (p.colsum) {
+      const int64_t slab = (int64_t)p.batch * HD, at = (int64_t)b * HD + hd * 64 + t;
+      const float qt = bf2f(p.qkv[(int64_t)b * L * p.ld_qkv + hd * 64 + t]) * 0.125f;
+      p.colsum[at] = v;
+      p.colsum[slab + at] = sds * qt;
+      p.colsum[2 * slab + at] = spd * bf2f(do0[t]);
+    }
+  }
+}
+
+void attention_row0_fwd_launch(const AttnParams& p, hipStream_t s) {
+  const dim3 grid(p.batch * p.heads);
+  if (drop_thr(p.drop_p)) hipLaunchKernelGGL(attn_row0_fwd_kernel<true>, grid, dim3(256), 0, s, p);
+  else hipLaunchKernelGGL(attn_row0_fwd_kernel<false>, grid, dim3(256), 0, s, p);
+}
+
+void attention_row0_bwd_launch(const AttnParams& p, hipStream_t s) {
+  const dim3 grid(p.batch * p.heads);
+  if (drop_thr(p.drop_p)) hipLaunchKernelGGL(attn_row0_bwd_kernel<true>, grid, dim3(256), 0, s, p);
+  else hipLaunchKernelGGL(attn_row0_bwd_kernel<false>, grid, dim3(256), 0, s, p);
+}
+
+}
diff --git a/multi-modal-uncertainty_amd/csrc/capi.hip b/multi-modal-uncertainty_amd/csrc/capi.hip
--- a/multi-modal-uncertainty_amd/csrc/capi.hip
+++ b/multi-modal-uncertainty_amd/csrc/capi.hip
@@ -117,9 +117,10 @@
   return 0;
 }
 
-int mmu_gemm(const void* A, int64_t lda, int a_kmajor, const void* B, int64_t ldb, int b_kmajor, void* C,
-             int64_t ldc, int c_dtype, int64_t M, int64_t N, int64_t K, int64_t batch, int64_t strideA,
-             int64_t strideB, int64_t strideC, const mmu_epilogue* epi, mmu_stream_t stream) {
+static int gemm_impl(const void* A, int64_t lda, int a_kmajor, const void* B, int64_t ldb, int b_kmajor, void* C,
+                     int64_t ldc, int c_dtype, int64_t M, int64_t N, int64_t K, int64_t batch, int64_t strideA,
+                     int64_t strideB, int64_t strideC, const mmu_epilogue* epi, int64_t drop_row_step,
+                     int64_t drop_row_off, mmu_stream_t stream) {
   if (!A || !B || !C) return fail("mmu_gemm: null operand");
   if (M <= 0 || N <= 0 || K <= 0 || batch <= 0) return fail("mmu_gemm: bad shape M=%ld N=%ld K=%ld", M, N, K);
   if (N % 128) return fail("mmu_gemm: N=%ld must be a multiple of 128", N);
@@ -131,6 +132,7 @@
   p.A = (const bf16*)A; p.B = (const bf16*)B; p.C = C;
   p.lda = lda; p.ldb = ldb; p.ldc = ldc; p.M = M; p.N = N; p.K = K;
   p.sA = strideA; p.sB = strideB; p.sC = strideC;
+  p.drop_ldn = N * drop_row_step; p.drop_base = N * drop_row_off;
   const int64_t a_span = 2 * (a_kmajor ? (M + 256) * lda : (K + 64) * lda);
   const int64_t b_span = 2 * (b_kmajor ? (N + 256) * ldb : (K + 64) * ldb);
   const bool big = M >= 256 && N >= 256 && a_span < (1ll << 32) - 4096 && b_span < (1ll << 32) - 4096;
@@ -298,6 +300,22 @@
   return check_launch("mmu_gemm");
 }
 
+int mmu_gemm(const void* A, int64_t lda, int a_kmajor, const void* B, int64_t ldb, int b_kmajor, void* C,
+             int64_t ldc, int c_dtype, int64_t M, int64_t N, int64_t K, int64_t batch, int64_t strideA,
+             int64_t strideB, int64_t strideC, const mmu_epilogue* epi, mmu_stream_t stream) {
+  return gemm_impl(A, lda, a_kmajor, B, ldb, b_kmajor, C, ldc, c_dtype, M, N, K, batch, strideA, strideB, strideC, epi,
+                   1, 0, stream);
+}
+
+int mmu_gemm_rows(const void* A, int64_t lda, int a_kmajor, const void* B, int64_t ldb, int b_kmajor, void* C,
+                  int64_t ldc, int c_dtype, int64_t M, int64_t N, int64_t K, int64_t batch, int64_t strideA,
+                  int64_t strideB, int64_t strideC, const mmu_epilogue* epi, int64_t drop_row_step,
+                  int64_t drop_row_offset, mmu_stream_t stream) {
+  if (drop_row_step < 1 || drop_row_offset < 0) return fail("mmu_gemm_rows: drop_row_step >= 1, drop_row_offset >= 0");
+  return gemm_impl(A, lda, a_kmajor, B, ldb, b_kmajor, C, ldc, c_dtype, M, N, K, batch, strideA, strideB, strideC, epi,
+                   drop_row_step, drop_row_offset, stream);
+}
+
 int mmu_transpose_bf16_batched(const int64_t* jobs, int n_jobs, int64_t max_rows, int64_t max_cols,
                                mmu_stream_t stream) {
   if (!jobs || n_jobs <= 0 || n_jobs > 65535 || max_rows <= 0 || max_cols <= 0)
@@ -382,6 +400,44 @@
   return check_launch("mmu_attention_bwd");
 }
 
+int mmu_attention_row0_fwd(const void* QKV, int64_t ld_qkv, const float* keymask, void* O, int64_t ld_o, float* LSE,
+                           int64_t batch, int64_t L, int64_t heads, float drop_p, uint64_t seed, uint64_t* dropmask,
+                           mmu_stream_t stream) {
+  if (!QKV || !keymask || !O || !LSE) return fail("mmu_attention_row0_fwd: null pointer");
+  if (attn_common(ld_qkv, batch, L, heads, drop_p)) return 1;
+  if (ld_o < heads * 64 || ld_o % 8) return fail("mmu_attention_row0_fwd: bad ld_o");
+  if (((uintptr_t)QKV | (uintptr_t)O) & 15) return fail("mmu_attention_row0_fwd: QKV / O must be 16-B aligned");
+  AttnParams p{};
+  p.qkv = (const bf16*)QKV; p.ld_qkv = ld_qkv; p.keymask = keymask; p.out = (bf16*)O; p.ld_out = ld_o;
+  p.lse = LSE; p.batch = (int)batch; p.L = (int)L; p.heads = (int)heads; p.drop_p = drop_p; p.seed = seed;
+  p.seed_off = g_seed_off;
+  p.dropmask = dropmask;
+  attention_row0_fwd_launch(p, (hipStream_t)stream);
+  return check_launch("mmu_attention_row0_fwd");
+}
+
+int mmu_attention_row0_bwd(const void* QKV, int64_t ld_qkv, const float* keymask, const void* O, int64_t ld_o,
+                           const void* dO, int64_t ld_do, const float* LSE, void* dQKV, int64_t ld_dqkv,
+                           int64_t batch, int64_t L, int64_t heads, float drop_p, const uint64_t* dropmask,
+                           float* dbias_sums, mmu_stream_t stream) {
+  if (!QKV || !keymask || !O || !dO || !LSE || !dQKV) return fail("mmu_attention_row0_bwd: null pointer");
+  if ((uint32_t)(drop_p * 65536.0f + 0.5f) != 0 && !dropmask)
+    return fail("mmu_attention_row0_bwd: dropout needs the forward's dropmask");
+  if (attn_common(ld_qkv, batch, L, heads, drop_p)) return 1;
+  if (ld_dqkv < 3 * heads * 64 || ld_do < heads * 64 || ld_o < heads * 64 || ld_do % 8 || ld_o % 8 || ld_dqkv % 8)
+    return fail("mmu_attention_row0_bwd: bad ld");
+  if (((uintptr_t)QKV | (uintptr_t)O | (uintptr_t)dO | (uintptr_t)dQKV) & 15)
+    return fail("mmu_attention_row0_bwd: QKV / O / dO / dQKV must be 16-B aligned");
+  AttnParams p{};
+  p.qkv = (const bf16*)QKV; p.ld_qkv = ld_qkv; p.keymask = keymask; p.o = (const bf16*)O; p.ld_o = ld_o;
+  p.dout = (const bf16*)dO; p.ld_do = ld_do; p.lse = (float*)LSE; p.out = (bf16*)dQKV;
+  p.ld_out = ld_dqkv; p.batch = (int)batch; p.L = (int)L; p.heads = (int)heads; p.drop_p = drop_p;
+  p.dropmask = (uint64_t*)dropmask;
+  p.colsum = dbias_sums;
+  attention_row0_bwd_launch(p, (hipStream_t)stream);
+  return check_launch("mmu_attention_row0_bwd");
+}
+
 int mmu_layernorm_fwd(const void* X, const float* w, const float* b, void* Y, float* mean, float* rstd, int64_t rows,
                       int64_t H, float eps, int64_t group_rows, int64_t param_stride, mmu_stream_t stream) {
   if (!X || !w || !b || !Y) return fail("mmu_layernorm_fwd: null pointer");
@@ -427,6 +483,22 @@
   layernorm_bwd_launch((const bf16*)dY, X, true, mean, rstd, w, (bf16*)dX, (bf16*)dXdrop, nullptr, drop_p, seed,
                        g_seed_off, part_dw, part_db, part_dbias, rows, H, rows_per_part, (hipStream_t)stream);
   return check_launch("mmu_layernorm_bwd_f32");
+}
+
+int mmu_layernorm_bwd_f32_rows(const void* dY, const float* X, const float* mean, const float* rstd, const float* w,
+                               void* dX, void* dXdrop, float drop_p, uint64_t seed, float* part_dw, float* part_db,
+                               float* part_dbias, int64_t rows, int64_t H, int64_t rows_per_part,
+                               int64_t drop_row_step, int64_t drop_row_offset, mmu_stream_t stream) {
+  if (!dY || !X || !mean || !rstd || !w || !dX) return fail("mmu_layernorm_bwd_f32_rows: null pointer");
+  if (rows <= 0 || H <= 0 || H % 256 || H > 1024 || rows_per_part <= 0)
+    return fail("mmu_layernorm_bwd_f32_rows: bad shape");
+  if (drop_p < 0.f || drop_p >= 1.f) return fail("mmu_layernorm_bwd_f32_rows: drop_p out of range");
+  if (drop_row_step < 1 || drop_row_offset < 0)
+    return fail("mmu_layernorm_bwd_f32_rows: drop_row_step >= 1, drop_row_offset >= 0");
+  layernorm_bwd_launch((const bf16*)dY, X, true, mean, rstd, w, (bf16*)dX, (bf16*)dXdrop, nullptr, drop_p, seed,
+                       g_seed_off, part_dw, part_db, part_dbias, rows, H, rows_per_part, (hipStream_t)stream,
+                       drop_row_step, drop_row_offset);
+  return check_launch("mmu_layernorm_bwd_f32_rows");
 }
 
 int mmu_layernorm_bwd_res(const void* dY, const void* X, const float* mean, const float* rstd, const float* w,
diff --git a/multi-modal-uncertainty_amd/csrc/gemm.hip b/multi-modal-uncertainty_amd/csrc/gemm.hip
--- a/multi-modal-uncertainty_amd/csrc/gemm.hip
+++ b/multi-modal-uncertainty_amd/csrc/gemm.hip
@@ -171,7 +171,7 @@
   constexpr bool DRP = EPI == MMU_EPI_BIAS_DROP_RES || EPI == MMU_EPI_BIAS_DROP_QGELU;
   const int64_t x_l = XST ? m_l * p.ldx + n : 0;
   const int64_t s_l = EPI == MMU_EPI_STORE ? m_l * p.N + n : 0;
-  const int64_t q_l = DRP ? (z * p.M + m_l) * p.N + n : 0;
+  const int64_t q_l = DRP ? p.drop_base + (z * p.M + m_l) * p.drop_ldn + n : 0;
   const uint64_t seed = DRP && thr ? mmu_eff_seed(p.seed, p.seed_off) : 0;
   const bool res_ln = RES32 && p.res_ln_w != nullptr && !slab;
   float lw[8], lb[8];
@@ -283,7 +283,7 @@
       }
       void* cdst = OUT_F32 ? (void*)((float*)p.C + c_l + d * p.ldc) : (void*)((bf16*)p.C + c_l + d * p.ldc);
       epi_oct<EPI, OUT_F32>(p, cdst, (XST && aux) ? aux + x_l + d * p.ldx : nullptr,
-                            DRP ? (uint64_t)(q_l + d * p.N) >> 2 : 0, v, inf, scale, thr, seed);
+                            DRP ? (uint64_t)(q_l + d * p.drop_ldn) >> 2 : 0, v, inf, scale, thr, seed);
       if (want_cs) {
 #pragma unroll
         for (int e = 0; e < 8; ++e) cs[e] += v[e];
diff --git a/multi-modal-uncertainty_amd/csrc/layernorm.hip b/multi-modal-uncertainty_amd/csrc/layernorm.hip
--- a/multi-modal-uncertainty_amd/csrc/layernorm.hip
+++ b/multi-modal-uncertainty_amd/csrc/layernorm.hip
@@ -200,7 +200,8 @@
                                                      bf16* __restrict__ dXd, const bf16* __restrict__ dR,
                                                      float drop_p, uint64_t seed, const uint64_t* seed_off,
                                                      float* __restrict__ pdw, float* __restrict__ pdb,
-                                                     float* __restrict__ pdbias, int64_t rows, int rpp) {
+                                                     float* __restrict__ pdbias, int64_t rows, int rpp,
+                                                     int64_t drop_step, int64_t drop_off) {
   constexpr int H = 256 * NV, nv = NV;
   __shared__ float red[4][H];
   const int l = threadIdx.x & 63, wv = threadIdx.x >> 6;
@@ -262,7 +263,7 @@
         }
         *(bf16x4*)(dX + row * H + c) = bf16x4{f2bf(dx[0]), f2bf(dx[1]), f2bf(dx[2]), f2bf(dx[3])};
         if (dXd) {
-          uint32_t keep = thr ? mmu_keep4(mmu_eff_seed(seed, seed_off), (uint64_t)(row * H + c) >> 2, thr) : 0xFu;
+          uint32_t keep = thr ? mmu_keep4(mmu_eff_seed(seed, seed_off), (uint64_t)((row * drop_step + drop_off) * H + c) >> 2, thr) : 0xFu;
 #pragma unroll
           for (int e = 0; e < 4; ++e) dx[e] = ((keep >> e) & 1) ? dx[e] * scale : 0.f;
           *(bf16x4*)(dXd + row * H + c) = bf16x4{f2bf(dx[0]), f2bf(dx[1]), f2bf(dx[2]), f2bf(dx[3])};
@@ -343,10 +344,10 @@
 static void ln_bwd_launch_t(const bf16* dY, const XT* X, const float* mean, const float* rstd, const float* w,
                             bf16* dX, bf16* dXdrop, const bf16* dR, float drop_p, uint64_t seed,
                             const uint64_t* seed_off, float* pdw, float* pdb, float* pdbias, int64_t rows, int64_t H,
-                            int64_t rpp, hipStream_t s) {
+                            int64_t rpp, hipStream_t s, int64_t dstep, int64_t doff) {
   const dim3 g((unsigned)((rows + rpp - 1) / rpp));
 #define LNB(NV) hipLaunchKernelGGL((ln_bwd_kernel<NV, XT>), g, dim3(256), 0, s, dY, X, mean, rstd, w, dX, dXdrop, dR, \
-                                   drop_p, seed, seed_off, pdw, pdb, pdbias, rows, (int)rpp)
+                                   drop_p, seed, seed_off, pdw, pdb, pdbias, rows, (int)rpp, dstep, doff)
   switch (H / 256) {
     case 1: LNB(1); break;
     case 2: LNB(2); break;
@@ -359,13 +360,13 @@
 void layernorm_bwd_launch(const bf16* dY, const void* X, bool x_f32, const float* mean, const float* rstd,
                           const float* w, bf16* dX, bf16* dXdrop, const bf16* dR, float drop_p, uint64_t seed,
                           const uint64_t* seed_off, float* pdw, float* pdb, float* pdbias, int64_t rows, int64_t H,
-                          int64_t rpp, hipStream_t s) {
+                          int64_t rpp, hipStream_t s, int64_t dstep, int64_t doff) {
   if (x_f32)
     ln_bwd_launch_t(dY, (const float*)X, mean, rstd, w, dX, dXdrop, dR, drop_p, seed, seed_off, pdw, pdb, pdbias, rows,
-                    H, rpp, s);
+                    H, rpp, s, dstep, doff);
   else
     ln_bwd_launch_t(dY, (const bf16*)X, mean, rstd, w, dX, dXdrop, dR, drop_p, seed, seed_off, pdw, pdb, pdbias, rows,
-                    H, rpp, s);
-}
-
-}
+                    H, rpp, s, dstep, doff);
+}
+
+}
diff --git a/multi-modal-uncertainty_amd/csrc/mmu_internal.h b/multi-modal-uncertainty_amd/csrc/mmu_internal.h
--- a/multi-modal-uncertainty_amd/csrc/mmu_internal.h
+++ b/multi-modal-uncertainty_amd/csrc/mmu_internal.h
@@ -28,6 +28,7 @@
   float drop_p;
   uint64_t seed;
   const uint64_t* seed_off;
+  int64_t drop_base, drop_ldn;
   const float *res_ln_mean, *res_ln_rstd, *res_ln_w, *res_ln_b;
   int64_t res_ln_bstride;
   int splitk;
@@ -97,6 +98,8 @@
 };
 void attention_fwd_launch(const AttnParams& p, hipStream_t s);
 void attention_bwd_launch(const AttnParams& p, hipStream_t s);
+void attention_row0_fwd_launch(const AttnParams& p, hipStream_t s);
+void attention_row0_bwd_launch(const AttnParams& p, hipStream_t s);
 
 void layernorm_fwd_launch(const bf16* X, const float* w, const float* b, bf16* Y, float* mean, float* rstd,
                           int64_t rows, int64_t H, float eps, int64_t group_rows, int64_t pstride, hipStream_t s);
@@ -106,7 +109,7 @@
 void layernorm_bwd_launch(const bf16* dY, const void* X, bool x_f32, const float* mean, const float* rstd,
                           const float* w, bf16* dX, bf16* dXdrop, const bf16* dR, float drop_p, uint64_t seed,
                           const uint64_t* seed_off, float* pdw, float* pdb, float* pdbias, int64_t rows, int64_t H,
-                          int64_t rows_per_part, hipStream_t s);
+                          int64_t rows_per_part, hipStream_t s, int64_t drop_row_step = 1, int64_t drop_row_off = 0);
 
 struct SeqAttnParams {
   const bf16* qkv;
diff --git a/multi-modal-uncertainty_amd/src/_native.py b/multi-modal-uncertainty_amd/src/_native.py
--- a/multi-modal-uncertainty_amd/src/_native.py
+++ b/multi-modal-uncertainty_amd/src/_native.py
@@ -28,6 +28,14 @@
     "mmu_set_seed_offset": (c_i32, [c_vp]),
     "mmu_gemm": (c_i32, [c_vp, c_i64, c_i32, c_vp, c_i64, c_i32, c_vp, c_i64, c_i32, c_i64, c_i64, c_i64,
                          c_i64, c_i64, c_i64, c_i64, ctypes.POINTER(Epilogue), c_vp]),
+    "mmu_gemm_rows": (c_i32, [c_vp, c_i64, c_i32, c_vp, c_i64, c_i32, c_vp, c_i64, c_i32, c_i64, c_i64, c_i64,
+                              c_i64, c_i64, c_i64, c_i64, ctypes.POINTER(Epilogue), c_i64, c_i64, c_vp]),
+    "mmu_attention_row0_fwd": (c_i32, [c_vp, c_i64, c_vp, c_vp, c_i64, c_vp, c_i64, c_i64, c_i64, c_f32, c_u64, c_vp,
+                                       c_vp]),
+    "mmu_attention_row0_bwd": (c_i32, [c_vp, c_i64, c_vp, c_vp, c_i64, c_vp, c_i64, c_vp, c_vp, c_i64,
+                                       c_i64, c_i64, c_i64, c_f32, c_vp, c_vp, c_vp]),
+    "mmu_layernorm_bwd_f32_rows": (c_i32, [c_vp, c_vp, c_vp, c_vp, c_vp, c_vp, c_vp, c_f32, c_u64, c_vp, c_vp, c_vp,
+                                           c_i64, c_i64, c_i64, c_i64, c_i64, c_vp]),
     "mmu_colsum_reduce": (c_i32, [c_vp, c_i64, c_i64, c_vp, c_i32, c_vp]),
     "mmu_colsum_reduce_multi": (c_i32, [c_i32, c_vp, c_vp, c_vp, c_i64, c_i32, c_vp]),
     "mmu_colsum_bf16": (c_i32, [c_vp, c_i64, c_i64, c_i64, c_vp, c_vp, c_i32, c_vp]),
diff --git a/multi-modal-uncertainty_amd/src/encoder.py b/multi-modal-uncertainty_amd/src/encoder.py
--- a/multi-modal-uncertainty_amd/src/encoder.py
+++ b/multi-modal-uncertainty_amd/src/encoder.py
@@ -78,6 +78,119 @@
     return Y, S2, mean2, rstd2, saved, Y32
 
 
+LAST_LAYER_CLS = os.environ.get("MMU_LAST_CLS", "1") != "0"
+
+
+def _cls_rows(t, B, L):
+    return t.view(B, L, *t.shape[1:])[:, 0].contiguous()
+
+
+def last_layer_forward(lw, X, R, keymask, B, L, p_attn, p_hid, seeds, save, res_ln=None):
+    M = B * L
+    dev = X.device
+    f32 = torch.float32
+    qkv = torch.empty(M, 3 * HID, dtype=bf16, device=dev)
+    K.gemm(X, HID, True, lw.wqkv16[HID:], HID, True, qkv[:, HID:], 3 * HID, M, 2 * HID, HID,
+           epi=K.epilogue(K.EPI_STORE, bias=lw.bqkv[HID:]))
+    Xc = _cls_rows(X, B, L)
+    K.gemm(Xc, HID, True, lw.wqkv16[:HID], HID, True, qkv, L * 3 * HID, B, HID, HID,
+           epi=K.epilogue(K.EPI_STORE, bias=lw.bqkv[:HID]))
+    O = torch.empty(M, HID, dtype=bf16, device=dev)
+    lse = torch.empty(B * HEADS, L, dtype=f32, device=dev)
+    dmask = K.dropmask_empty(B, L, HEADS, dev) if (save and p_attn > 0) else None
+    K.attention_row0_fwd(qkv, keymask, O, lse, B, L, HEADS, p_attn, seeds[0], dmask)
+    Oc = _cls_rows(O, B, L)
+    Rc = _cls_rows(R, B, L)
+    if res_ln is not None:
+        res_ln = (_cls_rows(res_ln[0], B, L), _cls_rows(res_ln[1], B, L), res_ln[2], res_ln[3])
+    S1 = torch.empty(B, HID, dtype=f32, device=dev)
+    K.gemm(Oc, HID, True, lw.wo16, HID, True, S1, HID, B, HID, HID,
+           epi=K.epilogue(K.EPI_BIAS_DROP_RES, bias=lw.bo, residual=Rc, drop_p=p_hid, seed=seeds[1], res_ln=res_ln),
+           row_step=L)
+    A = torch.empty(B, HID, dtype=bf16, device=dev)
+    mean1 = torch.empty(B, dtype=f32, device=dev)
+    rstd1 = torch.empty(B, dtype=f32, device=dev)
+    K.layernorm_fwd_f32(S1, lw.ln1w, lw.ln1b, A, None, mean1, rstd1)
+    Z = torch.empty(B, FFN, dtype=bf16, device=dev) if save else None
+    Hh = torch.empty(B, FFN, dtype=bf16, device=dev)
+    K.gemm(A, HID, True, lw.w116, HID, True, Hh, FFN, B, FFN, HID, epi=K.epilogue(K.EPI_BIAS_GELU, bias=lw.b1, aux=Z))
+    S2 = torch.empty(B, HID, dtype=f32, device=dev)
+    K.gemm(Hh, FFN, True, lw.w216, FFN, True, S2, HID, B, HID, FFN,
+           epi=K.epilogue(K.EPI_BIAS_DROP_RES, bias=lw.b2, residual=S1, drop_p=p_hid, seed=seeds[2],
+                          res_ln=(mean1, rstd1, lw.ln1w, lw.ln1b)), row_step=L)
+    Y32 = torch.empty(B, HID, dtype=f32, device=dev)
+    mean2 = torch.empty(B, dtype=f32, device=dev)
+    rstd2 = torch.empty(B, dtype=f32, device=dev)
+    K.layernorm_fwd_f32(S2, lw.ln2w, lw.ln2b, torch.empty(B, HID, dtype=bf16, device=dev), Y32, mean2, rstd2)
+    saved = None
+    if save:
+        saved = (X, Xc, qkv, Oc, lse[:, 0].contiguous(), dmask[:, 0].contiguous() if dmask is not None else None,
+                 S1, mean1, rstd1, A, Z, Hh, S2, mean2, rstd2)
+    return Y32, saved
+
+
+def last_layer_backward(lw, saved, dY32, keymask, B, L, p_attn, p_hid, seeds, wgrad):
+    X, Xc, qkv, Oc, lse0, kw0, S1, mean1, rstd1, A, Z, Hh, S2, mean2, rstd2 = saved
+    M = B * L
+    dev = dY32.device
+    P = K.ln_parts(B)
+    side = _Side(dev, wgrad)
+    pw = pb = pbias = pw1 = pb1 = pbias1 = None
+    if wgrad:
+        pw, pb, pbias, pw1, pb1, pbias1 = (torch.empty(P, HID, dtype=torch.float32, device=dev) for _ in range(6))
+    acc = K.epilogue(K.EPI_STORE, accumulate=True)
+    dY = dY32.to(bf16).contiguous()
+    dS2 = torch.empty(B, HID, dtype=bf16, device=dev)
+    dY2 = torch.empty(B, HID, dtype=bf16, device=dev)
+    K.layernorm_bwd(dY, S2, mean2, rstd2, lw.ln2w, dS2, dY2, p_hid, seeds[2], pw, pb, pbias, row_step=L)
+    if wgrad:
+        def w2():
+            K.colsum_reduce_multi([(pw, lw.g_ln2w), (pb, lw.g_ln2b), (pbias, lw.g_b2)], accumulate=True)
+            K.gemm(dY2, HID, False, Hh, FFN, False, lw.g_w2, FFN, HID, FFN, B, epi=acc)
+        side.run(w2, pw, pb, pbias, dY2, Hh)
+    dZ = torch.empty(B, FFN, dtype=bf16, device=dev)
+    K.gemm(dY2, HID, True, lw.w2t16, HID, True, dZ, FFN, B, FFN, HID,
+           epi=K.epilogue(K.EPI_DGELU, aux=Z, colsum=lw.g_b1 if wgrad else None))
+    if wgrad:
+        side.run(lambda: K.gemm(dZ, FFN, False, A, HID, False, lw.g_w1, HID, FFN, HID, B, epi=acc), dZ, A)
+    dA = torch.empty(B, HID, dtype=bf16, device=dev)
+    K.gemm(dZ, FFN, True, lw.w1t16, FFN, True, dA, HID, B, HID, FFN, epi=K.epilogue(K.EPI_ADD_RES, residual=dS2))
+    dS1 = torch.empty(B, HID, dtype=bf16, device=dev)
+    dAo = torch.empty(B, HID, dtype=bf16, device=dev)
+    K.layernorm_bwd(dA, S1, mean1, rstd1, lw.ln1w, dS1, dAo, p_hid, seeds[1], pw1, pb1, pbias1, row_step=L)
+    if wgrad:
+        def wo():
+            K.colsum_reduce_multi([(pw1, lw.g_ln1w), (pb1, lw.g_ln1b), (pbias1, lw.g_bo)], accumulate=True)
+            K.gemm(dAo, HID, False, Oc, HID, False, lw.g_wo, HID, HID, HID, B, epi=acc)
+        side.run(wo, pw1, pb1, pbias1, dAo, Oc)
+    dO = torch.empty(M, HID, dtype=bf16, device=dev)
+    K.gemm(dAo, HID, True, lw.wot16, HID, True, dO, L * HID, B, HID, HID)
+    O = torch.empty(M, HID, dtype=bf16, device=dev)
+    O.view(B, L, HID)[:, 0] = Oc
+    lse = torch.empty(B * HEADS, L, dtype=torch.float32, device=dev)
+    lse[:, 0] = lse0
+    dmask = None
+    if kw0 is not None:
+        dmask = K.dropmask_empty(B, L, HEADS, dev)
+        dmask[:, 0] = kw0
+    dqkv = torch.empty(M, 3 * HID, dtype=bf16, device=dev)
+    dbs = K.attention_row0_dbias(B, HEADS, dev) if wgrad else None
+    K.attention_row0_bwd(qkv, keymask, O, dO, lse, dqkv, B, L, HEADS, p_attn, dmask, dbs)
+    dqkv_c = _cls_rows(dqkv, B, L)
+    if wgrad:
+        def wqkv():
+            K.colsum_reduce_multi([(dbs[0], lw.g_bqkv[:HID]), (dbs[1], lw.g_bqkv[HID:2 * HID]),
+                                   (dbs[2], lw.g_bqkv[2 * HID:])], accumulate=True)
+            K.gemm(dqkv[:, HID:], 3 * HID, False, X, HID, False, lw.g_wqkv[HID:], HID, 2 * HID, HID, M, epi=acc)
+            K.gemm(dqkv_c, 3 * HID, False, Xc, HID, False, lw.g_wqkv[:HID], HID, HID, HID, B, epi=acc)
+        side.run(wqkv, dqkv, dqkv_c, X, Xc, dbs)
+    dX = torch.empty(M, HID, dtype=bf16, device=dev)
+    K.gemm(dqkv[:, HID:], 3 * HID, True, lw.wqkvt16[:, HID:], 3 * HID, True, dX, HID, M, HID, 2 * HID)
+    K.gemm(dqkv_c, 3 * HID, True, lw.wqkvt16, 3 * HID, True, dX, L * HID, B, HID, 3 * HID,
+           epi=K.epilogue(K.EPI_ADD_RES, residual=dS1))
+    return dX, side
+
+
 def encoder_stack(lws, X, X32, keymask, B, L, p_attn, p_hid, seeds_of, need_grad, hook=None, all_layers=False,
                   cls_only=False):
     R, rln, outs = X32, None, []
@@ -86,6 +199,11 @@
         out32 = all_layers or i == n - 1
         if out32 and cls_only and not all_layers:
             out32 = "cls"
+        if out32 == "cls" and LAST_LAYER_CLS:
+            if need_grad:
+                return BertLastLayerFunction.apply(X, R, lw.anchor, lw, keymask, B, L, p_attn, p_hid, seeds_of(i),
+                                                   hook, rln, i == 0)
+            return last_layer_forward(lw, X, R, keymask, B, L, p_attn, p_hid, seeds_of(i), False, rln)[0]
         if need_grad:
             X, R, mu, rs, Y32 = BertLayerFunction.apply(X, R, lw.anchor, lw, keymask, B, L, p_attn, p_hid,
                                                         seeds_of(i), hook, rln, out32, i == 0)
@@ -309,3 +427,39 @@
         elif wgrad and hook is not None:
             hook(lw)
         return (dX,) + (None,) * 13
+
+
+
+class BertLastLayerFunction(torch.autograd.Function):
+
+    @staticmethod
+    def forward(ctx, X, R, anchor, lw, keymask, B, L, p_attn, p_hid, seeds, on_grads_ready, res_ln=None,
+                flush=False):
+        ctx.set_materialize_grads(False)
+        e0 = _mark()
+        Y32, saved = last_layer_forward(lw, X, R, keymask, B, L, p_attn, p_hid, seeds, True, res_ln)
+        if e0 is not None:
+            _block_events.append((e0, _mark()))
+        ctx.saved_bufs = saved
+        ctx.meta = (lw, keymask, B, L, p_attn, p_hid, seeds, on_grads_ready, flush)
+        return Y32
+
+    @staticmethod
+    def backward(ctx, dY32):
+        lw, keymask, B, L, p_attn, p_hid, seeds, hook, flush = ctx.meta
+        if dY32 is None:
+            return (None,) * 13
+        wgrad = lw.trainable()
+        e0 = _mark()
+        dX, side = last_layer_backward(lw, ctx.saved_bufs, dY32, keymask, B, L, p_attn, p_hid, seeds, wgrad)
+        if e0 is not None:
+            _block_events.append((e0, _mark()))
+        ctx.saved_bufs = None
+        if wgrad and side.defer:
+            if hook is not None:
+                _defer(side.dev, lambda: hook(lw), ())
+            if flush:
+                _flush_deferred(side.dev, INTERLEAVE)
+        elif wgrad and hook is not None:
+            hook(lw)
+        return (dX,) + (None,) * 12
diff --git a/multi-modal-uncertainty_amd/src/kernels.py b/multi-modal-uncertainty_amd/src/kernels.py
--- a/multi-modal-uncertainty_amd/src/kernels.py
+++ b/multi-modal-uncertainty_amd/src/kernels.py
@@ -150,7 +150,8 @@
     torch.autograd.Variable._execution_engine.queue_callback(join)
 
 
-def gemm(A, lda, a_kmajor, B, ldb, b_kmajor, C, ldc, M, N_, K, epi=None, batch=1, sA=0, sB=0, sC=0):
+def gemm(A, lda, a_kmajor, B, ldb, b_kmajor, C, ldc, M, N_, K, epi=None, batch=1, sA=0, sB=0, sC=0, row_step=None,
+         row_offset=0):
     _dev_check(A, B, C)
     _want(A, torch.bfloat16, "gemm A")
     _want(B, torch.bfloat16, "gemm B")
@@ -163,8 +164,12 @@
         epi = type(epi).from_buffer_copy(epi)
         ws = _splitk_workspace(C.device)
         epi.workspace, epi.workspace_floats = ws.data_ptr(), ws.numel()
-    N.call("mmu_gemm", _ptr(A), lda, int(a_kmajor), _ptr(B), ldb, int(b_kmajor), _ptr(C), ldc, cdt, M, N_, K,
-           batch, sA, sB, sC, ctypes.byref(epi) if epi is not None else None, _stream(C))
+    if row_step is not None:
+        N.call("mmu_gemm_rows", _ptr(A), lda, int(a_kmajor), _ptr(B), ldb, int(b_kmajor), _ptr(C), ldc, cdt, M, N_, K,
+               batch, sA, sB, sC, ctypes.byref(epi), int(row_step), int(row_offset), _stream(C))
+    else:
+        N.call("mmu_gemm", _ptr(A), lda, int(a_kmajor), _ptr(B), ldb, int(b_kmajor), _ptr(C), ldc, cdt, M, N_, K,
+               batch, sA, sB, sC, ctypes.byref(epi) if epi is not None else None, _stream(C))
     if _alg["on"]:
         _count_alg(M, N_, K, batch, 4 if cdt == N.MMU_F32 else 2, epi)
     return C
@@ -249,6 +254,48 @@
     N.call("mmu_attention_bwd", _ptr(qkv), qkv.stride(0), _ptr(keymask), _ptr(O), O.stride(0), _ptr(dO), dO.stride(0),
            _ptr(lse), _ptr(delta), _ptr(dqkv), dqkv.stride(0), batch, L, heads, float(drop_p), int(seed),
            _ptr(dropmask) if dropmask is not None else None, _ptr(dbias_parts), _stream(qkv))
+
+
+def _row0_check(who, batch, L, heads, *mats):
+    for t in mats:
+        _want(t, torch.bfloat16, who)
+        if t.dim() != 2 or t.shape[0] < batch * L or t.shape[1] < heads * 64 or t.stride(1) != 1 \
+                or t.stride(0) % 8 or t.data_ptr() % 16:
+            raise N.NativeError(f"{who}: operands are [batch * L, cols] bf16 with 16-B aligned rows, got "
+                                f"{tuple(t.shape)} strides {t.stride()}")
+
+
+def attention_row0_fwd(qkv, keymask, O, lse, batch, L, heads=12, drop_p=0.0, seed=0, dropmask=None):
+    _dev_check(qkv, keymask, O, lse)
+    _row0_check("attention_row0_fwd", batch, L, heads, qkv, O)
+    if dropmask is not None:
+        _dev_check(dropmask)
+        if dropmask.numel() < batch * heads * L * ((L + 63) // 64) or not dropmask.is_contiguous():
+            raise ValueError("attention_row0_fwd: dropmask too small / not contiguous")
+    if lse.numel() < batch * heads * L or keymask.numel() < batch * L:
+        raise ValueError("attention_row0_fwd: lse [batch * heads, L] / keymask [batch, L] too small")
+    N.call("mmu_attention_row0_fwd", _ptr(qkv), qkv.stride(0), _ptr(keymask), _ptr(O), O.stride(0), _ptr(lse), batch,
+           L, heads, float(drop_p), int(seed) & 0xFFFFFFFFFFFFFFFF, _ptr(dropmask), _stream(qkv))
+
+
+def attention_row0_dbias(batch, heads=12, device=None):
+    return torch.empty(3, batch, heads * 64, dtype=torch.float32, device=device)
+
+
+def attention_row0_bwd(qkv, keymask, O, dO, lse, dqkv, batch, L, heads=12, drop_p=0.0, dropmask=None,
+                       dbias_sums=None):
+    _dev_check(qkv, keymask, O, dO, lse, dqkv, dbias_sums)
+    _row0_check("attention_row0_bwd", batch, L, heads, qkv, dqkv, O, dO)
+    if dropmask is not None:
+        _dev_check(dropmask)
+        if dropmask.numel() < batch * heads * L * ((L + 63) // 64) or not dropmask.is_contiguous():
+            raise ValueError("attention_row0_bwd: dropmask too small / not contiguous")
+    if dbias_sums is not None and (dbias_sums.dtype != torch.float32 or not dbias_sums.is_contiguous()
+                                   or dbias_sums.numel() < 3 * batch * heads * 64):
+        raise ValueError("attention_row0_bwd: dbias_sums must be contiguous f32 [3, batch, heads * 64]")
+    N.call("mmu_attention_row0_bwd", _ptr(qkv), qkv.stride(0), _ptr(keymask), _ptr(O), O.stride(0), _ptr(dO),
+           dO.stride(0), _ptr(lse), _ptr(dqkv), dqkv.stride(0), batch, L, heads, float(drop_p), _ptr(dropmask),
+           _ptr(dbias_sums), _stream(qkv))
 
 
 LN_ROWS_PER_PART = 64
@@ -326,13 +373,21 @@
 
 
 def layernorm_bwd(dY, X, mean, rstd, w, dX, dXdrop=None, drop_p=0.0, seed=0, part_dw=None, part_db=None,
-                  part_dbias=None):
+                  part_dbias=None, row_step=None, row_offset=0):
     x32 = X.dtype == torch.float32
+    stepped = row_step is not None
+    if stepped and not x32:
+        raise N.NativeError("layernorm_bwd: row_step / row_offset need an f32 X")
     rows, H = _ln_rows("layernorm_bwd", X, torch.float32 if x32 else torch.bfloat16,
                        same=(("dY", dY), ("dX", dX), ("dXdrop", dXdrop)), vecs=(("mean", mean), ("rstd", rstd)),
                        parts=(("part_dw", part_dw), ("part_db", part_db), ("part_dbias", part_dbias)))
     _ln_params("layernorm_bwd", rows, H, 0, 0, w=w)
     _dev_check(dY, X, mean, rstd, w, dX, dXdrop, part_dw, part_db, part_dbias)
+    if stepped:
+        N.call("mmu_layernorm_bwd_f32_rows", _ptr(dY), _ptr(X), _ptr(mean), _ptr(rstd), _ptr(w), _ptr(dX),
+               _ptr(dXdrop), float(drop_p), int(seed), _ptr(part_dw), _ptr(part_db), _ptr(part_dbias), rows, H,
+               LN_ROWS_PER_PART, int(row_step), int(row_offset), _stream(X))
+        return
     N.call("mmu_layernorm_bwd_f32" if x32 else "mmu_layernorm_bwd", _ptr(dY), _ptr(X), _ptr(mean), _ptr(rstd),
            _ptr(w), _ptr(dX), _ptr(dXdrop), float(drop_p), int(seed), _ptr(part_dw), _ptr(part_db), _ptr(part_dbias),
            rows, H, LN_ROWS_PER_PART, _stream(X))
```

Result: faster. 1684 (median of 6 runs) (+4.2%).
